# ashiq24/UNO

Measured on AMD Instinct MI355X. Metric: UNO training samples/s (421^2 Darcy), higher is better.
Workload: dtype f32; 1 GPU; Darcy 2D 421x421, UNO_9(3,64,pad=5) 64ch, batch 16/GPU, train step (fwd+loss+bwd+allreduce+Adam); global_batch=16, parallelism=dp1

## Files before the change

include/uno_spectral.h:

```cpp
#ifndef UNO_SPECTRAL_H
#define UNO_SPECTRAL_H

#ifdef __cplusplus
extern "C" {
#endif

#define UNO_SPECTRAL_ABI_VERSION 14

int uno_abi_version(void);
void* uno_upload_table(const void* host, long long bytes);

const char* uno_last_error(void);

long long uno_spectral_conv2d_fwd_ws_bytes(int B, int Ci, int Co, int m1, int m2);
long long uno_spectral_conv2d_bwd_ws_bytes(int B, int Ci, int Co, int m1, int m2);

int uno_spectral_conv2d_forward(const float* x, const float* w1, const float* w2, float* y,
                                float* xtrunc, void* ws, int B, int Ci, int Co, int H, int W,
                                int Ho, int Wo, int m1, int m2, void* stream);

int uno_spectral_conv2d_backward(const float* gy, const float* xtrunc, const float* w1,
                                 const float* w2, float* gx, float* gw1, float* gw2, void* ws,
                                 int B, int Ci, int Co, int H, int W, int Ho, int Wo, int m1,
                                 int m2, void* stream);

int uno_spectral_conv2d_forward_bf16(const void* x, const float* w1, const float* w2, void* y,
                                     float* xtrunc, void* ws, int B, int Ci, int Co, int H, int W,
                                     int Ho, int Wo, int m1, int m2, void* stream);
int uno_spectral_conv2d_backward_bf16(const void* gy, const float* xtrunc, const float* w1,
                                      const float* w2, void* gx, float* gw1, float* gw2, void* ws,
                                      int B, int Ci, int Co, int H, int W, int Ho, int Wo, int m1,
                                      int m2, void* stream);

long long uno_fft_resample3d_ws_bytes(int n_vol, int D1, int M1, int J1, int J2, int m3);
int uno_fft_resample3d(const float* x, float* y, void* ws, int n_vol, int D1, int D2, int D3, int M1, int M2, int M3,
                       int J1, const int* f1_in, const int* f1_out, int J2, const int* f2_in, const int* f2_out, int m3,
                       float scale, int herm_in, int herm_out, void* stream);

int uno_fft_resample3d_acc(const float* x, float* y, float* y_act, void* ws, int n_vol, int D1, int D2, int D3, int M1, int M2, int M3,
                           int J1, const int* f1_in, const int* f1_out, int J2, const int* f2_in, const int* f2_out, int m3,
                           float scale, int herm_in, int herm_out, void* stream);

long long uno_fft_resample3d_any_ws_bytes(int n_vol, int D1, int M1, int J1, int J2, int m3);
int uno_fft_resample3d_any(const float* x, float* y, void* ws, int n_vol, int D1, int D2, int D3, int M1, int M2, int M3,
                           int J1, const int* f1_in, const int* f1_out, int J2, const int* f2_in, const int* f2_out, int m3,
                           float scale, int herm_in, int herm_out, void* stream);

int uno_fft_resample3d_any_acc(const float* x, float* y, float* y_act, void* ws, int n_vol, int D1, int D2, int D3, int M1, int M2, int M3,
                               int J1, const int* f1_in, const int* f1_out, int J2, const int* f2_in, const int* f2_out, int m3,
                               float scale, int herm_in, int herm_out, void* stream);

long long uno_spectral_conv3d_fwd_ws_bytes(int B, int Ci, int Co, int H, int Ho, int m1, int m2, int m3);
long long uno_spectral_conv3d_bwd_ws_bytes(int B, int Ci, int Co, int H, int Ho, int m1, int m2, int m3);
int uno_spectral_conv3d_forward(const float* x, const float* const* w, float* y, float* xtrunc, void* ws,
                                int B, int Ci, int Co, int H, int W, int T, int Ho, int Wo, int To,
                                int m1, int m2, int m3, void* stream);
int uno_spectral_conv3d_backward(const float* gy, const float* xtrunc, const float* const* w, float* gx,
                                 float* const* gw, void* ws, int B, int Ci, int Co, int H, int W, int T,
                                 int Ho, int Wo, int To, int m1, int m2, int m3, void* stream);

int uno_cdft_axis(const float* in, float* out, int inverse, int n_img, int H, int m1, int m2, int m3,
                  float scale, int mask_overlap, void* stream);


int uno_dft2d_forward(const float* images, float* spec, int n_img, int H, int W, int m1, int m2,
                      float scale, int hermitian_cols, int mask_overlap, void* stream);

int uno_dft2d_inverse(const float* spec, float* images, int n_img, int H, int W, int m1, int m2,
                      float scale, int hermitian_cols, int mask_overlap, void* stream);

int uno_reserve_cus(int n);

int uno_sweep_alternation(int enable);

int uno_dft2d_inverse_add_applies(int n_img, int H, int W, int m1, int m2, int Hs, int Ws);
int uno_dft2d_inverse_add(const float* spec, float* images, int n_img, int H, int W, int m1, int m2, float scale, int hermitian_cols,
                          int mask_overlap, const float* addend, int Hs, int Ws, const int* tile_p0, const float* row_op,
                          const int* col_v0, const float* col_op, void* stream);

int uno_dft2d_forward_resample_applies(int n_img, int H, int W, int m1, int m2, int Ho, int Wo, int KW);
int uno_dft2d_forward_resample(const float* images, float* spec, int n_img, int H, int W, int m1, int m2, float scale, int hermitian_cols,
                               int mask_overlap, int group, int stride, int offset, float* resampled, int Ho, int Wo, const int* col_start,
                               const float* col_wt, int KW, const int* row_tiles, const float* row_op, void* stream);

int uno_dft2d_forward_bf16(const void* images, float* spec, int n_img, int H, int W, int m1, int m2,
                           float scale, int hermitian_cols, int mask_overlap, void* stream);
int uno_dft2d_inverse_bf16(const float* spec, void* images, int n_img, int H, int W, int m1, int m2,
                           float scale, int hermitian_cols, int mask_overlap, void* stream);

int uno_dft2d_forward_grouped(const float* images, float* spec, int n_img, int H, int W, int m1, int m2, float scale,
                              int hermitian_cols, int mask_overlap, int group, int stride, int offset, void* stream);
int uno_dft2d_inverse_grouped(const float* spec, float* images, int n_img, int H, int W, int m1, int m2, float scale,
                              int hermitian_cols, int mask_overlap, int group, int stride, int offset, void* stream);

int uno_mode_mix(const float* in, const float* const* w, float* out, int op, int B, int Ci, int Co,
                 int ncorner, int modes_per_corner, void* stream);

int uno_mode_wgrad(const float* xtrunc, const float* go, float* const* gw, int B, int Ci, int Co,
                   int ncorner, int modes_per_corner, void* stream);
int uno_mode_backward(const float* xtrunc, const float* go, const float* const* w, float* gx_spec, float* const* gw, int B, int Ci,
                      int Co, int ncorner, int modes_per_corner, int accumulate, void* stream);
int uno_mode_wgrad_acc(const float* xtrunc, const float* go, float* const* gw, int B, int Ci, int Co, int ncorner,
                       int modes_per_corner, int accumulate, void* stream);
int uno_spectral_conv2d_backward_acc(const void* gy, const float* xtrunc, const void* w1, const void* w2, void* gx,
                                     float* gw1, float* gw2, void* ws, int B, int Ci, int Co, int H, int W, int Ho, int Wo,
                                     int m1, int m2, int io_format, int accumulate_gw, void* stream);

int uno_resample2d(const float* in, float* out, float* tmp, int n_img, int H, int W, int Ho, int Wo,
                   const int* startH, const float* wtH, int KH, const int* startW, const float* wtW, int KW,
                   const int* tile_p0, const float* tile_w, int NP, int accumulate, void* stream);

int uno_channel_mix(const float* x, const float* w, const float* bias, float* y, int B, int Ci, int Co,
                    long long P, int transpose_w, int accumulate, int act_in, const float* dgelu_of, void* stream);

long long uno_channel_wgrad_ws_bytes(int B, int Ci, int Co, long long P);
int uno_channel_wgrad(const float* gy, const float* x, float* gw, float* gb, void* ws, int B, int Ci, int Co,
                      long long P, int act_x, void* stream);

int uno_channel_mix2(const float* x1, const float* x2, int C1, const float* w, const float* bias, float* y1, float* y2, int Co1,
                     float* y_act, int B, int Ci, int Co, long long P, int transpose_w, int accumulate, int act_in,
                     const float* dgelu_of, const float* proj_w, const float* proj_b, float* proj_out, void* stream);
int uno_channel_wgrad2(const float* gy, const float* x1, const float* x2, int C1, float* gw, float* gb, void* ws, int B, int Ci,
                       int Co, long long P, int act_x, int accumulate, void* stream);
int uno_channel_wgrad_finish(const void* parts, float* gw, float* gb, int Ci, int Co, long long nparts, int accumulate, void* stream);

int uno_gelu_project_forward(const float* pre, const float* w, const float* bias, float* out, int B, int C, long long P,
                             void* stream);
long long uno_gelu_project_bwd_ws_bytes(int B, int C, long long P);
int uno_gelu_project_backward(const float* pre, const float* w, const float* gout, float* gpre, float* gw, float* gb,
                              void* ws, int B, int C, long long P, void* stream);

int uno_gelu_project2_forward(const float* pre, const float* s, const float* w, const float* bias, float* out, int B, int C1, int C2,
                              long long P, int act2, void* stream);
long long uno_gelu_project2_bwd_ws_bytes(int B, int C1, int C2, long long P);
int uno_gelu_project2_backward(const float* pre, const float* s, const float* w, const float* gout, float* gpre, float* gs, float* gw,
                               float* gb, void* ws, int B, int C1, int C2, long long P, int act2, void* stream);

long long uno_rel_l2_steps_ws_bytes(int B, long long P, int T);
int uno_rel_l2_steps(const float* pred, const float* target, float* sums, float* rel, float* totals, void* ws, int B, long long P, int T,
                     void* stream);

long long uno_rollout_ws_bytes(int B, long long P, int T);
int uno_rollout_advance(float* window, const float* frame, const float* target, float* pred, void* ws, int B, int C, int T_in, long long P,
                        int T, int t, int shift, void* stream);
int uno_rollout_finish(const void* ws, float* sums, float* rel, float* totals, int B, long long P, int T, void* stream);

int uno_rollout_lift(const float* given, const float* pred, const float* feat, const float* w, const float* bias, float* h, int B, int T_in,
                     int F, int Cm, long long P, int T, int t, void* stream);
long long uno_rollout_lift_bwd_ws_bytes(int B, int T_in, int F, int Cm, long long P, int T);
int uno_rollout_lift_backward(const float* gh, const float* given, const float* pred, const float* target, const float* feat, const float* w,
                              const float* sums, const float* gL, float* gpred, float* gframe, void* parts, int B, int T_in, int F, int Cm,
                              long long P, int T, int t, void* stream);
int uno_rollout_loss_seed(const float* pred, const float* target, const float* sums, const float* gL, float* gframe, int B, long long P, int T,
                          void* stream);

int uno_channel_mix2_win(const float* x1, const float* x2, int C1, const float* w, const float* bias, float* y1, float* y2, int Co1,
                         float* y_act, int B, int Ci, int Co, int rows, int cols, int pitch, long long plane, int transpose_w,
                         int accumulate, int act_in, const float* dgelu_of, const float* proj_w, const float* proj_b, float* proj_out,
                         void* stream);
int uno_channel_wgrad2_win(const float* gy, const float* x1, const float* x2, int C1, float* gw, float* gb, void* ws, int B, int Ci,
                           int Co, int rows, int cols, int pitch, long long plane, int act_x, int accumulate, void* stream);
int uno_gelu_project_backward_win(const float* pre, const float* w, const float* gout, float* gpre, float* gw, float* gb, void* ws,
                                  int B, int C, int rows, int cols, int pitch, long long plane, void* stream);
int uno_project_backward_applies(int B, int C1, int Ci, int Co, int rows, int cols, int pitch, long long plane);
long long uno_project_backward_ws_bytes(int B, int Ci, int Co, long long P);
int uno_project_backward(const float* x1, const float* x2, int C1, const float* w, const float* pre, const float* w2, const float* gout,
                         float* g1, float* g2, float* gw, float* gb, float* gw2, float* gb2, void* ws, int B, int Ci, int Co, int rows,
                         int cols, int pitch, long long plane, int act_in, int accumulate_w, void* stream);
int uno_clear_border(float* t, long long n_planes, int Hp, int Wp, int rows, int cols, void* stream);
int uno_channel_mix_act_padded(const float* x, const float* w, const float* bias, float* y, float* y_act, int B, int Ci, int Co, int H,
                               int W, int Hp, int Wp, int act_in, void* stream);
int uno_channel_mix_dgelu_padded(const float* x, const float* w, const float* bias, const float* g_padded, float* gz, int B, int Ci,
                                 int Co, int H, int W, int Hp, int Wp, int act_in, void* stream);
int uno_lift_forward(const float* x, const float* w1, const float* b1, const float* w0, const float* b0, float* act, int B, int Cin,
                     int Cm, int Co, int H, int W, int Hp, int Wp, void* stream);
long long uno_lift_bwd_ws_bytes(int B, int Cin, int Cm, int Co, int H, int W);
int uno_lift_backward(const float* x, const float* w1, const float* b1, const float* w0, const float* b0, const float* g_act, float* gw1,
                      float* gb1, float* gw0, float* gb0, void* ws, int B, int Cin, int Cm, int Co, int H, int W, int Hp, int Wp,
                      void* stream);
int uno_lift_backward_takes_second(int B, int Cin, int Cm, int Co, int H, int W, int Hp, int Wp);
int uno_lift_backward2(const float* x, const float* w1, const float* b1, const float* w0, const float* b0, const float* g_act,
                       const float* g_act2, float* gw1, float* gb1, float* gw0, float* gb0, void* ws, int B, int Cin, int Cm, int Co,
                       int H, int W, int Hp, int Wp, void* stream);

int uno_gelu_pad(const float* s, const float* gy, float* out, int n_img, int H, int W, int Hp, int Wp, int backward,
                 void* stream);

int uno_instnorm_forward(const float* x, const float* gamma, const float* beta, float* y, float* mean, float* rstd, long long rows,
                         int C, long long N, float eps, int gelu, void* stream);
int uno_instnorm_backward(const float* x, const float* gy, const float* gamma, const float* beta, const float* mean,
                          const float* rstd, float* gx, float* s1, float* s2, long long rows, int C, long long N, int gelu,
                          void* stream);

int uno_adam_step(float* p, const float* g, float* m, float* v, long long n, int is_complex, double lr, double beta1,
                  double beta2, double eps, double weight_decay, int step, void* stream);

int uno_adam_step_multi(int n_tensors, float* const* p, const float* const* g, float* const* m, float* const* v,
                        const long long* n, const int* is_complex, double lr, double beta1, double beta2, double eps,
                        double weight_decay, int step, void* stream);

int uno_adam_step_multi_dev(int n_tensors, float* const* p, const float* const* g, float* const* m, float* const* v,
                            const long long* n, const int* is_complex, double lr, double beta1, double beta2, double eps,
                            double weight_decay, int* step_counter, float* scalars, const double* hyper, void* stream);

int uno_spectral_conv2d_forward_mixed(const void* x_bf16, const void* w1_f16, const void* w2_f16, void* y_bf16,
                                      float* xtrunc, void* ws, int B, int Ci, int Co, int H, int W, int Ho, int Wo,
                                      int modes1, int modes2, void* stream);
int uno_spectral_conv2d_backward_mixed(const void* gy_bf16, const float* xtrunc, const void* w1_f16, const void* w2_f16,
                                       void* gx_bf16, float* gw1, float* gw2, void* ws, int B, int Ci, int Co, int H, int W,
                                       int Ho, int Wo, int modes1, int modes2, void* stream);
int uno_mode_mix_f16w(const float* in, const void* const* w_f16, float* out, int op, int B, int Ci, int Co, int ncorner,
                      int modes_per_corner, void* stream);
int uno_dft2d_forward_grouped_bf16(const void* images, float* spec, int n_img, int H, int W, int m1, int m2, float scale,
                                   int hermitian_cols, int mask_overlap, int group, int stride, int offset, void* stream);
int uno_dft2d_inverse_grouped_bf16(const float* spec, void* images, int n_img, int H, int W, int m1, int m2, float scale,
                                   int hermitian_cols, int mask_overlap, int group, int stride, int offset, void* stream);
int uno_resample2d_bf16(const void* in, void* out, float* tmp, int n_img, int H, int W, int Ho, int Wo, const int* startH,
                        const float* wtH, int KH, const int* startW, const float* wtW, int KW, const int* tile_p0,
                        const float* tile_w, int NP, int accumulate, void* stream);
int uno_channel_mix_bf16(const void* x, const float* w, const float* bias, void* y, int B, int Ci, int Co, long long P,
                         int transpose_w, int accumulate, int act_in, const void* dgelu_of, void* stream);
int uno_channel_wgrad_bf16(const void* gy, const void* x, float* gw, float* gb, void* ws, int B, int Ci, int Co, long long P,
                           int act_x, void* stream);
int uno_channel_mix2_bf16(const void* x1, const void* x2, int C1, const float* w, const float* bias, void* y1, void* y2, int Co1,
                          void* y_act, int B, int Ci, int Co, long long P, int transpose_w, int accumulate, int act_in,
                          const void* dgelu_of, const float* proj_w, const float* proj_b, void* proj_out, void* stream);
int uno_channel_wgrad2_bf16(const void* gy, const void* x1, const void* x2, int C1, float* gw, float* gb, void* ws, int B, int Ci,
                            int Co, long long P, int act_x, int accumulate, void* stream);
int uno_gelu_project_forward_bf16(const void* pre, const float* w, const float* bias, void* out, int B, int C, long long P,
                                  void* stream);
int uno_gelu_project_backward_bf16(const void* pre, const float* w, const void* gout, void* gpre, float* gw, float* gb,
                                   void* ws, int B, int C, long long P, void* stream);
int uno_gelu_pad_bf16(const void* s, const void* gy, void* out, int n_img, int H, int W, int Hp, int Wp, int backward,
                      void* stream);
int uno_instnorm_forward_bf16(const void* x, const float* gamma, const float* beta, void* y, float* mean, float* rstd,
                              long long rows, int C, long long N, float eps, int gelu, void* stream);
// ... 20 lines not shown
```

uno_amd/_native.py:

```python
from __future__ import annotations

import ctypes as C
import os
import threading

import torch

_HERE = os.path.dirname(os.path.abspath(__file__))
LIB_PATH = os.path.join(_HERE, "lib", "libuno_spectral.so")
ABI_VERSION = 14

_lib = None
_lock = threading.Lock()

_fp = C.c_void_p
_i = C.c_int
_SIGNATURES = {
    "uno_abi_version": (C.c_int, []),
    "uno_last_error": (C.c_char_p, []),
    "uno_dft2d_any_ws_bytes": (C.c_longlong, [_i] * 5),
    "uno_scratch_provide": (C.c_int, [_fp, C.c_longlong]),
    "uno_spectral_conv2d_fwd_ws_bytes": (C.c_longlong, [_i] * 5),
    "uno_spectral_conv2d_bwd_ws_bytes": (C.c_longlong, [_i] * 5),
    "uno_spectral_conv2d_forward": (C.c_int, [_fp] * 6 + [_i] * 9 + [_fp]),
    "uno_spectral_conv2d_backward": (C.c_int, [_fp] * 8 + [_i] * 9 + [_fp]),
    "uno_spectral_conv2d_forward_bf16": (C.c_int, [_fp] * 6 + [_i] * 9 + [_fp]),
    "uno_spectral_conv2d_backward_bf16": (C.c_int, [_fp] * 8 + [_i] * 9 + [_fp]),
    "uno_fft_resample3d_ws_bytes": (C.c_longlong, [_i] * 6),
    "uno_fft_resample3d": (C.c_int, [_fp] * 3 + [_i] * 8 + [_fp, _fp, _i, _fp, _fp, _i, C.c_float, _i, _i, _fp]),
    "uno_fft_resample3d_acc": (C.c_int, [_fp] * 4 + [_i] * 8 + [_fp, _fp, _i, _fp, _fp, _i, C.c_float, _i, _i, _fp]),
    "uno_fft_resample3d_any_ws_bytes": (C.c_longlong, [_i] * 6),
    "uno_fft_resample3d_any": (C.c_int, [_fp] * 3 + [_i] * 8 + [_fp, _fp, _i, _fp, _fp, _i, C.c_float, _i, _i, _fp]),
    "uno_fft_resample3d_any_acc": (C.c_int, [_fp] * 4 + [_i] * 8 + [_fp, _fp, _i, _fp, _fp, _i, C.c_float, _i, _i, _fp]),
    "uno_dft2d_forward": (C.c_int, [_fp, _fp] + [_i] * 5 + [C.c_float, _i, _i, _fp]),
    "uno_dft2d_forward_bf16": (C.c_int, [_fp, _fp] + [_i] * 5 + [C.c_float, _i, _i, _fp]),
    "uno_dft2d_inverse_bf16": (C.c_int, [_fp, _fp] + [_i] * 5 + [C.c_float, _i, _i, _fp]),
    "uno_dft2d_inverse": (C.c_int, [_fp, _fp] + [_i] * 5 + [C.c_float, _i, _i, _fp]),
    "uno_reserve_cus": (C.c_int, [_i]),
    "uno_sweep_alternation": (C.c_int, [_i]),
    "uno_dft2d_inverse_add_applies": (C.c_int, [_i] * 7),
    "uno_dft2d_forward_resample_applies": (C.c_int, [_i] * 8),
    "uno_dft2d_forward_resample": (C.c_int, [_fp, _fp] + [_i] * 5 + [C.c_float] + [_i] * 5 + [_fp, _i, _i, _fp, _fp, _i, _fp, _fp, _fp]),
    "uno_dft2d_inverse_add": (C.c_int, [_fp, _fp] + [_i] * 5 + [C.c_float, _i, _i, _fp, _i, _i, _fp, _fp, _fp, _fp, _fp]),
    "uno_dft2d_forward_grouped": (C.c_int, [_fp, _fp] + [_i] * 5 + [C.c_float] + [_i] * 5 + [_fp]),
    "uno_dft2d_inverse_grouped": (C.c_int, [_fp, _fp] + [_i] * 5 + [C.c_float] + [_i] * 5 + [_fp]),
    "uno_mode_mix": (C.c_int, [_fp, C.POINTER(_fp), _fp] + [_i] * 6 + [_fp]),
    "uno_mode_wgrad": (C.c_int, [_fp, _fp, C.POINTER(_fp)] + [_i] * 5 + [_fp]),
    "uno_mode_backward": (C.c_int, [_fp, _fp, C.POINTER(_fp), _fp, C.POINTER(_fp)] + [_i] * 6 + [_fp]),
    "uno_spectral_conv3d_fwd_ws_bytes": (C.c_longlong, [_i] * 8),
    "uno_spectral_conv3d_bwd_ws_bytes": (C.c_longlong, [_i] * 8),
    "uno_spectral_conv3d_forward": (C.c_int, [_fp, C.POINTER(_fp), _fp, _fp, _fp] + [_i] * 12 + [_fp]),
    "uno_spectral_conv3d_backward": (C.c_int, [_fp, _fp, C.POINTER(_fp), _fp, C.POINTER(_fp), _fp] + [_i] * 12 + [_fp]),
    "uno_cdft_axis": (C.c_int, [_fp, _fp] + [_i] * 6 + [C.c_float, _i, _fp]),
    "uno_resample2d": (C.c_int, [_fp, _fp, _fp] + [_i] * 5 + [_fp, _fp, _i, _fp, _fp, _i, _fp, _fp, _i, _i, _fp]),
    "uno_channel_mix": (C.c_int, [_fp, _fp, _fp, _fp, _i, _i, _i, C.c_longlong, _i, _i, _i, _fp, _fp]),
    "uno_channel_wgrad_ws_bytes": (C.c_longlong, [_i, _i, _i, C.c_longlong]),
    "uno_channel_wgrad": (C.c_int, [_fp, _fp, _fp, _fp, _fp, _i, _i, _i, C.c_longlong, _i, _fp]),
    "uno_channel_mix2": (C.c_int, [_fp, _fp, _i, _fp, _fp, _fp, _fp, _i, _fp, _i, _i, _i, C.c_longlong, _i, _i, _i, _fp, _fp, _fp, _fp, _fp]),
    "uno_channel_wgrad2": (C.c_int, [_fp, _fp, _fp, _i, _fp, _fp, _fp, _i, _i, _i, C.c_longlong, _i, _i, _fp]),
    "uno_channel_mix2_win": (C.c_int, [_fp, _fp, _i, _fp, _fp, _fp, _fp, _i, _fp, _i, _i, _i, _i, _i, _i, C.c_longlong, _i, _i, _i, _fp, _fp, _fp, _fp, _fp]),
    "uno_channel_mix_ws_bytes": (C.c_longlong, [_i, _i, C.c_longlong, _i]),
    "uno_clear_border": (C.c_int, [_fp, C.c_longlong, _i, _i, _i, _i, _fp]),
    "uno_channel_mix_act_padded": (C.c_int, [_fp, _fp, _fp, _fp, _fp, _i, _i, _i, _i, _i, _i, _i, _i, _fp]),
    "uno_lift_forward": (C.c_int, [_fp] * 6 + [_i] * 8 + [_fp]),
    "uno_lift_bwd_ws_bytes": (C.c_longlong, [_i] * 6),
    "uno_lift_backward": (C.c_int, [_fp] * 11 + [_i] * 8 + [_fp]),
    "uno_lift_backward2": (C.c_int, [_fp] * 12 + [_i] * 8 + [_fp]),
    "uno_lift_backward_takes_second": (C.c_int, [_i] * 8),
    "uno_channel_mix_dgelu_padded": (C.c_int, [_fp, _fp, _fp, _fp, _fp, _i, _i, _i, _i, _i, _i, _i, _i, _fp]),
    "uno_channel_wgrad2_win": (C.c_int, [_fp, _fp, _fp, _i, _fp, _fp, _fp, _i, _i, _i, _i, _i, _i, C.c_longlong, _i, _i, _fp]),
    "uno_gelu_project_backward_win": (C.c_int, [_fp] * 7 + [_i, _i, _i, _i, _i, C.c_longlong, _fp]),
    "uno_channel_wgrad_finish": (C.c_int, [_fp, _fp, _fp, _i, _i, C.c_longlong, _i, _fp]),
    "uno_mode_wgrad_acc": (C.c_int, [_fp, _fp, C.POINTER(_fp)] + [_i] * 6 + [_fp]),
    "uno_spectral_conv2d_backward_acc": (C.c_int, [_fp] * 8 + [_i] * 11 + [_fp]),
    "uno_upload_table": (C.c_void_p, [_fp, C.c_longlong]),
    "uno_project_backward_applies": (C.c_int, [_i] * 7 + [C.c_longlong]),
    "uno_project_backward_ws_bytes": (C.c_longlong, [_i, _i, _i, C.c_longlong]),
    "uno_project_backward": (C.c_int, [_fp, _fp, _i] + [_fp] * 11 + [_i] * 6 + [C.c_longlong, _i, _i, _fp]),
    "uno_gelu_project_forward": (C.c_int, [_fp, _fp, _fp, _fp, _i, _i, C.c_longlong, _fp]),
    "uno_gelu_project_bwd_ws_bytes": (C.c_longlong, [_i, _i, C.c_longlong]),
    "uno_gelu_project_backward": (C.c_int, [_fp] * 7 + [_i, _i, C.c_longlong, _fp]),
    "uno_gelu_project2_forward": (C.c_int, [_fp] * 5 + [_i, _i, _i, C.c_longlong, _i, _fp]),
    "uno_gelu_project2_bwd_ws_bytes": (C.c_longlong, [_i, _i, _i, C.c_longlong]),
    "uno_gelu_project2_backward": (C.c_int, [_fp] * 9 + [_i, _i, _i, C.c_longlong, _i, _fp]),
    "uno_rel_l2_steps_ws_bytes": (C.c_longlong, [_i, C.c_longlong, _i]),
    "uno_rel_l2_steps": (C.c_int, [_fp] * 6 + [_i, C.c_longlong, _i, _fp]),
    "uno_rollout_ws_bytes": (C.c_longlong, [_i, C.c_longlong, _i]),
    "uno_rollout_advance": (C.c_int, [_fp] * 5 + [_i, _i, _i, C.c_longlong, _i, _i, _i, _fp]),
    "uno_rollout_finish": (C.c_int, [_fp] * 4 + [_i, C.c_longlong, _i, _fp]),
    "uno_rollout_lift": (C.c_int, [_fp] * 6 + [_i, _i, _i, _i, C.c_longlong, _i, _i, _fp]),
    "uno_rollout_lift_bwd_ws_bytes": (C.c_longlong, [_i, _i, _i, _i, C.c_longlong, _i]),
    "uno_rollout_lift_backward": (C.c_int, [_fp] * 11 + [_i, _i, _i, _i, C.c_longlong, _i, _i, _fp]),
    "uno_rollout_loss_seed": (C.c_int, [_fp] * 5 + [_i, C.c_longlong, _i, _fp]),
    "uno_gelu_pad": (C.c_int, [_fp, _fp, _fp] + [_i] * 6 + [_fp]),
    "uno_transpose_batched": (C.c_int, [_fp, _fp, _i, C.c_longlong, _i] + [C.c_longlong] * 4 + [_fp]),
    "uno_instnorm_forward": (C.c_int, [_fp] * 6 + [C.c_longlong, _i, C.c_longlong, C.c_float, _i, _fp]),
    "uno_instnorm_backward": (C.c_int, [_fp] * 9 + [C.c_longlong, _i, C.c_longlong, _i, _fp]),
    "uno_adam_step": (C.c_int, [_fp, _fp, _fp, _fp, C.c_longlong, _i] + [C.c_double] * 5 + [_i, _fp]),
    "uno_adam_step_multi": (C.c_int, [_i, C.POINTER(_fp), C.POINTER(_fp), C.POINTER(_fp), C.POINTER(_fp), C.POINTER(C.c_longlong),
                                      C.POINTER(_i)] + [C.c_double] * 5 + [_i, _fp]),
    "uno_adam_step_multi_dev": (C.c_int, [_i, C.POINTER(_fp), C.POINTER(_fp), C.POINTER(_fp), C.POINTER(_fp), C.POINTER(C.c_longlong),
                                          C.POINTER(_i)] + [C.c_double] * 5 + [_fp, _fp, _fp, _fp]),
    "uno_spectral_conv2d_forward_mixed": (C.c_int, [_fp] * 6 + [_i] * 9 + [_fp]),
    "uno_spectral_conv2d_backward_mixed": (C.c_int, [_fp] * 8 + [_i] * 9 + [_fp]),
    "uno_mode_mix_f16w": (C.c_int, [_fp, C.POINTER(_fp), _fp] + [_i] * 6 + [_fp]),
    "uno_dft2d_forward_grouped_bf16": (C.c_int, [_fp, _fp] + [_i] * 5 + [C.c_float] + [_i] * 5 + [_fp]),
    "uno_dft2d_inverse_grouped_bf16": (C.c_int, [_fp, _fp] + [_i] * 5 + [C.c_float] + [_i] * 5 + [_fp]),
    "uno_resample2d_bf16": (C.c_int, [_fp, _fp, _fp] + [_i] * 5 + [_fp, _fp, _i, _fp, _fp, _i, _fp, _fp, _i, _i, _fp]),
    "uno_channel_mix_bf16": (C.c_int, [_fp, _fp, _fp, _fp, _i, _i, _i, C.c_longlong, _i, _i, _i, _fp, _fp]),
    "uno_channel_wgrad_bf16": (C.c_int, [_fp, _fp, _fp, _fp, _fp, _i, _i, _i, C.c_longlong, _i, _fp]),
    "uno_channel_mix2_bf16": (C.c_int, [_fp, _fp, _i, _fp, _fp, _fp, _fp, _i, _fp, _i, _i, _i, C.c_longlong, _i, _i, _i, _fp, _fp, _fp, _fp, _fp]),
    "uno_channel_wgrad2_bf16": (C.c_int, [_fp, _fp, _fp, _i, _fp, _fp, _fp, _i, _i, _i, C.c_longlong, _i, _i, _fp]),
    "uno_gelu_project_forward_bf16": (C.c_int, [_fp, _fp, _fp, _fp, _i, _i, C.c_longlong, _fp]),
    "uno_gelu_project_backward_bf16": (C.c_int, [_fp] * 7 + [_i, _i, C.c_longlong, _fp]),
    "uno_gelu_pad_bf16": (C.c_int, [_fp, _fp, _fp] + [_i] * 6 + [_fp]),
    "uno_instnorm_forward_bf16": (C.c_int, [_fp] * 6 + [C.c_longlong, _i, C.c_longlong, C.c_float, _i, _fp]),
    "uno_instnorm_backward_bf16": (C.c_int, [_fp] * 9 + [C.c_longlong, _i, C.c_longlong, _i, _fp]),
    "uno_profile_begin": (C.c_int, [_i]),
    "uno_profile_end": (C.c_int, []),
    "uno_profile_get": (C.c_int, [_i, C.c_char_p, _i, C.POINTER(C.c_double), C.POINTER(C.c_double)]),
}
EXPORTED_SYMBOLS = tuple(_SIGNATURES)


def lib():
    global _lib
    if _lib is None:
        with _lock:
            if _lib is None:
                if not os.path.exists(LIB_PATH):
                    raise RuntimeError(
                        f"uno_amd: native library {LIB_PATH} is missing - build it with "
                        "`python -m uno_amd.build` (hipcc, gfx950); there is no CPU fallback")
                h = C.CDLL(LIB_PATH)
                for name, (res, args) in _SIGNATURES.items():
                    fn = getattr(h, name)
                    fn.restype = res
                    fn.argtypes = args
                if h.uno_abi_version() != ABI_VERSION:
                    raise RuntimeError(f"uno_amd: ABI mismatch, library {h.uno_abi_version()} != binding {ABI_VERSION}")
                _lib = h
    return _lib


def _check(rc: int, what: str):
    if rc != 0:
        msg = lib().uno_last_error().decode(errors="replace")
        raise RuntimeError(f"{what} failed (code {rc}): {msg}")


def _ptr(t: torch.Tensor):
    return C.c_void_p(t.data_ptr())


def _opt(t):
    return _ptr(t) if t is not None else C.c_void_p(0)


def _count(lead) -> int:
    n = 1
    for d in lead:
        n *= d
    return n


def _stream(t: torch.Tensor):
    return C.c_void_p(torch.cuda.current_stream(t.device).cuda_stream)


class _scratch:

    def __init__(self, device, nbytes):
        self.bytes, self.device, self.buf = nbytes, device, None

    def __enter__(self):
        if self.bytes > 0:
            self.buf = torch.empty(self.bytes, dtype=torch.uint8, device=self.device)
            _check(lib().uno_scratch_provide(_ptr(self.buf), self.bytes), "uno_scratch_provide")
        return self

    def __exit__(self, *exc):
        if self.bytes > 0:
            lib().uno_scratch_provide(None, 0)
        return False


class _any_mode_scratch(_scratch):

    def __init__(self, device, *needs):
        L = lib()
        _scratch.__init__(self, device, max((int(L.uno_dft2d_any_ws_bytes(*[int(v) for v in n])) for n in needs), default=0))


class _mix_scratch(_scratch):

    def __init__(self, device, Ci, Co, P, bf16):
        _scratch.__init__(self, device, int(lib().uno_channel_mix_ws_bytes(int(Ci), int(Co), int(P), 1 if bf16 else 0)))

# ... 17 lines not shown
    _require(t, torch.bfloat16 if bf16 else torch.float32, name)
    return bf16


def _weights_half(w1, w2, bf16):
    if w1.dtype == torch.float16:
        if not bf16:
            raise RuntimeError("uno_amd: half-precision weight storage goes with bfloat16 activations")
        for w, name in ((w1, "weights1"), (w2, "weights2")):
            _require(w, torch.float16, name)
            if w.dim() != 5 or w.shape[-1] != 2:
                raise RuntimeError("uno_amd: half-precision weights are stored as (Ci, Co, m1, m2, 2) = (re, im)")
        return True
    _require(w1, torch.complex64, "weights1")
    _require(w2, torch.complex64, "weights2")
    return False


def _complex_grad_buffers(out, shape, n: int, device, accumulate: bool):
    if out is None:
        return [torch.empty(shape, dtype=torch.complex64, device=device) for _ in range(n)], False
    gws = list(out)
    for t in gws:
        _require(t, torch.complex64, "weight-gradient buffer")
        if tuple(t.shape) != tuple(shape):
            raise RuntimeError("uno_amd: weight-gradient buffer has the wrong shape")
    return gws, accumulate


def _real_grad_buffers(out_w, out_b, Ci: int, Co: int, need_bias: bool, device, accumulate: bool):
    if out_w is None:
        gw = torch.empty((Co, Ci), dtype=torch.float32, device=device)
        return gw, (torch.empty((Co,), dtype=torch.float32, device=device) if need_bias else None), False
    gw, gb = out_w, (out_b if need_bias else None)
    _require(gw, torch.float32, "weight-gradient buffer")
    if gw.numel() != Co * Ci or (need_bias and (gb is None or gb.numel() != Co)):
        raise RuntimeError("uno_amd: gradient buffers do not match the layer")
    if gb is not None:
        _require(gb, torch.float32, "bias-gradient buffer")
    return gw, gb, accumulate


def spectral_conv2d_forward(x, w1, w2, Ho: int, Wo: int, xt_out=None):
    bf16 = _act_dtype(x, "x")
    wh = _weights_half(w1, w2, bf16)
    B, Ci, H, W = x.shape
    Ci2, Co, m1, m2 = w1.shape[:4]
    if Ci2 != Ci or tuple(w2.shape) != tuple(w1.shape):
        raise RuntimeError(f"uno_amd: weight shapes {tuple(w1.shape)} / {tuple(w2.shape)} do not match input channels {Ci}")
    L = lib()
    with torch.cuda.device(x.device):
        y = torch.empty((B, Co, Ho, Wo), dtype=x.dtype, device=x.device)
        if xt_out is None:
            xt = torch.empty((B, Ci, 2 * m1, m2), dtype=torch.complex64, device=x.device)
        else:
            xt = xt_out
            _require(xt, torch.complex64, "xtrunc buffer")
            if tuple(xt.shape) != (B, Ci, 2 * m1, m2):
                raise RuntimeError("uno_amd: xtrunc buffer has the wrong shape")
        ws = torch.empty(max(1, L.uno_spectral_conv2d_fwd_ws_bytes(B, Ci, Co, m1, m2)), dtype=torch.uint8, device=x.device)
        fn = L.uno_spectral_conv2d_forward_mixed if wh else _entry("uno_spectral_conv2d_forward", bf16)
        with _any_mode_scratch(x.device, (B * Ci, H, W, m1, m2), (B * Co, Ho, Wo, m1, m2)):
            rc = fn(_ptr(x), _ptr(w1), _ptr(w2), _ptr(y), _ptr(xt), _ptr(ws), B, Ci, Co, H, W, Ho, Wo, m1, m2, _stream(x))
    _check(rc, "uno_spectral_conv2d_forward")
    return y, xt


def spectral_conv2d_backward(gy, xt, w1, w2, H: int, W: int, need_gx=True, need_gw=True, gw_out=None, accumulate_gw=False):
    bf16 = _act_dtype(gy, "grad_output")
    _require(xt, torch.complex64, "xtrunc")
    wh = _weights_half(w1, w2, bf16)
    B, Co, Ho, Wo = gy.shape
    Ci, Co2, m1, m2 = w1.shape[:4]
    if Co2 != Co:
        raise RuntimeError("uno_amd: grad_output channels do not match the weights")
    L = lib()
    with torch.cuda.device(gy.device):
        gx = torch.empty((B, Ci, H, W), dtype=gy.dtype, device=gy.device) if need_gx else None
        gw1, gw2, accumulate_gw = None, None, accumulate_gw and need_gw
        if need_gw:
            (gw1, gw2), accumulate_gw = _complex_grad_buffers(gw_out, (Ci, Co, m1, m2), 2, gy.device, accumulate_gw)
        ws = torch.empty(max(1, L.uno_spectral_conv2d_bwd_ws_bytes(B, Ci, Co, m1, m2)), dtype=torch.uint8, device=gy.device)
        with _any_mode_scratch(gy.device, (B * Co, Ho, Wo, m1, m2), (B * Ci, H, W, m1, m2)):
            rc = L.uno_spectral_conv2d_backward_acc(_ptr(gy), _ptr(xt), _ptr(w1), _ptr(w2), _opt(gx), _opt(gw1), _opt(gw2),
                                                    _ptr(ws), B, Ci, Co, H, W, Ho, Wo, m1, m2, 2 if wh else (1 if bf16 else 0),
                                                    1 if accumulate_gw else 0, _stream(gy))
    _check(rc, "uno_spectral_conv2d_backward")
    return gx, gw1, gw2


def _fft_resample3d(any_grid: bool, x, out_size, f1, f2, m3, scale, adjoint, out, act):
    name = "uno_fft_resample3d_any" if any_grid else "uno_fft_resample3d"
    _require(x, torch.float32, "x")
    *lead, D1, D2, D3 = x.shape
    M1, M2, M3 = (int(v) for v in out_size)
    n = _count(lead)
    for t in (*f1, *f2):
        if t.dtype != torch.int32 or not t.is_cuda or not t.is_contiguous():
            raise RuntimeError("uno_amd: frequency tables must be contiguous int32 device tensors")
    J1, J2 = f1[0].numel(), f2[0].numel()
    if any_grid and (f1[1].numel() != J1 or f2[1].numel() != J2):
        raise RuntimeError("uno_amd: the forward and inverse frequency tables of an axis must have the same length")
    L = lib()
    with torch.cuda.device(x.device):
        ws = torch.empty(max(1, getattr(L, name + "_ws_bytes")(n, D1, M1, J1, J2, int(m3))), dtype=torch.uint8, device=x.device)
        if out is not None:
            _require(out, torch.float32, "out")
            if tuple(out.shape) != (*lead, M1, M2, M3) or not out.is_contiguous():
                raise RuntimeError(f"uno_amd: out must be a contiguous {(*lead, M1, M2, M3)} tensor")
            ya = torch.empty_like(out) if act else None
            fn, dst, res = getattr(L, name + "_acc"), (_ptr(out), _opt(ya)), ((out, ya) if act else out)
        else:
            res = torch.empty((*lead, M1, M2, M3), dtype=torch.float32, device=x.device)
            fn, dst = getattr(L, name), (_ptr(res),)
        rc = fn(_ptr(x), *dst, _ptr(ws), n, D1, D2, D3, M1, M2, M3, J1, _ptr(f1[0]), _ptr(f1[1]), J2, _ptr(f2[0]), _ptr(f2[1]),
                int(m3), float(scale), int(adjoint), int(not adjoint), _stream(x))
    _check(rc, name + ("_acc" if out is not None else ""))
    return res


def fft_resample3d(x, out_size, f1, f2, m3: int, scale: float, adjoint: bool, out=None, act=False):
    return _fft_resample3d(False, x, out_size, f1, f2, m3, scale, adjoint, out, act)


def fft_resample3d_any(x, out_size, f1, f2, m3: int, scale: float, adjoint: bool, out=None, act=False):
    return _fft_resample3d(True, x, out_size, f1, f2, m3, scale, adjoint, out, act)


def dft2d_forward(images, m1, m2, scale=1.0, hermitian_cols=False, mask_overlap=False, out=None, channel_offset=0):
    bf16 = _act_dtype(images, "images")
    *lead, H, W = images.shape
    n = _count(lead)
    if out is None:
        spec = torch.empty((*lead, 2 * m1, m2), dtype=torch.complex64, device=images.device)
        with torch.cuda.device(images.device):
            fn = _entry("uno_dft2d_forward", bf16)
            with _any_mode_scratch(images.device, (n, H, W, m1, m2)):
                rc = fn(_ptr(images), _ptr(spec), n, H, W, m1, m2, float(scale), int(hermitian_cols), int(mask_overlap), _stream(images))
        _check(rc, "uno_dft2d_forward")
        return spec
    _require(out, torch.complex64, "out")
    if images.dim() != 4 or out.dim() != 4 or out.shape[0] != images.shape[0] or tuple(out.shape[2:]) != (2 * m1, m2) \
            or channel_offset < 0 or channel_offset + images.shape[1] > out.shape[1]:
        raise RuntimeError("uno_amd: out must be (B, Ctot, 2*m1, m2) with room for the image channels at channel_offset")
    with torch.cuda.device(images.device):
        fn = _entry("uno_dft2d_forward_grouped", bf16)
        with _any_mode_scratch(images.device, (n, H, W, m1, m2)):
            rc = fn(_ptr(images), _ptr(out), n, H, W, m1, m2, float(scale), int(hermitian_cols),
                    int(mask_overlap), images.shape[1], out.shape[1], int(channel_offset), _stream(images))
    _check(rc, "uno_dft2d_forward_grouped")
    return out


def reserve_cus(n: int) -> int:
    return int(lib().uno_reserve_cus(int(n)))


def sweep_alternation(enable: bool) -> bool:
    return bool(lib().uno_sweep_alternation(1 if enable else 0))


def sweep_direction(mode: str, mask: int = 255) -> int:
    if mode not in ("alternate", "forward", "reversed") or not 0 <= int(mask) <= 255:
        raise ValueError(f"uno_amd: sweep_direction({mode!r}, {mask!r}): mode is alternate | forward | reversed, mask 0 .. 255")
    value = {"alternate": int(mask), "forward": 0, "reversed": 256 | int(mask)}[mode]
    if value == 1:
        raise ValueError("uno_amd: sweep_direction('alternate', 1): the C entry point reads 1 as 'every family' (255)")
    return int(lib().uno_sweep_alternation(value))


def dft2d_inverse_add_applies(n_img, H, W, m1, m2, Hs, Ws) -> bool:
    return bool(lib().uno_dft2d_inverse_add_applies(int(n_img), int(H), int(W), int(m1), int(m2), int(Hs), int(Ws)))


def dft2d_forward_resample_applies(n_img, H, W, m1, m2, Ho, Wo, KW) -> bool:
    return bool(lib().uno_dft2d_forward_resample_applies(int(n_img), int(H), int(W), int(m1), int(m2), int(Ho), int(Wo), int(KW)))


def dft2d_forward_resample(images, m1, m2, Ho, Wo, tables, scale=1.0, hermitian_cols=False, mask_overlap=False, out=None, channel_offset=0):
    _require(images, torch.float32, "images")
    col_start, col_wt, row_tiles, row_op = tables
    *lead, H, W = images.shape
    n = _count(lead)
    group = stride = 0
    if out is None:
        spec = torch.empty((*lead, 2 * m1, m2), dtype=torch.complex64, device=images.device)
    else:
        _require(out, torch.complex64, "out")
        if images.dim() != 4 or out.dim() != 4 or out.shape[0] != images.shape[0] or tuple(out.shape[2:]) != (2 * m1, m2) \
                or channel_offset < 0 or channel_offset + images.shape[1] > out.shape[1]:
            raise RuntimeError("uno_amd: out must be (B, Ctot, 2*m1, m2) with room for the image channels at channel_offset")
        spec, group, stride = out, images.shape[1], out.shape[1]
    res = torch.empty((*lead, Ho, Wo), dtype=torch.float32, device=images.device)
    with torch.cuda.device(images.device):
        rc = lib().uno_dft2d_forward_resample(_ptr(images), _ptr(spec), n, H, W, m1, m2, float(scale), int(hermitian_cols), int(mask_overlap),
                                              int(group), int(stride), int(channel_offset), _ptr(res), int(Ho), int(Wo), _ptr(col_start),
                                              _ptr(col_wt), int(col_wt.shape[1]), _ptr(row_tiles), _ptr(row_op), _stream(images))
    _check(rc, "uno_dft2d_forward_resample")
    return spec, res


def dft2d_inverse(spec, H, W, scale=1.0, hermitian_cols=True, mask_overlap=True, channels=None, channel_offset=0,
                  dtype=torch.float32, addend=None):
    _require(spec, torch.complex64, "spec")
    *lead, r2, m2 = spec.shape
    m1 = r2 // 2
    if addend is not None:
        t, (p0, rowop, v0, colop) = addend
        _require(t, torch.float32, "addend")
        if channels is not None or dtype != torch.float32 or tuple(t.shape[:-2]) != tuple(lead):
            raise RuntimeError("uno_amd: dft2d_inverse(addend=) takes the plain float32 form with one addend image per spectrum")
        n = _count(lead)
        img = torch.empty((*lead, H, W), dtype=torch.float32, device=spec.device)
        with torch.cuda.device(spec.device):
            rc = lib().uno_dft2d_inverse_add(_ptr(spec), _ptr(img), n, H, W, m1, m2, float(scale), int(hermitian_cols), int(mask_overlap),
                                             _ptr(t), t.shape[-2], t.shape[-1], _ptr(p0), _ptr(rowop), _ptr(v0), _ptr(colop), _stream(spec))
        _check(rc, "uno_dft2d_inverse_add")
        return img
    if channels is None:
        n = _count(lead)
        if dtype not in (torch.float32, torch.bfloat16):
            raise RuntimeError("uno_amd: images are float32 or bfloat16")
        img = torch.empty((*lead, H, W), dtype=dtype, device=spec.device)
        with torch.cuda.device(spec.device):
            fn = _entry("uno_dft2d_inverse", dtype == torch.bfloat16)
            with _any_mode_scratch(spec.device, (n, H, W, m1, m2)):
                rc = fn(_ptr(spec), _ptr(img), n, H, W, m1, m2, float(scale), int(hermitian_cols), int(mask_overlap), _stream(spec))
        _check(rc, "uno_dft2d_inverse")
        return img
    if dtype not in (torch.float32, torch.bfloat16):
        raise RuntimeError("uno_amd: images are float32 or bfloat16")
    if spec.dim() != 4 or channel_offset < 0 or channels < 1 or channel_offset + channels > spec.shape[1]:
        raise RuntimeError("uno_amd: spec must be (B, Ctot, 2*m1, m2) holding the requested channel range")
    B = spec.shape[0]
    img = torch.empty((B, channels, H, W), dtype=dtype, device=spec.device)
    with torch.cuda.device(spec.device):
        fn = _entry("uno_dft2d_inverse_grouped", dtype == torch.bfloat16)
        with _any_mode_scratch(spec.device, (B * channels, H, W, m1, m2)):
            rc = fn(_ptr(spec), _ptr(img), B * channels, H, W, m1, m2, float(scale), int(hermitian_cols),
                    int(mask_overlap), int(channels), spec.shape[1], int(channel_offset), _stream(spec))
    _check(rc, "uno_dft2d_inverse_grouped")
    return img


def _ptr_array(ts):
    return (C.c_void_p * len(ts))(*[t.data_ptr() for t in ts])


def mode_mix(inp, weights, op: int):
    _require(inp, torch.complex64, "spectrum")
    half = weights[0].dtype == torch.float16
    for w in weights:
        _require(w, torch.float16 if half else torch.complex64, "weights")
    B = inp.shape[0]
    Ci, Co = weights[0].shape[:2]
    nc = len(weights)
    Mc = weights[0][0, 0].numel() // (2 if half else 1)
    cout = Co if op == 0 else Ci
    out = torch.empty((B, cout, *inp.shape[2:]), dtype=torch.complex64, device=inp.device)
    with torch.cuda.device(inp.device):
        fn = lib().uno_mode_mix_f16w if half else lib().uno_mode_mix
        rc = fn(_ptr(inp), _ptr_array(weights), _ptr(out), op, B, Ci, Co, nc, Mc, _stream(inp))
    _check(rc, "uno_mode_mix")
    return out


def mode_wgrad(xt, go, weight_shape, ncorner: int, out=None, accumulate: bool = False):
    _require(xt, torch.complex64, "xtrunc")
    _require(go, torch.complex64, "grad spectrum")
    B, Ci = xt.shape[:2]
    Co = go.shape[1]
    gws, accumulate = _complex_grad_buffers(out, weight_shape, ncorner, xt.device, accumulate)
    Mc = gws[0][0, 0].numel()
    with torch.cuda.device(xt.device):
        rc = lib().uno_mode_wgrad_acc(_ptr(xt), _ptr(go), _ptr_array(gws), B, Ci, Co, ncorner, Mc, 1 if accumulate else 0, _stream(xt))
    _check(rc, "uno_mode_wgrad")
    return gws


def mode_backward(xt, go, weights, out=None, accumulate: bool = False):
    _require(xt, torch.complex64, "xtrunc")
    _require(go, torch.complex64, "grad spectrum")
    for w in weights:
        _require(w, torch.complex64, "weights")
    B, Ci = xt.shape[:2]
    Co = go.shape[1]
    nc = len(weights)
    Mc = weights[0][0, 0].numel()
    gws, accumulate = _complex_grad_buffers(out, weights[0].shape, nc, xt.device, accumulate)
    gX = torch.empty((B, Ci, nc * Mc), dtype=torch.complex64, device=xt.device)
    with torch.cuda.device(xt.device):
        rc = lib().uno_mode_backward(_ptr(xt), _ptr(go), _ptr_array(list(weights)), _ptr(gX), _ptr_array(gws), B, Ci, Co, nc, Mc,
                                     1 if accumulate else 0, _stream(xt))
    _check(rc, "uno_mode_backward")
    return gX, gws


def spectral_conv3d_forward(x, ws_, Ho: int, Wo: int, To: int):
    _require(x, torch.float32, "x")
    if len(ws_) != 4:
        raise RuntimeError("uno_amd: the 3-D spectral convolution takes four weight tensors")
    for w in ws_:
        _require(w, torch.complex64, "weights")
        if tuple(w.shape) != tuple(ws_[0].shape):
            raise RuntimeError("uno_amd: weights1..4 must have one shape")
    B, Ci, H, W, T = x.shape
# ... 839 lines not shown
```

uno_amd/block2d.py:

```python
import torch
import torch.nn.functional as F
from torch.autograd.function import once_differentiable

from . import _native
from ._param_grads import _grad_targets, _note_use, _stack_arrived, _stack_grad_slot, _stack_take, _stack_wanted
from .pointwise import _mix2_forward, _mix2_input_grads, _plain, _wgrad_into
from .resample import fused_resample_tables, resample_adjoint, resample_forward, upsample_add_tables


def _half_weights(w1, w2):
    out = []
    capturing = w1.is_cuda and torch.cuda.is_current_stream_capturing()
    with torch.no_grad():
        for w in (w1, w2):
            cached = None if capturing else getattr(w, "_uno_half", None)
            if cached is None or cached[0] != w._version or cached[1].device != w.device or cached[2] != w.data_ptr():
                cached = (w._version, torch.view_as_real(w.detach()).half().contiguous(), w.data_ptr())
                if not capturing:
                    try:
                        w._uno_half = cached
                    except (AttributeError, RuntimeError):
                        pass
            out.append(cached[1])
    return out[0], out[1]


def _xt_slot(stack):
    return None if stack is None else stack.xt


def _xt_dest(stack, B, Ci, m1, m2, device):
    slot = _xt_slot(stack)
    return torch.empty((B, Ci, 2 * m1, m2), dtype=torch.complex64, device=device) if slot is None else slot


def _block_prologue(ctx, iw, x, Ci, w1, w2, cw, cb, Ho, Wo, half_weights):
    B, _, H, W = x.shape
    ctx.stack = _stack_take(w1, (B, Ci, 2 * w1.shape[2], w1.shape[3]), x.device, _stack_wanted(ctx, iw, x, half_weights))
    w1, w2 = _plain(w1), _plain(w2)
    if half_weights:
        w1, w2 = _half_weights(w1, w2)
    cwm = _plain(cw).reshape(cw.shape[0], Ci)
    cb = None if cb is None else _plain(cb)
    same = (H, W) == (Ho, Wo)
    return w1, w2, cwm, cb, same, same or Ho * Wo < H * W


def _pointwise_input_grads(g_src, w, C1, gx1, gx2, geom, dgelu_of=None, dgelu_total=False, g_act=None):
    H, W, Ho, Wo, same, mix_last = geom
    B = g_src.shape[0]
    direct = same or not mix_last

    def dest(gx):
        return gx.view(B, gx.shape[1], -1) if direct else None

    g1, g2 = g_act, None
    if gx1 is not None and gx2 is not None:
        g1, g2 = _mix2_input_grads(g_src, w, C1, out1=dest(gx1), out2=dest(gx2))
    else:
        if gx1 is not None and g1 is None:
            g1 = _native.channel_mix(g_src, w if C1 == w.shape[1] else w[:, :C1].contiguous(), None, transpose_w=True, out=dest(gx1),
                                     dgelu_of=dgelu_of, dgelu_total=dgelu_total)
        if gx2 is not None:
            g2 = _native.channel_mix(g_src, w[:, C1:].contiguous(), None, transpose_w=True, out=dest(gx2))
    if not direct:
        for g, gx in ((g1, gx1), (g2, gx2)):
            if gx is not None:
                resample_adjoint(g.view(B, gx.shape[1], Ho, Wo), H, W, out=gx)


class _SpectralConv2dFn(torch.autograd.Function):

    @staticmethod
    def forward(ctx, x, w1, w2, Ho, Wo, half_weights=False):
        ctx.params = (w1, w2)
        x = _plain(x)
        ctx.stack = _stack_take(w1, (x.shape[0], x.shape[1], 2 * w1.shape[2], w1.shape[3]), x.device, _stack_wanted(ctx, 1, x, half_weights))
        w1, w2 = _plain(w1), _plain(w2)
        if half_weights:
            w1, w2 = _half_weights(w1, w2)
        y, xt = _native.spectral_conv2d_forward(x, w1, w2, int(Ho), int(Wo), xt_out=_xt_slot(ctx.stack))
        ctx.save_for_backward(xt, w1, w2)
        ctx.in_hw = (x.shape[-2], x.shape[-1])
        return y

    @staticmethod
    @once_differentiable
    def backward(ctx, gy):
        xt, w1, w2 = ctx.saved_tensors
        gx, gw1, gw2, _ = _spectral_backward(_plain(gy), xt, w1, w2, ctx.in_hw[0], ctx.in_hw[1], ctx.needs_input_grad[0],
                                          ctx.needs_input_grad[1] or ctx.needs_input_grad[2],
                                          ctx.needs_input_grad[1] and ctx.needs_input_grad[2], ctx.params, ctx.stack)
        return gx, gw1, gw2, None, None, None


FUSE_UPSAMPLE_ADD = True


def _fused_addend(t, H, W, m1, m2, adjoint):
    if not FUSE_UPSAMPLE_ADD or t.dtype != torch.float32 or t.dim() != 4 or not t.is_cuda:
        return None
    Hs, Ws = t.shape[-2], t.shape[-1]
    if Hs * Ws >= H * W or not _native.dft2d_inverse_add_applies(t.shape[0] * t.shape[1], H, W, m1, m2, Hs, Ws):
        return None
    tabs = upsample_add_tables(Hs, Ws, H, W, str(t.device), bool(adjoint))
    return None if tabs is None else (t, tabs)


FUSE_FORWARD_RESAMPLE = True


def _fused_resample(x, m1, m2, Ho, Wo, adjoint):
    if not FUSE_FORWARD_RESAMPLE or x.dtype != torch.float32 or x.dim() != 4 or not x.is_cuda:
        return None
    H, W = x.shape[-2], x.shape[-1]
    n = x.shape[0] * x.shape[1]
    if Ho * Wo >= H * W or not _native.dft2d_forward_resample_applies(n, H, W, m1, m2, Ho, Wo, 1):
        return None
    tabs = fused_resample_tables(H, W, Ho, Wo, str(x.device), bool(adjoint))
    if tabs is None or not _native.dft2d_forward_resample_applies(n, H, W, m1, m2, Ho, Wo, tabs[1].shape[1]):
        return None
    return tabs


def _stage_wgrad(stack, gslot, xt, gO, w1, w2, leaves, both_gw, need_gx):
    if gslot is not None:
        return (None, *_stack_arrived(stack, leaves, w1.shape, both_gw))
    tg = _grad_targets(leaves) if both_gw else None
    _note_use(leaves[0])
    out, acc = (tg.dest, tg.accumulate) if tg else (None, False)
    gX = None
    if need_gx and w1.dtype == torch.complex64:
        gX, (gw1, gw2) = _native.mode_backward(xt, gO, [w1, w2], out=out, accumulate=acc)
        gX = gX.view(xt.shape)
    else:
        gw1, gw2 = _native.mode_wgrad(xt, gO, tuple(w1.shape[:4]), 2, out=out, accumulate=acc)
    if tg:
        gw1, gw2 = tg.returned
    return gX, gw1, gw2


def _spectral_backward(gs, xt, w1, w2, H, W, need_gx, need_gw, both_gw, leaves, stack, join=None, addend=None, k1=None):
    B, Co = gs.shape[:2]
    Ci, _, m1, m2 = w1.shape[:4]
    gslot = _stack_grad_slot(stack, Co) if (stack is not None and need_gw) else None
    merging = join is not None and need_gx and bool(join.spectra)
    if addend is not None and not need_gx:
        raise RuntimeError("uno_amd: an addend for the input gradient needs the input gradient")
    if gslot is None and not merging and addend is None and k1 is None and not (need_gx and need_gw and w1.dtype == torch.complex64):
        tg = _grad_targets(leaves) if (need_gw and both_gw) else None
        if need_gw:
            _note_use(leaves[0])
        gx, gw1, gw2 = _native.spectral_conv2d_backward(gs, xt, w1, w2, H, W, need_gx=need_gx, need_gw=need_gw,
                                                        gw_out=tg.dest if tg else None, accumulate_gw=bool(tg and tg.accumulate))
        if tg:
            gw1, gw2 = tg.returned
        return gx, gw1, gw2, False
    gO = _native.dft2d_forward(gs, m1, m2, 1.0, True, True, out=gslot) if k1 is None else k1(gslot)
    gX, gw1, gw2 = _stage_wgrad(stack, gslot, xt, gO, w1, w2, leaves, both_gw, need_gx) if need_gw else (None, None, None)
    gx = None
    if need_gx:
        if gX is None:
            gX = _native.mode_mix(gO.view(B, Co, 2, m1 * m2), [w1, w2], 1).view(B, Ci, 2 * m1, m2)
        if merging:
            gX = join.merge(gX, (H, W))
        gx = _native.dft2d_inverse(gX, H, W, 1.0 / (H * W), False, False, dtype=gs.dtype, addend=addend)
    return gx, gw1, gw2, gslot is not None


class _OperatorBlock2dFn(torch.autograd.Function):

    @staticmethod
    def forward(ctx, x, w1, w2, cw, cb, Ho, Wo, half_weights=False, fuse_gelu=False, join=None, out_join=None):
        ctx.leaves = (w1, w2, cw, cb)
        ctx.join = None
        if join is not None:
            join.reset()
            if ctx.needs_input_grad[0]:
                join.owner = True
                ctx.join = join
        x = _plain(x)
        B, Ci, H, W = x.shape
        Co = cw.shape[0]
        w1, w2, cwm, cb, same, mix_last = _block_prologue(ctx, 1, x, Ci, w1, w2, cw, cb, Ho, Wo, half_weights)
        t = fused = None
        if not mix_last and not half_weights and x.dtype == torch.float32:
            t = _native.channel_mix(x.view(B, Ci, -1), cwm, cb).view(B, Co, H, W)
            fused = _fused_addend(t, Ho, Wo, w1.shape[2], w1.shape[3], False)
        if fused is not None:
            m1, m2 = w1.shape[2], w1.shape[3]
            xt = _xt_dest(ctx.stack, B, Ci, m1, m2, x.device)
            _native.dft2d_forward(x, m1, m2, 1.0 / (H * W), out=xt, channel_offset=0)
            O = _native.mode_mix(xt.view(B, Ci, 2, m1 * m2), [w1, w2], 0)
            s = _native.dft2d_inverse(O.view(B, Co, 2 * m1, m2), Ho, Wo, 1.0, True, True, addend=fused)
        elif mix_last and not same and not half_weights and (rs := _fused_resample(x, w1.shape[2], w1.shape[3], Ho, Wo, False)) is not None:
            m1, m2 = w1.shape[2], w1.shape[3]
            xt = _xt_dest(ctx.stack, B, Ci, m1, m2, x.device)
            _, pre_act = _native.dft2d_forward_resample(x, m1, m2, Ho, Wo, rs, 1.0 / (H * W), out=xt, channel_offset=0)
            O = _native.mode_mix(xt.view(B, Ci, 2, m1 * m2), [w1, w2], 0)
            s = _native.dft2d_inverse(O.view(B, Co, 2 * m1, m2), Ho, Wo, 1.0, True, True)
        else:
            pre_act = None
            if mix_last and not same:
                pre_act = resample_forward(x, Ho, Wo)
            s, xt = _native.spectral_conv2d_forward(x, w1, w2, Ho, Wo, xt_out=_xt_slot(ctx.stack))
        out = s
        if fused is not None:
            act = x
            if fuse_gelu:
                out = F.gelu(s)
        elif mix_last:
            act = x if same else pre_act
            if fuse_gelu:
                _, out = _native.channel_mix2(act.view(B, Ci, -1), None, cwm, cb, out=s.view(B, Co, -1), accumulate=True, y_act=True)
                out = out.view(B, Co, Ho, Wo)
            else:
                _native.channel_mix(act.view(B, Ci, -1), cwm, cb, out=s.view(B, Co, -1))
        else:
            act = x
            if t is None:
                t = _native.channel_mix(x.view(B, Ci, -1), cwm, cb).view(B, Co, H, W)
            resample_forward(t, Ho, Wo, out=s)
            if fuse_gelu:
                out = F.gelu(s)
        ctx.save_for_backward(xt, w1, w2, cwm, act, s if fuse_gelu else None)
        ctx.geom = (H, W, same, mix_last, cb is not None, tuple(cw.shape))
        ctx.out_join = None
        if fuse_gelu and out_join is not None:
            out_join.pre, out_join.dgelu_applied = s, False
            ctx.out_join = out_join
        return out

    @staticmethod
    @once_differentiable
    def backward(ctx, gs):
        xt, w1, w2, cwm, act, pre = ctx.saved_tensors
        H, W, same, mix_last, has_bias, cw_shape = ctx.geom
        gs = _plain(gs)
        if pre is not None:
            oj = ctx.out_join
            if oj is not None and oj.dgelu_applied and oj.pre is not None and oj.pre.data_ptr() == pre.data_ptr():
                oj.dgelu_applied = False
            else:
                gs = torch.ops.aten.gelu_backward(gs, pre)
            if oj is not None:
                oj.pre = None
        B, Co, Ho, Wo = gs.shape
        Ci = cwm.shape[1]
        need_gx = ctx.needs_input_grad[0]
        need_gw = ctx.needs_input_grad[1] or ctx.needs_input_grad[2]
        need_gc = ctx.needs_input_grad[3] or (has_bias and ctx.needs_input_grad[4])
        join = ctx.join
        lw1, lw2, lcw, lcb = ctx.leaves
        g_act = addend = g_t = k1 = None
        if not mix_last:
            rs = _fused_resample(gs, w1.shape[2], w1.shape[3], H, W, True) if w1.dtype == torch.complex64 else None
            if rs is None:
                g_t = resample_adjoint(gs, H, W).view(B, Co, -1)
            else:
                both = []

                def k1(out):
                    both.extend(_native.dft2d_forward_resample(gs, w1.shape[2], w1.shape[3], H, W, rs, 1.0, True, True, out=out))
                    return both[0]
        if mix_last and not same and need_gx and gs.dtype == torch.float32:
            g_act = _native.channel_mix(gs.view(B, Co, -1), cwm, None, transpose_w=True).view(B, Ci, Ho, Wo)
            addend = _fused_addend(g_act, H, W, w1.shape[2], w1.shape[3], True)
        gx, gw1, gw2, stacked = _spectral_backward(gs, xt, w1, w2, H, W, need_gx, need_gw, ctx.needs_input_grad[1] and ctx.needs_input_grad[2],
                                                   (lw1, lw2), ctx.stack, join, addend, k1)
        if k1 is not None:
            g_t = both[1].view(B, Co, -1)
        pstack = ctx.stack if stacked else None
        gcw = gcb = None
        xpre = join.pre if (join is not None and need_gx) else None
        own_last = xpre is not None and not join.pending
        dg_view = xpre.view(B, Ci, -1) if own_last else None
        direct = same or not mix_last
        g_src = gs.view(B, Co, -1) if mix_last else g_t
        if need_gx and (direct or addend is None):
            _pointwise_input_grads(g_src, cwm, Ci, gx, None, (H, W, Ho, Wo, same, mix_last), dgelu_of=dg_view if direct else None,
                                   dgelu_total=own_last and direct, g_act=g_act)
        dg_done = own_last and direct
        if need_gc:
            gcw, gcb = _wgrad_into((lcw, lcb), g_src, act.view(B, Ci, -1), None, ctx.needs_input_grad[3],
                                   has_bias and ctx.needs_input_grad[4], stack=pstack)
            gcw = None if gcw is None else gcw.view(cw_shape)
        if join is not None:
            if need_gx:
                dg_done = join.apply(gx, xpre if not dg_done else None) or dg_done
                if xpre is not None:
                    if not dg_done:
                        gx = torch.ops.aten.gelu_backward(gx, xpre)
                    join.dgelu_applied = True
            join.reset()
        return gx, gw1, gw2, gcw, gcb, None, None, None, None, None, None


class _OperatorBlock2dCatFn(torch.autograd.Function):

    @staticmethod
    def forward(ctx, x1, x2, w1, w2, cw, cb, Ho, Wo, half_weights=False, defer=None):
        ctx.leaves = (w1, w2, cw, cb)
        ctx.defer = defer if (defer is not None and defer.owner and ctx.needs_input_grad[1]) else None
        x1, x2 = _plain(x1), _plain(x2)
        B, C1, H, W = x1.shape
        C2 = x2.shape[1]
        Ci, Co, m1, m2 = w1.shape
        w1, w2, cwm, cb, same, mix_last = _block_prologue(ctx, 2, x1, Ci, w1, w2, cw, cb, Ho, Wo, half_weights)
        xt = _xt_dest(ctx.stack, B, Ci, m1, m2, x1.device)
        _native.dft2d_forward(x1, m1, m2, 1.0 / (H * W), out=xt, channel_offset=0)
        _native.dft2d_forward(x2, m1, m2, 1.0 / (H * W), out=xt, channel_offset=C1)
        O = _native.mode_mix(xt.view(B, Ci, 2, m1 * m2), [w1, w2], 0)
        t = fused = None
        if not mix_last and not half_weights and x1.dtype == torch.float32:
            t = _mix2_forward(x1.view(B, C1, -1), x2.view(B, C2, -1), cwm, cb).view(B, Co, H, W)
            fused = _fused_addend(t, Ho, Wo, m1, m2, False)
        s = _native.dft2d_inverse(O.view(B, Co, 2 * m1, m2), Ho, Wo, 1.0, True, True, dtype=x1.dtype, addend=fused)
        if fused is not None:
            a1, a2 = x1, x2
        elif mix_last:
            a1 = x1 if same else resample_forward(x1, Ho, Wo)
            a2 = x2 if same else resample_forward(x2, Ho, Wo)
            _mix2_forward(a1.view(B, C1, -1), a2.view(B, C2, -1), cwm, cb, out=s.view(B, Co, -1), accumulate=True)
        else:
            a1, a2 = x1, x2
            if t is None:
                t = _mix2_forward(x1.view(B, C1, -1), x2.view(B, C2, -1), cwm, cb).view(B, Co, H, W)
            resample_forward(t, Ho, Wo, out=s)
        ctx.save_for_backward(xt, w1, w2, cwm, a1, a2)
        ctx.geom = (H, W, same, mix_last, cb is not None, tuple(cw.shape))
        return s

    @staticmethod
    @once_differentiable
    def backward(ctx, gs):
        xt, w1, w2, cwm, a1, a2 = ctx.saved_tensors
        H, W, same, mix_last, has_bias, cw_shape = ctx.geom
        gs = _plain(gs)
        B, Co, Ho, Wo = gs.shape
        Ci, _, m1, m2 = w1.shape[:4]
        C1, C2 = a1.shape[1], a2.shape[1]
        need1, need2 = ctx.needs_input_grad[0], ctx.needs_input_grad[1]
        need_gw = ctx.needs_input_grad[2] or ctx.needs_input_grad[3]
        need_gc = ctx.needs_input_grad[4] or (has_bias and ctx.needs_input_grad[5])
        lw1, lw2, lcw, lcb = ctx.leaves
        both_gw = ctx.needs_input_grad[2] and ctx.needs_input_grad[3]
        gslot = _stack_grad_slot(ctx.stack, Co) if (ctx.stack is not None and need_gw) else None
        rs = _fused_resample(gs, m1, m2, H, W, True) if (not mix_last and w1.dtype == torch.complex64) else None
        if rs is not None:
            gO, g_src = _native.dft2d_forward_resample(gs, m1, m2, H, W, rs, 1.0, True, True, out=gslot)
            g_src = g_src.view(B, Co, -1)
        else:
            g_src = gs.view(B, Co, -1) if mix_last else resample_adjoint(gs, H, W).view(B, Co, -1)
            gO = _native.dft2d_forward(gs, m1, m2, 1.0, True, True, out=gslot)
        gXp, gw1, gw2 = _stage_wgrad(ctx.stack, gslot, xt, gO, w1, w2, (lw1, lw2), both_gw, need1 or need2) if need_gw else (None, None, None)
        gx1 = gx2 = None
        defer = ctx.defer if (need2 and ctx.defer is not None and ctx.defer.owner) else None
        if need1 or need2:
            gX = gXp if gXp is not None else _native.mode_mix(gO.view(B, Co, 2, m1 * m2), [w1, w2], 1).view(B, Ci, 2 * m1, m2)
            if need1:
                gx1 = _native.dft2d_inverse(gX, H, W, 1.0 / (H * W), False, False, channels=C1, channel_offset=0, dtype=gs.dtype)
            if defer is not None:
                defer.spectra.append((gX[:, C1:].contiguous(), (H, W)))
            elif need2:
                gx2 = _native.dft2d_inverse(gX, H, W, 1.0 / (H * W), False, False, channels=C2, channel_offset=C1, dtype=gs.dtype)
        gcw = gcb = None
        geom = (H, W, Ho, Wo, same, mix_last)
        if defer is not None:
            cw2 = cwm[:, C1:].contiguous()

            def x2_part(out, dg=None):
                _pointwise_input_grads(g_src, cw2, C2, out, None, geom, dgelu_of=None if dg is None else dg.view(B, C2, -1),
                                       dgelu_total=dg is not None)
            defer.pending.append((x2_part, same or not mix_last))
            _pointwise_input_grads(g_src, cwm, C1, gx1, None, geom)
        else:
            _pointwise_input_grads(g_src, cwm, C1, gx1, gx2, geom)
        if need_gc:
            gcw, gcb = _wgrad_into((lcw, lcb), g_src, a1.view(B, C1, -1), a2.view(B, C2, -1), ctx.needs_input_grad[4],
                                   has_bias and ctx.needs_input_grad[5])
            gcw = None if gcw is None else gcw.view(cw_shape)
        if ctx.defer is not None and gx2 is not None:
            gx2 = ctx.defer.late(gx2)
        return gx1, gx2, gw1, gw2, gcw, gcb, None, None, None, None


def spectral_conv2d(x, weights1, weights2, dim1, dim2):
    return _SpectralConv2dFn.apply(x, weights1, weights2, dim1, dim2)


def spectral_conv2d_mixed(x, weights1, weights2, dim1, dim2):
    if x.dtype != torch.bfloat16:
        raise RuntimeError(f"spectral_conv2d_mixed: input must be bfloat16 (got {x.dtype})")
    for w in (weights1, weights2):
        if w.dtype == torch.float16 and w.shape[-1] != 2:
            raise RuntimeError("spectral_conv2d_mixed: half-precision weights are stored as (..., 2) = (re, im)")
    if weights1.dtype == torch.float16:
        return _SpectralConv2dHalfFn.apply(x, weights1, weights2, dim1, dim2)
    return _SpectralConv2dFn.apply(x, weights1, weights2, dim1, dim2)


class _SpectralConv2dHalfFn(torch.autograd.Function):

    @staticmethod
    def forward(ctx, x, w1h, w2h, Ho, Wo):
        x, w1h, w2h = _plain(x), _plain(w1h), _plain(w2h)
        y, xt = _native.spectral_conv2d_forward(x, w1h, w2h, int(Ho), int(Wo))
        ctx.save_for_backward(xt, w1h, w2h)
        ctx.in_hw = (x.shape[-2], x.shape[-1])
        return y

    @staticmethod
    @once_differentiable
    def backward(ctx, gy):
        xt, w1h, w2h = ctx.saved_tensors
        need_gx = ctx.needs_input_grad[0]
        need_gw = ctx.needs_input_grad[1] or ctx.needs_input_grad[2]
        gx, gw1, gw2 = _native.spectral_conv2d_backward(_plain(gy), xt, w1h, w2h, ctx.in_hw[0], ctx.in_hw[1],
                                                        need_gx=need_gx, need_gw=need_gw)
        if need_gw:
            gw1, gw2 = torch.view_as_real(gw1).half(), torch.view_as_real(gw2).half()
        return gx, gw1, gw2, None, None
```

uno_amd/build.py:

```python
from __future__ import annotations

import argparse
import concurrent.futures as cf
import hashlib
import os
import shutil
import subprocess
import sys

HERE = os.path.dirname(os.path.abspath(__file__))
CSRC = os.path.join(HERE, "csrc")
LIBDIR = os.path.join(HERE, "lib")
LIB = os.path.join(LIBDIR, "libuno_spectral.so")
STAMP = os.path.join(LIBDIR, "libuno_spectral.stamp")
SOURCES = ["capi.hip", "capi_spectral.hip", "capi_pointwise.hip", "dft2d_fwd.hip", "dft2d_fwd_r4.hip", "dft2d_fwd_fd.hip", "dft2d_inv.hip", "dft2d_inv_b.hip", "dft2d_inv_c.hip", "dft2d_inv_add.hip", "dft2d_plane.hip", "dft2d_b16.hip", "mode_gemm.hip", "cdft_axis.hip", "dft3d_volume.hip", "dft_generic.hip", "resample3d_any.hip", "resample2d.hip", "channel_mix.hip", "channel_wgrad.hip", "adam.hip", "pointwise_fused.hip", "instnorm.hip", "lift_bwd.hip", "rel_l2_steps.hip", "rollout.hip", "rollout_train.hip"]
HEADERS = ["uno_common.h", "channel_mix_common.h", "dft2d_fwd_common.h", "dft2d_fwd_kernel.h", "dft2d_fwd_ft_kernel.h", "dft2d_fwd_ht_kernel.h", "dft2d_fwd_fd_kernel.h", "dft2d_inv_kernel.h", "dft2d_inv_add_kernel.h", os.path.join("..", "..", "include", "uno_spectral.h")]
ARCH = "gfx950"
FLAGS = ["-O3", "-std=c++17", "-fPIC", f"--offload-arch={ARCH}", "-fno-gpu-rdc", "-Wall", "-Wno-unused-function"]
EXTRA_FLAGS = {"mode_gemm.hip": ["-mllvm", "-amdgpu-mfma-vgpr-form"], "dft2d_inv_add.hip": ["-mllvm", "-amdgpu-mfma-vgpr-form"]}


def _hipcc() -> str:
    for cand in (os.environ.get("HIPCC"), shutil.which("hipcc"), "/opt/rocm/bin/hipcc"):
        if cand and os.path.exists(cand):
            return cand
    raise RuntimeError("hipcc not found (set HIPCC or install ROCm)")


def _digest() -> str:
    h = hashlib.sha256()
    for f in SOURCES + HEADERS:
        with open(os.path.join(CSRC, f), "rb") as fh:
            h.update(fh.read())
    h.update(" ".join(FLAGS).encode())
    h.update(repr(sorted(EXTRA_FLAGS.items())).encode())
    return h.hexdigest()


def build(force: bool = False, verbose: bool = False) -> str:
    os.makedirs(LIBDIR, exist_ok=True)
    digest = _digest()
    if not force and os.path.exists(LIB) and os.path.exists(STAMP) and open(STAMP).read().strip() == digest:
        return LIB
    hipcc = _hipcc()
    objdir = os.path.join(LIBDIR, "obj")
    os.makedirs(objdir, exist_ok=True)

    def compile_one(src):
        obj = os.path.join(objdir, os.path.splitext(src)[0] + ".o")
        cmd = [hipcc, *FLAGS, *EXTRA_FLAGS.get(src, []), "-c", os.path.join(CSRC, src), "-o", obj]
        if verbose:
            print(" ".join(cmd), flush=True)
        r = subprocess.run(cmd, capture_output=True, text=True)
        if r.returncode != 0:
            raise RuntimeError(f"hipcc failed on {src}:\n{r.stdout}\n{r.stderr}")
        if verbose and r.stderr.strip():
            print(r.stderr)
        return obj

    jobs = min(len(SOURCES), os.cpu_count() or 1, int(os.environ.get("MAX_JOBS", 16)))
    with cf.ThreadPoolExecutor(max_workers=max(1, jobs)) as ex:
        objs = list(ex.map(compile_one, SOURCES))
    cmd = [hipcc, "-shared", "-fPIC", f"--offload-arch={ARCH}", "-fno-gpu-rdc", *objs, "-o", LIB]
    r = subprocess.run(cmd, capture_output=True, text=True)
    if r.returncode != 0:
        raise RuntimeError(f"link failed:\n{r.stdout}\n{r.stderr}")
    with open(STAMP, "w") as fh:
        fh.write(digest)
    return LIB


if __name__ == "__main__":
    ap = argparse.ArgumentParser()
    ap.add_argument("--force", action="store_true")
    ap.add_argument("--verbose", action="store_true")
    a = ap.parse_args()
    print(build(a.force, a.verbose))
```

uno_amd/csrc/capi_spectral.hip:

```cpp
#include "../../include/uno_spectral.h"
#include "uno_common.h"

#include <cstdlib>
#include <map>
#include <mutex>

namespace uno {

static int check_modes2d(const char* who, int H, int W, int Ho, int Wo, int m1, int m2) {
    if (H < 1 || W < 1 || Ho < 1 || Wo < 1) { set_error("%s: empty grid %dx%d -> %dx%d", who, H, W, Ho, Wo); return -1; }
    if (m1 < 1 || m1 > H || m1 > Ho) {
        set_error("%s: modes1=%d incompatible with grid rows %d -> %d (need 1 <= modes1 <= min rows)", who, m1, H, Ho);
        return -1;
    }
    if (m2 < 1 || m2 > W / 2 + 1 || m2 > Wo / 2 + 1) {
        set_error("%s: modes2=%d incompatible with grid cols %d -> %d (need modes2 <= cols/2+1)", who, m2, W, Wo);
        return -1;
    }
    return 0;
}

static int dft2d(bool inverse, const float* in, float* out, int n_img, int H, int W, int m1, int m2, float scale,
                 int herm, int mask, hipStream_t s, int sp_group = 0, int sp_stride = 0, int sp_offset = 0, int bf16 = 0) {
    const char* who = inverse ? "uno_dft2d_inverse" : "uno_dft2d_forward";
// ... 68 lines not shown
                     float2* const* out_w, int B, int Ci, int Co, int nc, int Mc, hipStream_t s, int w_half = 0, int accumulate = 0) {
    ModeGemmParams p;
    const int rc = mode_gemm_params(p, op, act, w, go, out_act, out_w, B, Ci, Co, nc, Mc, s, w_half, accumulate);
    if (rc != 0) return rc < 0 ? rc : 0;
    return launch_mode_gemm(p, s);
}

static int mode_backward(const float2* xtrunc, const float2* go, const float2* const* w, float2* gx_spec, float2* const* gw, int B, int Ci,
                         int Co, int nc, int Mc, hipStream_t s, int accumulate) {
    ModeGemmParams pa, pb;
    const int ra = mode_gemm_params(pa, 1, go, w, nullptr, gx_spec, nullptr, B, Ci, Co, nc, Mc, s, 0, 0);
    if (ra < 0) return ra;
    const int rb = mode_gemm_params(pb, 2, xtrunc, nullptr, go, nullptr, gw, B, Ci, Co, nc, Mc, s, 0, accumulate);
    if (rb < 0) return rb;
    if (ra == 0 && rb == 0) return launch_mode_gemm_pair(pa, pb, s);
    if (rb == 0) if (int rc = launch_mode_gemm(pb, s)) return rc;
    if (ra == 0) return launch_mode_gemm(pa, s);
    return 0;
}

}

using namespace uno;


namespace {
struct SideStream {
    hipStream_t s = nullptr;
    hipEvent_t fork_ev = nullptr, join_ev = nullptr;
    std::mutex mu;
    bool ok = false;
};
SideStream* side_stream_of_current_device() {
    static std::mutex mu;
    static std::map<int, SideStream*> table;
    int dev = 0;
    if (hipGetDevice(&dev) != hipSuccess) return nullptr;
    std::lock_guard<std::mutex> g(mu);
    auto it = table.find(dev);
    if (it != table.end()) return it->second->ok ? it->second : nullptr;
    SideStream* ss = new SideStream();
    ss->ok = hipStreamCreateWithFlags(&ss->s, hipStreamNonBlocking) == hipSuccess &&
             hipEventCreateWithFlags(&ss->fork_ev, hipEventDisableTiming) == hipSuccess &&
             hipEventCreateWithFlags(&ss->join_ev, hipEventDisableTiming) == hipSuccess;
    table[dev] = ss;
    return ss->ok ? ss : nullptr;
}
}

extern "C" {

long long uno_dft2d_any_ws_bytes(int n_img, int H, int W, int m1, int m2) {
    (void)W;
    if (n_img <= 0 || H <= 0 || m2 <= 0) return 0;
    return (m1 > 40 || m2 > 48) ? 8LL * n_img * H * m2 : 0;
}

long long uno_spectral_conv2d_fwd_ws_bytes(int B, int Ci, int Co, int m1, int m2) {
    (void)Ci;
    return 8LL * B * Co * 2 * m1 * m2;
}

long long uno_spectral_conv2d_bwd_ws_bytes(int B, int Ci, int Co, int m1, int m2) {
    return 8LL * B * (Ci + Co) * 2 * m1 * m2;
}

int uno_dft2d_forward(const float* images, float* spec, int n_img, int H, int W, int m1, int m2, float scale,
                      int hermitian_cols, int mask_overlap, void* stream) {
    return dft2d(false, images, spec, n_img, H, W, m1, m2, scale, hermitian_cols, mask_overlap, (hipStream_t)stream);
}

int uno_dft2d_inverse(const float* spec, float* images, int n_img, int H, int W, int m1, int m2, float scale,
                      int hermitian_cols, int mask_overlap, void* stream) {
    return dft2d(true, spec, images, n_img, H, W, m1, m2, scale, hermitian_cols, mask_overlap, (hipStream_t)stream);
}

int uno_dft2d_inverse_add_applies(int n_img, int H, int W, int m1, int m2, int Hs, int Ws) {
    if (n_img < 1 || H < 1 || W < 1 || m1 < 1 || m2 < 1 || Hs < 1 || Ws < 1 || m1 > H || m2 > W / 2 + 1 || m1 > 40 || m2 > 48) return 0;
    Dft2dParams p;
    p.n_img = n_img; p.H = H; p.W = W; p.m1 = m1; p.m2 = m2; p.herm = 1; p.mask = 1;
    p.sp_group = n_img; p.sp_stride = 0;
    p.add_Hs = Hs; p.add_Ws = Ws;
    if (dft2d_inv_plane_applies(p)) return 0;
    return dft2d_inv_add_applies(p) ? 1 : 0;
}

int uno_dft2d_inverse_add(const float* spec, float* images, int n_img, int H, int W, int m1, int m2, float scale, int hermitian_cols,
                          int mask_overlap, const float* addend, int Hs, int Ws, const int* tile_p0, const float* row_op,
                          const int* col_v0, const float* col_op, void* stream) {
    const char* who = "uno_dft2d_inverse_add";
    if (n_img < 0) { set_error("%s: negative image count", who); return -1; }
    if (n_img > 0 && (!spec || !images || !addend || !tile_p0 || !row_op || !col_v0 || !col_op)) { set_error("%s: null pointer", who); return -1; }
    if (int rc = check_modes2d(who, H, W, H, W, m1, m2)) return rc;
    if (Hs < 1 || Ws < 12 || (long long)Hs * Ws * 4 > 0x7fffffffLL) { set_error("%s: bad addend grid %dx%d", who, Hs, Ws); return -1; }
    if (n_img == 0) return 0;
    if (!uno_dft2d_inverse_add_applies(n_img, H, W, m1, m2, Hs, Ws)) {
        set_error("%s: the fused form does not apply to %d images of %dx%d, modes (%d, %d) (query uno_dft2d_inverse_add_applies)", who, n_img, H, W, m1, m2);
        return -3;
    }
    Dft2dParams p;
    p.in = spec; p.out = images; p.n_img = n_img; p.H = H; p.W = W; p.m1 = m1; p.m2 = m2;
    p.scale = scale; p.herm = hermitian_cols ? 1 : 0; p.mask = mask_overlap ? 1 : 0;
    p.sp_group = n_img; p.sp_stride = 0;
    p.twH = twiddle_table(H);
    p.twW = twiddle_table(W);
    if (!p.twH || !p.twW) return -6;
    p.add_src = addend; p.add_Hs = Hs; p.add_Ws = Ws; p.add_p0 = tile_p0; p.add_rowop = row_op; p.add_v0 = col_v0; p.add_colop = col_op;
#ifdef UNO_K3A_DEV
    { static const int dev_exp = getenv("UNO_K3A_STAGGER") ? atoi(getenv("UNO_K3A_STAGGER")) : 0; p.exp = dev_exp; }
#endif
    return launch_dft2d_inv_add(p, (hipStream_t)stream);
}

static void fwd_resample_shape(Dft2dParams& p, int n_img, int H, int W, int m1, int m2, int Ho, int Wo, int KW) {
    p.n_img = n_img; p.H = H; p.W = W; p.m1 = m1; p.m2 = m2;
    p.fd_Ho = Ho; p.fd_Wo = Wo; p.fd_KW = KW;
}

int uno_dft2d_forward_resample_applies(int n_img, int H, int W, int m1, int m2, int Ho, int Wo, int KW) {
    if (n_img < 1 || H < 1 || W < 1 || m1 < 1 || m2 < 1 || Ho < 1 || Wo < 1 || KW < 1 || m1 > H || m2 > W / 2 + 1 || m1 > 40 || m2 > 48) return 0;
    Dft2dParams p;
    fwd_resample_shape(p, n_img, H, W, m1, m2, Ho, Wo, KW);
    return dft2d_fwd_fd_applies(p) ? 1 : 0;
}

int uno_dft2d_forward_resample(const float* images, float* spec, int n_img, int H, int W, int m1, int m2, float scale, int hermitian_cols,
                               int mask_overlap, int group, int stride, int offset, float* resampled, int Ho, int Wo, const int* col_start,
                               const float* col_wt, int KW, const int* row_tiles, const float* row_op, void* stream) {
    const char* who = "uno_dft2d_forward_resample";
    if (n_img < 0) { set_error("%s: negative image count", who); return -1; }
    if (n_img > 0 && (!images || !spec || !resampled || !col_start || !col_wt || !row_tiles || !row_op)) { set_error("%s: null pointer", who); return -1; }
    if (int rc = check_modes2d(who, H, W, H, W, m1, m2)) return rc;
    if (Ho < 1 || Wo < 1 || KW < 1) { set_error("%s: bad output grid %dx%d or band (%d taps)", who, Ho, Wo, KW); return -1; }
    if (n_img == 0) return 0;
    if (group <= 0) { group = n_img; stride = 0; offset = 0; }
    else if (offset < 0 || stride < offset + group || n_img % group) {
        set_error("%s: bad spectrum grouping (group %d, stride %d, offset %d, images %d)", who, group, stride, offset, n_img);
        return -1;
    }
    if (!uno_dft2d_forward_resample_applies(n_img, H, W, m1, m2, Ho, Wo, KW)) {
        set_error("%s: the fused form does not apply to %d images of %dx%d -> %dx%d, modes (%d, %d), %d taps (query uno_dft2d_forward_resample_applies)",
                  who, n_img, H, W, Ho, Wo, m1, m2, KW);
        return -3;
    }
    Dft2dParams p;
    fwd_resample_shape(p, n_img, H, W, m1, m2, Ho, Wo, KW);
    p.in = images; p.out = spec; p.scale = scale; p.herm = hermitian_cols ? 1 : 0; p.mask = mask_overlap ? 1 : 0;
    p.sp_group = group; p.sp_stride = stride; p.sp_offset = offset;
    p.twH = twiddle_table(H);
    p.twW = twiddle_table(W);
    if (!p.twH || !p.twW) return -6;
    p.fd_out = resampled; p.fd_startW = col_start; p.fd_wtW = col_wt; p.fd_tiles = row_tiles; p.fd_rowop = row_op;
    return launch_dft2d_fwd_fd(p, (hipStream_t)stream);
}

int uno_dft2d_forward_bf16(const void* images, float* spec, int n_img, int H, int W, int m1, int m2, float scale,
                           int hermitian_cols, int mask_overlap, void* stream) {
    return dft2d(false, static_cast<const float*>(images), spec, n_img, H, W, m1, m2, scale, hermitian_cols, mask_overlap,
                 (hipStream_t)stream, 0, 0, 0, 1);
}

int uno_dft2d_inverse_bf16(const float* spec, void* images, int n_img, int H, int W, int m1, int m2, float scale,
                           int hermitian_cols, int mask_overlap, void* stream) {
    return dft2d(true, spec, static_cast<float*>(images), n_img, H, W, m1, m2, scale, hermitian_cols, mask_overlap,
                 (hipStream_t)stream, 0, 0, 0, 1);
}

int uno_dft2d_forward_grouped(const float* images, float* spec, int n_img, int H, int W, int m1, int m2, float scale,
                              int hermitian_cols, int mask_overlap, int group, int stride, int offset, void* stream) {
    if (group < 1) { set_error("uno_dft2d_forward_grouped: group must be positive"); return -1; }
    return dft2d(false, images, spec, n_img, H, W, m1, m2, scale, hermitian_cols, mask_overlap, (hipStream_t)stream, group, stride, offset);
}

int uno_dft2d_forward_grouped_bf16(const void* images, float* spec, int n_img, int H, int W, int m1, int m2, float scale,
                                   int hermitian_cols, int mask_overlap, int group, int stride, int offset, void* stream) {
    if (group < 1) { set_error("uno_dft2d_forward_grouped_bf16: group must be positive"); return -1; }
    return dft2d(false, static_cast<const float*>(images), spec, n_img, H, W, m1, m2, scale, hermitian_cols, mask_overlap,
                 (hipStream_t)stream, group, stride, offset, 1);
}

int uno_dft2d_inverse_grouped_bf16(const float* spec, void* images, int n_img, int H, int W, int m1, int m2, float scale,
                                   int hermitian_cols, int mask_overlap, int group, int stride, int offset, void* stream) {
    if (group < 1) { set_error("uno_dft2d_inverse_grouped_bf16: group must be positive"); return -1; }
    return dft2d(true, spec, static_cast<float*>(images), n_img, H, W, m1, m2, scale, hermitian_cols, mask_overlap,
                 (hipStream_t)stream, group, stride, offset, 1);
}

int uno_dft2d_inverse_grouped(const float* spec, float* images, int n_img, int H, int W, int m1, int m2, float scale,
                              int hermitian_cols, int mask_overlap, int group, int stride, int offset, void* stream) {
    if (group < 1) { set_error("uno_dft2d_inverse_grouped: group must be positive"); return -1; }
    return dft2d(true, spec, images, n_img, H, W, m1, m2, scale, hermitian_cols, mask_overlap, (hipStream_t)stream, group, stride, offset);
}

static int mode_mix_impl(const float* in, const float* const* w, float* out, int op, int B, int Ci, int Co, int ncorner,
                         int modes_per_corner, void* stream, int w_half) {
    if (!w || (B > 0 && (!in || !out))) { set_error("uno_mode_mix: null pointer"); return -1; }
    if (op != 0 && op != 1) { set_error("uno_mode_mix: op must be 0 or 1"); return -1; }
    if (ncorner < 1 || ncorner > 4) { set_error("uno_mode_mix: ncorner=%d out of range", ncorner); return -1; }
    for (int c = 0; c < ncorner; ++c)
        if (!w[c]) { set_error("uno_mode_mix: null weight pointer %d", c); return -1; }
    return mode_gemm(op, reinterpret_cast<const float2*>(in), reinterpret_cast<const float2* const*>(w), nullptr,
                     reinterpret_cast<float2*>(out), nullptr, B, Ci, Co, ncorner, modes_per_corner, (hipStream_t)stream, w_half);
}

int uno_mode_mix(const float* in, const float* const* w, float* out, int op, int B, int Ci, int Co, int ncorner,
                 int modes_per_corner, void* stream) {
    return mode_mix_impl(in, w, out, op, B, Ci, Co, ncorner, modes_per_corner, stream, 0);
}

int uno_mode_mix_f16w(const float* in, const void* const* w, float* out, int op, int B, int Ci, int Co, int ncorner,
                      int modes_per_corner, void* stream) {
    return mode_mix_impl(in, reinterpret_cast<const float* const*>(w), out, op, B, Ci, Co, ncorner, modes_per_corner, stream, 1);
}

static int mode_wgrad_impl(const float* xtrunc, const float* go, float* const* gw, int B, int Ci, int Co, int ncorner,
                           int modes_per_corner, int accumulate, void* stream) {
    if (!gw || (B > 0 && (!xtrunc || !go))) { set_error("uno_mode_wgrad: null pointer"); return -1; }
    if (ncorner < 1 || ncorner > 4) { set_error("uno_mode_wgrad: ncorner=%d out of range", ncorner); return -1; }
    for (int c = 0; c < ncorner; ++c)
        if (!gw[c]) { set_error("uno_mode_wgrad: null output pointer %d", c); return -1; }
    return mode_gemm(2, reinterpret_cast<const float2*>(xtrunc), nullptr, reinterpret_cast<const float2*>(go), nullptr,
                     reinterpret_cast<float2* const*>(gw), B, Ci, Co, ncorner, modes_per_corner, (hipStream_t)stream, 0, accumulate);
}

int uno_mode_wgrad(const float* xtrunc, const float* go, float* const* gw, int B, int Ci, int Co, int ncorner,
                   int modes_per_corner, void* stream) {
    return mode_wgrad_impl(xtrunc, go, gw, B, Ci, Co, ncorner, modes_per_corner, 0, stream);
}

int uno_mode_backward(const float* xtrunc, const float* go, const float* const* w, float* gx_spec, float* const* gw, int B, int Ci, int Co,
                      int ncorner, int modes_per_corner, int accumulate, void* stream) {
    if (!w || !gw || (B > 0 && (!xtrunc || !go || !gx_spec))) { set_error("uno_mode_backward: null pointer"); return -1; }
    if (ncorner < 1 || ncorner > 4) { set_error("uno_mode_backward: ncorner=%d out of range", ncorner); return -1; }
    for (int c = 0; c < ncorner; ++c)
        if (!w[c] || !gw[c]) { set_error("uno_mode_backward: null weight / gradient pointer %d", c); return -1; }
    return mode_backward(reinterpret_cast<const float2*>(xtrunc), reinterpret_cast<const float2*>(go), reinterpret_cast<const float2* const*>(w),
                         reinterpret_cast<float2*>(gx_spec), reinterpret_cast<float2* const*>(gw), B, Ci, Co, ncorner, modes_per_corner,
                         (hipStream_t)stream, accumulate);
}

int uno_mode_wgrad_acc(const float* xtrunc, const float* go, float* const* gw, int B, int Ci, int Co, int ncorner,
                       int modes_per_corner, int accumulate, void* stream) {
    return mode_wgrad_impl(xtrunc, go, gw, B, Ci, Co, ncorner, modes_per_corner, accumulate, stream);
}

int uno_cdft_axis(const float* in, float* out, int inverse, int n_img, int H, int m1, int m2, int m3, float scale,
                  int mask_overlap, void* stream) {
    if (n_img < 0 || H < 1 || m1 < 1 || m1 > H || m2 < 1 || m3 < 1) {
        set_error("uno_cdft_axis: bad sizes n_img=%d H=%d modes=(%d,%d,%d)", n_img, H, m1, m2, m3);
        return -1;
    }
    if (n_img == 0) return 0;
    if (!in || !out) { set_error("uno_cdft_axis: null pointer"); return -1; }
    CdftParams p;
    p.in = in; p.out = out; p.n_img = n_img; p.H = H; p.C = 2 * m2 * m3; p.m1 = m1; p.m2 = m2; p.m3 = m3;
    p.scale = scale; p.mask = mask_overlap ? 1 : 0;
    p.tw = twiddle_table(H);
    if (!p.tw) return -6;
    if (m1 > 40) return launch_cdft_generic(p, inverse != 0, (hipStream_t)stream);
    return launch_cdft(p, inverse != 0, (hipStream_t)stream);
}

long long uno_fft_resample3d_ws_bytes(int n_vol, int D1, int M1, int J1, int J2, int m3) {
    const long long C = (long long)J2 * m3;
    return 8LL * n_vol * ((long long)D1 * C + (long long)M1 * C + (long long)J1 * C);
}

static int fft_resample3d_impl(const float* x, float* y, void* ws, int n_vol, int D1, int D2, int D3, int M1, int M2, int M3,
                               int J1, const int* f1_in, const int* f1_out, int J2, const int* f2_in, const int* f2_out, int m3,
                               float scale, int herm_in, int herm_out, int accumulate, float* act_out, void* stream) {
    const char* who = "uno_fft_resample3d";
    if (n_vol < 0 || D1 < 1 || D2 < 1 || D3 < 1 || M1 < 1 || M2 < 1 || M3 < 1) { set_error("%s: bad sizes", who); return -1; }
    if (J1 < 2 || (J1 & 1) || J2 < 2 || (J2 & 1) || J1 > 80 || J2 > 48 || m3 < 1 || m3 > D3 / 2 + 1 || m3 > M3 / 2 + 1) {
        set_error("%s: row counts must be even (J1=%d <= 80, J2=%d <= 48) and 1 <= modes3=%d <= n/2+1", who, J1, J2, m3);
        return -1;
    }
    if (n_vol == 0) return 0;
    if (!x || !y || !ws || !f1_in || !f1_out || !f2_in || !f2_out) { set_error("%s: null pointer", who); return -1; }
    hipStream_t s = (hipStream_t)stream;
    const long long C = (long long)J2 * m3;
    float* Z1 = static_cast<float*>(ws);
    float* Z2 = Z1 + 2LL * n_vol * D1 * C;
    float* S = Z2 + 2LL * n_vol * M1 * C;
    Dft2dParams p;
    p.n_img = n_vol * D1; p.H = D2; p.W = D3; p.m1 = J2 / 2; p.m2 = m3; p.herm = herm_in ? 1 : 0;
    p.sp_group = p.n_img; p.sp_stride = 0;
    p.in = x; p.out = Z1; p.rowfreq = f2_in;
    p.twH = twiddle_table(D2); p.twW = twiddle_table(D3);
    if (!p.twH || !p.twW) return -6;
    if (!dft2d_fwd_plane_applies(p)) { set_error("%s: input planes %d x %d (%d of them) are outside the plane-batched kernels' range", who, D2, D3, p.n_img); return -2; }
    if (int rc = launch_dft2d_fwd_plane(p, s)) return rc;
    CdftParams c;
    c.n_img = n_vol; c.C = (int)C; c.m1 = J1 / 2; c.m2 = J2 / 2; c.m3 = m3;
    c.in = Z1; c.out = S; c.H = D1; c.rowfreq = f1_in; c.tw = twiddle_table(D1);
    if (!c.tw) return -6;
    if (int rc = launch_cdft(c, false, s)) return rc;
    c.in = S; c.out = Z2; c.H = M1; c.rowfreq = f1_out; c.tw = twiddle_table(M1);
    if (!c.tw) return -6;
    if (int rc = launch_cdft(c, true, s)) return rc;
    p.n_img = n_vol * M1; p.H = M2; p.W = M3; p.scale = scale; p.herm = herm_out ? 1 : 0;
    p.sp_group = p.n_img;
    p.in = Z2; p.out = y; p.rowfreq = f2_out;
    p.twH = twiddle_table(M2); p.twW = twiddle_table(M3);
    if (!p.twH || !p.twW) return -6;
    if (!dft2d_inv_plane_applies(p)) { set_error("%s: output planes %d x %d (%d of them) are outside the plane-batched kernels' range", who, M2, M3, p.n_img); return -2; }
    p.accumulate = accumulate ? 1 : 0; p.act_out = act_out;
// ... 268 lines not shown
```

uno_amd/csrc/dft2d_fwd_fd.hip:

```cpp
#include "dft2d_fwd_fd_kernel.h"

namespace uno {

static bool fd_class(const Dft2dParams& p, int* NT, int* MT, int* R4) {
    if (p.m1 < 1 || p.m2 < 1 || p.m1 > 40 || p.m2 > 48) return false;
    *NT = (p.m2 + 15) / 16; *MT = (2 * p.m1 + 15) / 16;
    const int rem = p.m2 - 16 * (*NT - 1);
    if (rem > 8) return false;
    *R4 = (rem + 3) / 4;
    return (*NT == 2 && *MT == 3 && *R4 == 1) || (*NT == 1 && *MT == 1 && (*R4 == 1 || *R4 == 2));
}

bool dft2d_fwd_fd_applies(const Dft2dParams& p) {
    int NT, MT, R4;
    FwdFtGeometry g;
    return fd_class(p, &NT, &MT, &R4) && fwd_fd_geometry(p, NT, MT, R4, &g);
}

int launch_dft2d_fwd_fd(const Dft2dParams& p, hipStream_t s) {
    int NT, MT, R4;
    FwdFtGeometry g;
    if (!fd_class(p, &NT, &MT, &R4) || !fwd_fd_geometry(p, NT, MT, R4, &g)) { set_error("dft2d_fwd_fd: the form does not apply"); return -3; }
    if (NT == 2) return launch_fwd_fd<2, 3, 1>(p, g, s);
    return R4 == 1 ? launch_fwd_fd<1, 1, 1>(p, g, s) : launch_fwd_fd<1, 1, 2>(p, g, s);
}

}
```

uno_amd/csrc/dft2d_fwd_fd_kernel.h:

```cpp
#pragma once
#include "dft2d_fwd_common.h"
#include "dft2d_fwd_ft_kernel.h"

namespace uno {

constexpr int FD_NC = 13;
constexpr int FD_KT = 10;
constexpr int FD_CE = 4;
constexpr int FD_WR = (FD_NC * 16 + 63) / 64;
#ifndef UNO_FD_KO
#define UNO_FD_KO 0
#endif
constexpr int FD_MINW = 416, FD_MAXW = 447;

template <int NT, int MT, int R4>
__global__ __launch_bounds__(256) void dft2d_fwd_fd_kernel(Dft2dParams p) {
    constexpr int NTF = R4 > 0 ? NT - 1 : NT;
    constexpr int NQ = R4 > 0 ? R4 : 1;
    constexpr int NTFA = NTF > 0 ? NTF : 1;
    extern __shared__ __attribute__((aligned(16))) char smem[];
    const int H = p.H, W = p.W, m1 = p.m1, m2 = p.m2;
    const int Ho = p.fd_Ho, Wo = p.fd_Wo;
    const int tid = threadIdx.x;
    const int nthreads = blockDim.x;
    const int NWT = nthreads >> 6;
    const int wave = __builtin_amdgcn_readfirstlane(tid >> 6);
    const int lane = tid & 63;
    const int r16 = lane & 15;
    const int kk = lane >> 4;
    const unsigned H8 = 8u * H;
    UNO_FWD_COLUMN_PAIRS(W);
    const int nk = 4 * nfull + tailsteps;

    const int tile_stride = (16 * W + 32 + 3) & ~3;
    float* sTile = reinterpret_cast<float*>(smem);
    float2* sTabF = reinterpret_cast<float2*>(sTile + (size_t)NWT * tile_stride);
    const int nka = UNO_FWD_TABLE_STEPS(nfull);
    float2* sTab4 = sTabF + (size_t)nka * NTF * 64;
    float2* sTwH = sTab4 + (size_t)nka * R4 * 16;
    int* sTailW = reinterpret_cast<int*>(sTwH + H);

    const int image = sweep_x(p.rev) * NWT + wave;
    const bool active = image < p.n_img;
    const int nrt = (H + 15) >> 4;
    float* buf = sTile + (size_t)wave * tile_stride;

    int a0;
    const __amdgpu_buffer_rsrc_t rsrc = image_rsrc(p.in, p.n_img, H, W, active ? image : 0, &a0);
    auto request_tile = [&](int rt) {
        const int toff = a0 + rt * 16 * W;
        const int rows = min(16, H - 16 * rt);
        const int total = (toff & 31) + rows * W;
        const int npiece = (total + 255) >> 8;
        const unsigned v0 = (unsigned)(((toff & ~31) + 4 * lane) * 4);
        for (int i = 0; i < npiece; ++i)
            if (256 * i + 4 * lane < total)
                __builtin_amdgcn_raw_ptr_buffer_load_lds(rsrc, (lds_ptr_t)(buf + 256 * i), 16, v0 + 1024u * (unsigned)i, 0, 0, FT_AUX);
    };
    if (active) request_tile(0);

    for (int n = tid; n < H; n += nthreads) sTwH[n] = p.twH[n];
    for (int e = tid; e < FWD_TAILMAX * 64; e += nthreads) { UNO_FWD_PUT_TAIL_COLUMNS(e); }
    UNO_FWD_BUILD_OPERAND_TABLES();

    int sc[FD_CE];
    float wc[FD_CE][FD_KT];
    {
        const int KW = p.fd_KW;
#pragma unroll
        for (int e = 0; e < FD_CE; ++e) {
            const int j = min(64 * e + lane, Wo - 1);
            const int s = p.fd_startW[j];
            sc[e] = max(min(s - (lane >> 5), W - FD_KT), 0);
            const int d = s - sc[e];
#pragma unroll
            for (int t = 0; t < FD_KT; ++t) {
                const int u = t - d;
                const bool in = u >= 0 && u < KW && s + u < W;
                const float wv = p.fd_wtW[(size_t)j * KW + min(max(u, 0), KW - 1)];
                wc[e][t] = in ? wv : 0.f;
            }
        }
    }
    __syncthreads();

    UNO_FWD_ACCUMULATORS(false, MT);

    const float2* tabF = sTabF + lane;
    const float2* tab4 = sTab4 + 4 * kk + (lane & 3);

    float C[FD_NC][FD_CE];
#pragma unroll
    for (int c = 0; c < FD_NC; ++c)
#pragma unroll
        for (int e = 0; e < FD_CE; ++e) C[c][e] = 0.f;

    if (active) {
        float* const oimg = p.fd_out + (size_t)image * Ho * Wo;
        int pend_ibase = 0, pend_ncomp = 0;
        auto flush_rows = [&]() {
#pragma unroll
            for (int c = 0; c < FD_NC; ++c) {
                if (c < pend_ncomp && (unsigned)(pend_ibase + c) < (unsigned)Ho && !(UNO_FD_KO & 4)) {
                    float* orow = oimg + (size_t)(pend_ibase + c) * Wo;
#pragma unroll
                    for (int e = 0; e < FD_CE; ++e)
                        if (64 * e + lane < Wo) orow[64 * e + lane] = C[c][e];
                }
            }
#pragma unroll
            for (int n = 1; n < 16; n *= 2) {
                if (pend_ncomp & n) {
#pragma unroll
                    for (int c = 0; c < FD_NC; ++c)
#pragma unroll
                        for (int e = 0; e < FD_CE; ++e) C[c][e] = (c + n < FD_NC) ? C[(c + n < FD_NC) ? c + n : 0][e] : 0.f;
                }
            }
        };
        for (int rt = 0; rt < nrt; ++rt) {
            const int toff = a0 + rt * 16 * W;
            const int phase = toff & 31;
            const int rows = min(16, H - 16 * rt);
            const float* row = buf + phase + r16 * W;
            asm volatile("s_waitcnt vmcnt(0)" ::: "memory");
            flush_rows();
            if (rows < 16) {
                for (int i = phase + rows * W + lane; i < phase + 16 * W; i += 64) buf[i] = 0.f;
            }
            const float* wd = p.fd_rowop + (size_t)rt * (FD_NC * 16);
            float wv[FD_WR];
#pragma unroll
            for (int k = 0; k < FD_WR; ++k) wv[k] = wd[min(64 * k + lane, FD_NC * 16 - 1)];
            int tinfo = p.fd_tiles[4 * rt + (lane & 3)];

            f32x4 Tr[NT], Tn[NT];
            f32x4 Qr[NQ], Qn[NQ];
#pragma unroll
            for (int t = 0; t < NT; ++t) { Tr[t] = f32x4{0, 0, 0, 0}; Tn[t] = f32x4{0, 0, 0, 0}; }
#pragma unroll
            for (int g = 0; g < NQ; ++g) { Qr[g] = f32x4{0, 0, 0, 0}; Qn[g] = f32x4{0, 0, 0, 0}; }
#define UNO_FD_MFMA(E_, D_, TWF_, TW4_)                                                   \
    do {                                                                                  \
        _Pragma("unroll") for (int t = 0; t < NTF; ++t) {                                 \
            Tr[t] = mfma16((E_), (TWF_)[t].x, Tr[t]);                                     \
            Tn[t] = mfma16((D_), (TWF_)[t].y, Tn[t]);                                     \
        }                                                                                 \
        _Pragma("unroll") for (int g = 0; g < R4; ++g) {                                  \
            Qr[g] = mfma4((E_), (TW4_)[g].x, Qr[g]);                                   \
            Qn[g] = mfma4((D_), (TW4_)[g].y, Qn[g]);                                   \
        }                                                                                 \
    } while (0)

            struct RowOps { float xl[4], xr[4]; float2 twF[4][NTFA], tw4[4][NQ]; };
            RowOps opA, opB;
            const float* pl = row + 1 + 4 * kk;
            const float* pr = row + W - 4 - 4 * kk;
            auto load_ops = [&](RowOps& o, int c) {
                const int cn = min(c, max(nfull - 1, 0));
                const float2* tf = tabF + (size_t)(4 * c) * (NTF * 64);
                const float2* t4 = tab4 + (size_t)(4 * c) * (R4 * 16);
#pragma unroll
                for (int s = 0; s < 4; ++s) {
                    o.xl[s] = pl[16 * cn + s]; o.xr[s] = pr[-16 * cn + s];
#pragma unroll
                    for (int t = 0; t < NTF; ++t) o.twF[s][t] = tf[(s * NTF + t) * 64];
#pragma unroll
                    for (int g = 0; g < R4; ++g) o.tw4[s][g] = t4[(s * R4 + g) * 16];
                }
            };
            auto chunk = [&](RowOps& cur, RowOps& nxt, int c) {
                load_ops(nxt, c + 1);
                __builtin_amdgcn_sched_barrier(0);
#pragma unroll
                for (int s = 0; s < 4; ++s) {
                    const float E = cur.xl[s] + cur.xr[3 - s];
                    const float D = cur.xl[s] - cur.xr[3 - s];
                    UNO_FD_MFMA(E, D, cur.twF[s], cur.tw4[s]);
                }
                __builtin_amdgcn_sched_barrier(0);
            };
            load_ops(opA, 0);
            {
                int c = 0;
                for (; c + 2 <= nfull; c += 2) { chunk(opA, opB, c); chunk(opB, opA, c + 1); }
                if (c < nfull) { chunk(opA, opB, c); opA = opB; }
            }
            float2 (&twF)[4][NTFA] = opA.twF;
            float2 (&tw4)[4][NQ] = opA.tw4;
            {
                const float2* tf = tabF + (size_t)(4 * nfull) * (NTF * 64);
                const float2* t4 = tab4 + (size_t)(4 * nfull) * (R4 * 16);
                float TL[FWD_TAILMAX], TR[FWD_TAILMAX];
#pragma unroll
                for (int s = 0; s < FWD_TAILMAX; ++s) {
                    const int wl = sTailW[(s * 2 + 0) * 64 + lane], wr = sTailW[(s * 2 + 1) * 64 + lane];
                    const float vl = row[max(wl, 0)], vr = row[max(wr, 0)];
                    TL[s] = wl >= 0 ? vl : 0.f; TR[s] = wr >= 0 ? vr : 0.f;
                }
                float2 twF5[NTFA], tw45[NQ];
#pragma unroll
                for (int t = 0; t < NTF; ++t) twF5[t] = tf[(4 * NTF + t) * 64];
#pragma unroll
                for (int g = 0; g < R4; ++g) tw45[g] = t4[(4 * R4 + g) * 16];
#pragma unroll
                for (int s = 0; s < FWD_TAILMAX; ++s) {
                    if (s < tailsteps) {
                        const float E = TL[s] + TR[s];
                        const float D = TL[s] - TR[s];
                        if (s < 4) UNO_FD_MFMA(E, D, twF[s], tw4[s]);
                        else UNO_FD_MFMA(E, D, twF5, tw45);
                    }
                }
            }
#undef UNO_FD_MFMA

            float Y[16][FD_CE];
            {
                const float* trow = buf + phase;
                float xv[2][FD_CE][FD_KT];
                auto read_row = [&](float (&x)[FD_CE][FD_KT], int r) {
#pragma unroll
                    for (int e = 0; e < FD_CE; ++e) {
                        const float* q = trow + r * W + sc[e];
#pragma unroll
                        for (int t = 0; t < FD_KT; ++t) x[e][t] = q[t];
                    }
                };
                if (!(UNO_FD_KO & 1)) read_row(xv[0], 0);
#pragma unroll
                for (int r = 0; r < 16; ++r) {
                    if (UNO_FD_KO & 1) { for (int e = 0; e < FD_CE; ++e) Y[r][e] = 0.f; continue; }
                    if (r + 1 < 16) read_row(xv[(r + 1) & 1], r + 1);
                    __builtin_amdgcn_sched_barrier(0);
#pragma unroll
                    for (int e = 0; e < FD_CE; ++e) {
                        float acc = 0.f;
#pragma unroll
                        for (int t = 0; t < FD_KT; ++t) acc = fmaf(wc[e][t], xv[r & 1][e][t], acc);
                        asm volatile("" : "+v"(acc));
                        Y[r][e] = acc;
                    }
                    __builtin_amdgcn_sched_barrier(0);
                }
            }
#pragma unroll
            for (int k = 0; k < FD_WR; ++k) asm volatile("" : "+v"(wv[k]));
            asm volatile("" : "+v"(tinfo));
            asm volatile("s_waitcnt lgkmcnt(0)" ::: "memory");
            if (rt + 1 < nrt) request_tile(rt + 1);

            const int ibase = __builtin_amdgcn_readlane(tinfo, 0);
            const int ncomp = __builtin_amdgcn_readlane(tinfo, 1);
            const unsigned mlo = (unsigned)__builtin_amdgcn_readlane(tinfo, 2);
            const unsigned mhi = (unsigned)__builtin_amdgcn_readlane(tinfo, 3);
#pragma unroll
            for (int c = 0; c < FD_NC; ++c) {
#pragma unroll
                for (int q4 = 0; q4 < 4; ++q4) {
                    const int b = 4 * c + q4;
                    const unsigned bit = b < 32 ? (mlo >> (b & 31)) & 1u : (mhi >> ((b - 32) & 31)) & 1u;
                    if (bit && !(UNO_FD_KO & 2)) {
#pragma unroll
                        for (int r = 4 * q4; r < 4 * q4 + 4; ++r) {
                            const float w = __int_as_float(__builtin_amdgcn_readlane(__float_as_int(wv[(c * 16 + r) >> 6]), (c * 16 + r) & 63));
#pragma unroll
                            for (int e = 0; e < FD_CE; ++e) C[c][e] = fmaf(w, Y[r][e], C[c][e]);
                        }
                    }
                }
            }
            pend_ibase = ibase;
            pend_ncomp = ncomp;

            UNO_FWD_REGROUP_4X4();
            UNO_FWD_STAGE_B(false, MT);
        }
        flush_rows();
    }

    if (active) UNO_FWD_STORE_SPECTRUM(false, MT, image);
}

static bool fwd_fd_geometry(const Dft2dParams& p, int NT, int MT, int R4, FwdFtGeometry* out) {
    (void)MT;
    const int NTF = R4 > 0 ? NT - 1 : NT;
    if (p.bf16 || p.rowfreq || p.W < FD_MINW || p.W > FD_MAXW) return false;
    if (p.fd_Ho < 1 || p.fd_Wo < 1 || p.fd_Wo > 64 * FD_CE || p.fd_KW < 1 || p.fd_KW > FD_KT - 1) return false;
    if ((long long)p.fd_Ho * p.fd_Wo > 0x7fffffffLL / 4) return false;
    const int cus = ft_device_cu_count();
    int g = 4;
    while (g > 1 && (long long)(p.n_img + g - 1) / g < cus) --g;
    while (g > 1 && fwd_ft_lds_bytes(p, NTF, R4, g) > FT_LDS_BUDGET) --g;
    const size_t lds = fwd_ft_lds_bytes(p, NTF, R4, g);
    if (lds > FT_LDS_BUDGET) return false;
    *out = FwdFtGeometry{1, g, lds};
    return true;
}

template <int NT, int MT, int R4>
static int launch_fwd_fd(Dft2dParams p, const FwdFtGeometry& g, hipStream_t s) {
    auto K = dft2d_fwd_fd_kernel<NT, MT, R4>;
    static int lds_slot[64];
    if (!ensure_dynamic_lds(reinterpret_cast<const void*>(K), g.lds, lds_slot)) { set_error("dft2d_fwd_fd: cannot raise dynamic LDS to %zu", g.lds); return -4; }
    char name[64];
    snprintf(name, sizeof(name), "uno::dft2d_fwd_fd_kernel<%d, %d, %d>", NT, MT, R4);
    p.nw = 1;
    p.rev = fwd_ft_sweep();
    {
        ProfScope prof(name, (double)p.n_img * ((double)p.H * p.W * 4.0 + (double)p.fd_Ho * p.fd_Wo * 4.0 + 2.0 * p.m1 * p.m2 * 8.0), s);
        hipLaunchKernelGGL(K, dim3((p.n_img + g.g - 1) / g.g), dim3(64 * g.g), g.lds, s, p);
    }
    const hipError_t e = hipGetLastError();
    if (e != hipSuccess) { set_error("dft2d_fwd_fd launch: %s", hipGetErrorString(e)); return -5; }
    return 0;
}

}
```

uno_amd/csrc/uno_common.h:

```cpp
#pragma once
#include <hip/hip_runtime.h>
#include <stdint.h>

namespace uno {

typedef float f32x4 __attribute__((ext_vector_type(4)));

__device__ __forceinline__ f32x4 mfma16(float a, float b, f32x4 c) {
    return __builtin_amdgcn_mfma_f32_16x16x4f32(a, b, c, 0, 0, 0);
}

__device__ __forceinline__ float uno_erf(float x) {
    x = __builtin_fminf(__builtin_fmaxf(x, -4.f), 4.f);
    const float t = x * x;
    float p = -2.72614225801306e-10f;
    p = fmaf(p, t, 2.77068142495902e-08f);
    p = fmaf(p, t, -2.10102402082508e-06f);
    p = fmaf(p, t, -5.69250639462346e-05f);
    p = fmaf(p, t, -7.34990630326855e-04f);
    p = fmaf(p, t, -2.95459980854025e-03f);
    p = fmaf(p, t, -1.60960333262415e-02f);
    p *= x;
    float q = -1.45660718464996e-05f;
    q = fmaf(q, t, -2.13374055278905e-04f);
// ... 66 lines not shown
__device__ __forceinline__ void io_store4(float* dst, float a, float b, float c, float d) {
    *reinterpret_cast<f4u*>(dst) = f4u{{a, b, c, d}};
}
__device__ __forceinline__ void io_store4(unsigned short* dst, float a, float b, float c, float d) {
    struct __attribute__((packed, aligned(2))) h4w { unsigned w[2]; };
    *reinterpret_cast<h4w*>(dst) = h4w{{bf16_pack2(a, b), bf16_pack2(c, d)}};
}
__device__ __forceinline__ void io_store8(unsigned short* dst, const f32x4& a, const f32x4& b) {
    *reinterpret_cast<h8u*>(dst) = h8u{{bf16_pack2(a[0], a[1]), bf16_pack2(a[2], a[3]), bf16_pack2(b[0], b[1]), bf16_pack2(b[2], b[3])}};
}
__device__ __forceinline__ float4 io_ld4(const float* p) {
    const f4u v = *reinterpret_cast<const f4u*>(p);
    return make_float4(v.v[0], v.v[1], v.v[2], v.v[3]);
}
__device__ __forceinline__ float4 io_ld4(const unsigned short* p) {
    const h4u v = *reinterpret_cast<const h4u*>(p);
    return make_float4(io_widen(v.v[0]), io_widen(v.v[1]), io_widen(v.v[2]), io_widen(v.v[3]));
}
__device__ __forceinline__ void io_store1(float* dst, float a) { *dst = a; }
__device__ __forceinline__ void io_store1(unsigned short* dst, float a) { *dst = bf16_rne(a); }

__device__ __forceinline__ float2 lds_tw(const float2* tab, unsigned byte_off) {
    return *reinterpret_cast<const float2*>(reinterpret_cast<const char*>(tab) + byte_off);
}

__device__ __forceinline__ float herm_weight(int l, int N) {
    return (l == 0 || 2 * l == N) ? 1.0f : 2.0f;
}

__host__ __device__ __forceinline__ int corner_freq(int j, int m, int N) { return j < m ? j : N - 2 * m + j; }

__host__ __device__ __forceinline__ bool row_survives(int j, int m, int N) { return j >= m || j < N - m; }

inline int pick_waves_per_image(int n_row_tiles) {
    int best = 1, best_waste = 1 << 30;
    for (int nw = 4; nw >= 1; --nw) {
        if (nw > n_row_tiles) continue;
        const int per = (n_row_tiles + nw - 1) / nw;
        const int waste = (per * nw - n_row_tiles) * 12 / nw;
        if (waste < best_waste) { best_waste = waste; best = nw; }
    }
    return best;
}

__device__ __forceinline__ int sweep_x(int rev) { return rev ? (int)(gridDim.x - 1 - blockIdx.x) : (int)blockIdx.x; }
__device__ __forceinline__ int sweep_y(int rev) { return rev ? (int)(gridDim.y - 1 - blockIdx.y) : (int)blockIdx.y; }

struct Dft2dParams {
    const float* in = nullptr;
    float* out = nullptr;
    const float2* twH = nullptr;
    const float2* twW = nullptr;
    int n_img = 0, H = 0, W = 0, m1 = 0, m2 = 0;
    float scale = 1.f;
    int herm = 0;
    int mask = 0;
    int sp_group = 1, sp_stride = 1, sp_offset = 0;
    int bf16 = 0;
    const int* rowfreq = nullptr;
    int nw = 1;
    int exp = 0;
    int accumulate = 0;
    float* act_out = nullptr;
    int rev = 0;
    const float* add_src = nullptr;
    int add_Hs = 0, add_Ws = 0;
    const int* add_p0 = nullptr;
    const float* add_rowop = nullptr;
    const int* add_v0 = nullptr;
    const float* add_colop = nullptr;
    float* fd_out = nullptr;
    int fd_Ho = 0, fd_Wo = 0, fd_KW = 0;
    const int* fd_startW = nullptr;
    const float* fd_wtW = nullptr;
    const int* fd_tiles = nullptr;
    const float* fd_rowop = nullptr;
};

__device__ __forceinline__ size_t spectrum_index(const Dft2dParams& p, int img) {
    return (size_t)(img / p.sp_group) * p.sp_stride + p.sp_offset + img % p.sp_group;
}

struct ModeOperand {
    const float2* base[4];
    long long s0, s1;
    int conj;
    int half;
};
struct ModeGemmParams {
    ModeOperand A, B;
    float2* out[4];
    long long o_sm, o_sn;
    int M, N, K, ncorner, Mc;
    int accumulate;
};

struct CdftParams {
    const float* in = nullptr;
    float* out = nullptr;
    const float2* tw = nullptr;
    int n_img = 0, H = 0, C = 0, m1 = 0, m2 = 0, m3 = 0;
    float scale = 1.f;
    int mask = 0;
    const int* rowfreq = nullptr;
};

struct Vol3dParams {
    const float* in = nullptr;
    float* out = nullptr;
    const float2* tw1 = nullptr;
    const float2* tw2 = nullptr;
    const float2* tw3 = nullptr;
    int n_vol = 0, D1 = 0, D2 = 0, D3 = 0, m1 = 0, m2 = 0, m3 = 0;
    float scale = 1.f;
    int herm = 0;
    const float* ctab = nullptr;
};

const float2* twiddle_table(int N);
void* upload_table(const void* host, size_t bytes);
float2 twiddle_value(long long n, int N);

inline bool ensure_dynamic_lds(const void* kernel, size_t bytes, int* slot) {
    if (bytes <= 64 * 1024) return true;
    int dev = 0;
    if (hipGetDevice(&dev) != hipSuccess || dev < 0 || dev >= 64) dev = 0;
    if ((size_t)__atomic_load_n(&slot[dev], __ATOMIC_RELAXED) >= bytes) return true;
    const int want = 160 * 1024;
    if (hipFuncSetAttribute(kernel, hipFuncAttributeMaxDynamicSharedMemorySize, want) != hipSuccess) return false;
    __atomic_store_n(&slot[dev], want, __ATOMIC_RELAXED);
    return true;
}
void set_error(const char* fmt, ...);
struct Scratch { void* ptr; size_t bytes; };
const Scratch& thread_scratch();
int reserved_cus();
int next_sweep_reversed(int family);
enum { SWEEP_K1 = 1, SWEEP_K3 = 2, SWEEP_K7 = 4, SWEEP_K8 = 8, SWEEP_K9 = 16, SWEEP_NORM = 32, SWEEP_PROJ = 64, SWEEP_LIFT = 128 };
inline int usable_cus(int device_cus) { const int r = reserved_cus(); return device_cus - r >= 8 ? device_cus - r : (device_cus < 8 ? device_cus : 8); }

struct ProfScope {
    int slot;
    hipStream_t stream;
    ProfScope(const char* name, double bytes, hipStream_t s);
    ~ProfScope();
};

int launch_dft2d_fwd(const Dft2dParams& p, hipStream_t s);
int launch_dft2d_inv(const Dft2dParams& p, hipStream_t s);
bool dft2d_inv_add_applies(const Dft2dParams& p);
int launch_dft2d_inv_add(const Dft2dParams& p, hipStream_t s);
bool dft2d_fwd_fd_applies(const Dft2dParams& p);
int launch_dft2d_fwd_fd(const Dft2dParams& p, hipStream_t s);
bool dft2d_fwd_plane_applies(const Dft2dParams& p);
bool dft2d_inv_plane_applies(const Dft2dParams& p);
bool dft2d_b16_applies(const Dft2dParams& p);
int launch_dft2d_fwd_b16(const Dft2dParams& p, hipStream_t s);
int launch_dft2d_inv_b16(const Dft2dParams& p, hipStream_t s);
int launch_dft2d_fwd_plane(const Dft2dParams& p, hipStream_t s);
int launch_dft2d_inv_plane(const Dft2dParams& p, hipStream_t s);
bool vol3d_fwd_applies(int n_vol, int D1, int D2, int D3, int m1, int m2, int m3);
bool vol3d_inv_applies(int n_vol, int D1, int D2, int D3, int m1, int m2, int m3);
int launch_dft3d_fwd_volume(const Vol3dParams& p, hipStream_t s);
int launch_dft3d_inv_volume(const Vol3dParams& p, hipStream_t s);
int launch_mode_gemm(const ModeGemmParams& p, hipStream_t s);
int launch_mode_gemm_pair(const ModeGemmParams& input_grad, const ModeGemmParams& weight_grad, hipStream_t s);
int launch_cdft(const CdftParams& p, bool inverse, hipStream_t s);
int launch_dft2d_generic(const Dft2dParams& p, bool inverse, void* ws, size_t ws_bytes, hipStream_t s);
int launch_cdft_generic(const CdftParams& p, bool inverse, hipStream_t s);
int launch_resample3d_any(const float* x, float* y, float* y_act, int accumulate, void* ws, int n_vol, int D1, int D2, int D3, int M1, int M2, int M3, int J1,
                          const int* f1_in, const int* f1_out, int J2, const int* f2_in, const int* f2_out, int m3, float scale,
                          int herm_in, int herm_out, hipStream_t s);
int launch_resample2d(const void* in, void* out, float* tmp, int n_img, int H, int W, int Ho, int Wo, const int* startH,
                      const float* wtH, int KH, const int* startW, const float* wtW, int KW, const int* tile_p0,
                      const float* tile_w, int NP, int accumulate, int bf16, hipStream_t s);
struct ChannelMixArgs {
    const void* x; const void* x2; const float* w; const float* bias; void* y; void* y2; void* y_act; const void* dgelu_of;
    const float* proj_w; const float* proj_b; void* proj_out;
    int B, Ci, Co, C1, Co1; long long P; int transpose_w, accumulate, act_in, bf16;
    PixelWindow win;
    void* ws = nullptr; size_t ws_bytes = 0;
    const float* vh_x = nullptr; const float* vh_w = nullptr; const float* vh_b = nullptr; int vh_ci = 0, vh_mode = 0;
    const void* gmul = nullptr;
    const float* pb_w2 = nullptr; const float* pb_g = nullptr;
    int act_cols = 0, act_pitch = 0; long long act_plane = 0;
};
int launch_clear_border(float* t, long long n_planes, int Hp, int Wp, int rows, int cols, hipStream_t s);
int launch_channel_mix2(const ChannelMixArgs& a, hipStream_t s);
int launch_channel_mix(const void* x, const float* w, const float* bias, void* y, int B, int Ci, int Co, long long P,
                       int transpose_w, int accumulate, int act_in, const void* dgelu_of, int bf16, hipStream_t s, void* ws = nullptr,
                       size_t ws_bytes = 0);
long long channel_mix_ws_bytes(int Ci, int Co, long long P, int bf16);
int launch_adam_multi(int n_tensors, float* const* p, const float* const* g, float* const* m, float* const* v, const long long* n,
                      const int* is_complex, double lr, double beta1, double beta2, double eps, double wd, int step, hipStream_t s,
                      const float* dev_scalars = nullptr);
int launch_adam_advance(int* step, float* scalars, const double* hyper, double lr, double eps, double wd, double beta1, double beta2,
                        hipStream_t s);
int launch_adam(float* p, const float* g, float* m, float* v, long long n, int is_complex, double lr, double beta1, double beta2,
                double eps, double wd, int step, hipStream_t s);
struct GeluProjectSecond { const void* s = nullptr; void* gs = nullptr; int C1 = 0, act = 0; };
int launch_gelu_project_fwd(const void* pre, const float* w, const float* bias, void* out, int B, int C, long long P, int bf16, hipStream_t s,
                            const GeluProjectSecond* two = nullptr);
long long gelu_project_ws_floats(int B, int C, long long P);
int launch_gelu_project_bwd(const void* pre, const float* w, const void* gout, void* gpre, float* gw, float* gb, float* ws, int B,
                            int C, long long P, int bf16, hipStream_t s, const PixelWindow& win = PixelWindow(),
                            const GeluProjectSecond* two = nullptr);
int launch_gelu_pad(const void* s, const void* gy, void* out, int n_img, int H, int W, int Hp, int Wp, int backward, int bf16, hipStream_t st);
int launch_transpose_batched(const float* in, float* out, int B, long long R, int C, long long ld_in, long long sb_in, long long ld_out,
                             long long sb_out, hipStream_t st);
int launch_instnorm_fwd(const void* x, const float* gamma, const float* beta, void* y, float* mean, float* rstd, long long rows, int C,
                        long long N, float eps, int gelu, int bf16, hipStream_t s);
int launch_instnorm_bwd(const void* x, const void* gy, const float* gamma, const float* beta, const float* mean, const float* rstd,
                        void* gx, float* s1, float* s2, long long rows, int C, long long N, int gelu, int bf16, hipStream_t s);
long long channel_wgrad_ws_floats(int B, int Ci, int Co, long long P, int* nsplit_out);
int launch_channel_wgrad(const void* gy, const void* x, float* gw, float* gb, float* ws, int B, int Ci, int Co, long long P,
                         int act_x, int bf16, hipStream_t s);
struct WgradProjectedBack { const float* w2 = nullptr; const float* g = nullptr; float* gw2 = nullptr; float* gb2 = nullptr; };
bool channel_wgrad_pb_applies(int B, int Ci, int Co, int C1, long long P);
long long channel_wgrad_pb_ws_floats(int B, int Ci, int Co, long long P);
int launch_channel_wgrad2(const void* gy, const void* x, const void* x2, int C1, float* gw, float* gb, float* ws, int B, int Ci, int Co,
                          long long P, int act_x, int accumulate, int bf16, hipStream_t s, const PixelWindow& win = PixelWindow(),
                          const WgradProjectedBack& pb = WgradProjectedBack());
int launch_channel_wgrad_vh(const void* gy, const float* vh_x, const float* vh_w, const float* vh_b, int vh_ci, float* gw, float* gb, float* ws,
                            int B, int Ci, int Co, long long P, int act_x, hipStream_t s, int accumulate = 0);
bool lift_bwd_fused_applies(int Cin, int Cm, int Co, int W, long long P);
long long lift_bwd_fused_parts(int B, int H, int W);
int launch_lift_forward_fused(const float* x, const float* w1, const float* b1, const float* w0, const float* b0, float* act, int B, int Cin,
                              int H, int W, int Hp, int Wp, hipStream_t s);
int launch_lift_backward_fused(const float* x, const float* w1, const float* b1, const float* w0, const float* b0, const float* g, float* part,
                               float* part1, int B, int Cin, int H, int W, int Hp, int Wp, hipStream_t s, const float* g2 = nullptr);
int launch_channel_wgrad_finish(const float* parts, float* gw, float* gb, int Ci, int Co, long long nparts, int accumulate, hipStream_t s);
long long rel_l2_steps_chunks(long long P, int T, long long* chunk_pixels);
long long rel_l2_steps_ws_floats(int B, long long P, int T);
int launch_rel_l2_steps(const float* pred, const float* target, float* sums, float* rel, float* totals, float* ws, int B, long long P, int T,
                        hipStream_t s);
int launch_rel_l2_steps_finish(const float* ws, float* sums, float* rel, float* totals, int B, int T, long long nc, hipStream_t s);
long long rollout_chunks(long long P, long long* chunk_pixels);
long long rollout_ws_floats(int B, long long P, int T);
int launch_rollout_advance(float* window, const float* frame, const float* target, float* pred, float* ws, int B, int C, int T_in, long long P,
                           int T, int t, int shift, hipStream_t s);
long long rollout_lift_bwd_ws_floats(int B, int C, int Cm, long long P, int T);
int launch_rollout_lift(const float* given, const float* pred, const float* feat, const float* w, const float* bias, float* h, int B, int T_in,
                        int F, int Cm, long long P, int T, int t, hipStream_t s);
int launch_rollout_lift_backward(const float* gh, const float* given, const float* pred, const float* target, const float* feat, const float* w,
                                 const float* sums, const float* gL, float* gpred, float* gframe, float* parts, int B, int T_in, int F, int Cm,
                                 long long P, int T, int t, hipStream_t s);
int launch_rollout_loss_seed(const float* pred, const float* target, const float* sums, const float* gL, float* gframe, int B, long long P, int T,
                             hipStream_t s);

}
```

uno_amd/harness/models.py:

```python
from __future__ import annotations

import math

import torch
import torch.nn as nn
import torch.nn.functional as F

from ..integral_operators import (GradJoin, OperatorBlock_2D, OperatorBlock_3D, channel_mix, channel_mix_cat, channel_mix_cat_project,
                                  enable_native_resample3d_any, enable_one_buffer_any_grid, gelu_channel_mix, gelu_channel_mix_pad, gelu_pad2d, gelu_project, gelu_project2,
                                  lift_gelu_pad)


def _block_cat(block, xs, *dims):
    if hasattr(block, "forward_cat"):
        return block.forward_cat(xs, *dims)
    return block(torch.cat(list(xs), dim=1), *dims)


def _cached(cache: dict, key, build):
    grid = cache.get(key)
    if grid is None:
        grid = build()
        cache.clear()
        cache[key] = grid
    return grid


class UNO_9(nn.Module):

    def __init__(self, in_width, width, pad=5, factor=1, block_cls=OperatorBlock_2D):
        super().__init__()
        self.in_width = in_width
        self.width = width
        self.padding = pad
        w, f = width, factor
        self.fc_n1 = nn.Linear(in_width, w // 2)
        self.fc0 = nn.Linear(w // 2, w)
        self.conv0 = block_cls(w, 2 * f * w, 40, 40, 18, 18)
        self.conv1 = block_cls(2 * f * w, 4 * f * w, 20, 20, 8, 8, Normalize=True)
        self.conv2 = block_cls(4 * f * w, 4 * f * w, 20, 20, 8, 8)
        self.conv4 = block_cls(4 * f * w, 2 * f * w, 40, 40, 8, 8, Normalize=True)
        self.conv5 = block_cls(4 * f * w, w, 85, 85, 18, 18)
        self.fc1 = nn.Linear(2 * w, w)
        self.fc2 = nn.Linear(w, 1)
        self._grid_cache = {}

    def get_grid(self, shape, device):
        def build():
            b, sx, sy = shape[0], shape[1], shape[2]
            gx = torch.linspace(0, 1, sx, dtype=torch.float64).to(torch.float32).reshape(1, sx, 1, 1).expand(b, sx, sy, 1)
            gy = torch.linspace(0, 1, sy, dtype=torch.float64).to(torch.float32).reshape(1, 1, sy, 1).expand(b, sx, sy, 1)
            return torch.cat((gx, gy), dim=-1).contiguous().to(device)
        return _cached(self._grid_cache, (tuple(shape[:3]), str(device)), build)

    def forward(self, x):
        S1, S2 = x.shape[1], x.shape[2]
        x = torch.cat((x, self.get_grid(x.shape, x.device).to(x.dtype)), dim=-1).permute(0, 3, 1, 2).contiguous()
        scale = math.ceil(S2 / 85)
        margin = scale * self.padding
        product = hasattr(self.conv5, "forward_cat")
        fused = product and self.conv5.non_lin and not self.conv5.normalize
        jl = GradJoin() if fused else None
        lifted = lift_gelu_pad(x, self.fc_n1, self.fc0, margin, margin, grad_join=jl)
        d1, d2 = lifted.shape[-2], lifted.shape[-1]

        if fused:
            jc, j2 = GradJoin(), GradJoin()
            c0 = self.conv0(lifted, d1 // 2, d2 // 2, join=jl, out_join=jc)
            c1 = self.conv1(c0, d1 // 4, d2 // 4, join=jc)
            c2 = self.conv2(c1, d1 // 4, d2 // 4, out_join=j2)
            skip5 = [self.conv4(c2, d1 // 2, d2 // 2, join=j2), c0]
            out = channel_mix_cat_project([self.conv5.forward_cat(skip5, d1, d2, defer_gelu=True, defer_grad=jc), lifted], self.fc1.weight,
                                          self.fc1.bias, self.fc2.weight, self.fc2.bias, gelu_first=True, defer_grad=jl, crop=(S1, S2))
            return out[:, :, :S1, :S2].permute(0, 2, 3, 1).contiguous()
        else:
            c0 = self.conv0(lifted, d1 // 2, d2 // 2)
            c1 = self.conv1(c0, d1 // 4, d2 // 4)
            c2 = self.conv2(c1, d1 // 4, d2 // 4)
            skip5 = [self.conv4(c2, d1 // 2, d2 // 2), c0]
            c5 = channel_mix_cat([_block_cat(self.conv5, skip5, d1, d2), lifted], self.fc1.weight, self.fc1.bias)
        out = gelu_project(c5, self.fc2.weight, self.fc2.bias)
        return out[:, :, :S1, :S2].permute(0, 2, 3, 1).contiguous()


class UNO(nn.Module):

    _BLOCKS = ((48, 48, 22, 22), (32, 32, 14, 14), (16, 16, 6, 6), (16, 16, 6, 6), (32, 32, 6, 6), (48, 48, 14, 14), (64, 64, 22, 22))
    _LIFT = None
    _FC1 = 4
    _TWO_SOURCE = False

    def __init__(self, in_width, width, pad=0, factor=3 / 4, block_cls=OperatorBlock_2D):
        super().__init__()
        self.in_width, self.width, self.factor, self.padding = in_width, width, factor, pad
        w, f = width, factor
        lift = w // 2 if self._LIFT is None else self._LIFT
        self.fc = nn.Linear(in_width, lift)
        self.fc0 = nn.Linear(lift, w)
        cin = (w, 2 * f * w, 4 * f * w, 8 * f * w, 8 * f * w, 8 * f * w, 4 * f * w)
        cout = (2 * f * w, 4 * f * w, 8 * f * w, 8 * f * w, 4 * f * w, 2 * f * w, w)
        for i, row in enumerate(self._BLOCKS):
            setattr(self, f"L{i}", block_cls(cin[i], cout[i], *row))
        self.fc1 = nn.Linear(2 * w, self._FC1 * w)
        self.fc2 = nn.Linear(self._FC1 * w + (lift if self._TWO_SOURCE else 0), 1)
        self._grid_cache = {}

    def get_grid(self, shape, device):
        def build():
            b, sx, sy = shape[0], shape[1], shape[2]
            gx = torch.linspace(0, 2 * math.pi, sx, dtype=torch.float64).to(torch.float32).reshape(1, sx, 1, 1).expand(b, sx, sy, 1)
            gy = torch.linspace(0, 2 * math.pi, sy, dtype=torch.float64).to(torch.float32).reshape(1, 1, sy, 1).expand(b, sx, sy, 1)
            return torch.cat((torch.sin(gx), torch.sin(gy), torch.cos(gx), torch.cos(gy)), dim=-1).contiguous().to(device)
        return _cached(self._grid_cache, (tuple(shape[:3]), str(device)), build)

    def _grids(self, d1, d2):
        a, b, c = (int(d1 * self.factor), int(d2 * self.factor)), (d1 // 2, d2 // 2), (d1 // 4, d2 // 4)
        return a, b, c, c, b, a, (d1, d2)

    def forward(self, x):
        z = torch.cat((x.permute(0, 3, 1, 2), self.get_grid(x.shape, x.device).permute(0, 3, 1, 2)), dim=1)
        return self.forward_cf(z).permute(0, 2, 3, 1).contiguous()

    def forward_cf(self, x):
        return self.body_cf(channel_mix(x, self.fc.weight, self.fc.bias))

    def body_cf(self, h):
        lifted = F.gelu(gelu_channel_mix(h, self.fc0.weight, self.fc0.bias))
        p = self.padding
        if p != 0:
            lifted = F.pad(lifted, [p, p, p, p])
        g = self._grids(lifted.shape[-2], lifted.shape[-1])
        c0 = self.L0(lifted, *g[0])
        c1 = self.L1(c0, *g[1])
        if hasattr(self.L6, "forward_cat") and all(b.non_lin and not b.normalize for b in (self.L2, self.L3)):
            j2, j3 = GradJoin(), GradJoin()
            c2 = self.L2(c1, *g[2], out_join=j2)
            c3 = self.L3(c2, *g[3], join=j2, out_join=j3)
            c4 = self.L4(c3, *g[4], join=j3)
        else:
            c4 = self.L4(self.L3(self.L2(c1, *g[2]), *g[3]), *g[4])
        c4 = torch.cat([c4, c1], dim=1)
        c5 = torch.cat([self.L5(c4, *g[5]), c0], dim=1)
        c6 = torch.cat([self.L6(c5, *g[6]), lifted], dim=1)
        if p != 0:
            c6 = c6[..., p:-p, p:-p] if self._TWO_SOURCE else c6[..., :-p, :-p]
        out = channel_mix(c6.contiguous(), self.fc1.weight, self.fc1.bias)
        if self._TWO_SOURCE:
            return gelu_project2(out, h, self.fc2.weight, self.fc2.bias, act2=True)
        return gelu_project(out, self.fc2.weight, self.fc2.bias)


class UNO_P(UNO):

    _BLOCKS = ((32, 32, 14, 14), (16, 16, 6, 6), (8, 8, 3, 3), (8, 8, 3, 3), (16, 16, 3, 3), (32, 32, 6, 6), (64, 64, 14, 14))
    _FC1, _TWO_SOURCE = 3, True
    _DIV = (2, 4, 8, 8, 4, 2, 1)

    def __init__(self, in_width, width, pad=0, factor=1, block_cls=OperatorBlock_2D):
        super().__init__(in_width, width, pad, factor, block_cls)

    def _grids(self, d1, d2):
        return [(d1 // k, d2 // k) for k in self._DIV]


class UNO_S256(UNO_P):

    _BLOCKS = ((64, 64, 32, 33), (16, 16, 8, 9), (8, 8, 4, 5), (8, 8, 4, 5), (16, 16, 4, 5), (64, 64, 8, 9), (256, 256, 32, 32))
    _LIFT = 16
    _DIV = (4, 16, 32, 32, 16, 4, 1)


def _grids3d(d1, d2, bottom, times):
    a, b, c = (int(3 * d1 / 4), int(3 * d2 / 4)), (d1 // 2, d2 // 2), (d1 // 4, d2 // 4)
    return [(*s, t) for s, t in zip((a, b, c, bottom, b, a, (d1, d2)), times)]


class Uno3D_T20(nn.Module):

    _NAMES = ("conv0", "conv1", "conv2", "conv3", "conv6", "conv7", "conv8")
    _BLOCKS = ((48, 48, 10, 22, 22, 5), (32, 32, 10, 14, 14, 5), (16, 16, 12, 6, 6, 5), (16, 16, 12, 6, 6, 6), (32, 32, 18, 6, 6, 6),
               (48, 48, 20, 14, 14, 8), (64, 64, 20, 22, 22, 8))

    @staticmethod
    def _lift_width(in_width, width):
        return in_width * 2

    @staticmethod
    def _plan(d1, d2, d3, padding):
        return _grids3d(d1, d2, (d1 // 4, d2 // 4), (d3, d3, int(d3 * 1.2), int(d3 * 1.2), int(d3 * 1.8), int(2.0 * d3), 2 * d3)), 2 * padding

    def __init__(self, in_width, width, pad=2, factor=1, pad_both=False, block_cls=OperatorBlock_3D):
        super().__init__()
        self.in_width, self.width, self.pad, self.pad_both = in_width, width, pad, pad_both
        w, f = width, factor
        lift = self._lift_width(in_width, w)
        self.fc = nn.Linear(in_width, lift)
        self.fc0 = nn.Linear(lift, w)
        cin = (w, 2 * f * w, 4 * f * w, 8 * f * w, 16 * f * w, 8 * f * w, 4 * f * w)
        cout = (2 * f * w, 4 * f * w, 8 * f * w, 16 * f * w, 4 * f * w, 2 * f * w, 2 * w)
        for i, (name, row) in enumerate(zip(self._NAMES, self._BLOCKS)):
            setattr(self, name, block_cls(cin[i], cout[i], *row, Normalize=name in ("conv0", "conv3", "conv7")))
        self.fc1 = nn.Linear(3 * w, 4 * w)
        self.fc2 = nn.Linear(4 * w, 1)
        self._grid_cache = {}

    def get_grid(self, shape, device):
        def build():
            b, sx, sy, sz = shape[0], shape[1], shape[2], shape[3]
            lin = lambda hi, n: torch.linspace(0, hi, n, dtype=torch.float64).to(torch.float32)
            gx = lin(2 * math.pi, sx).reshape(1, sx, 1, 1, 1).expand(b, sx, sy, sz, 1)
            gy = lin(2 * math.pi, sy).reshape(1, 1, sy, 1, 1).expand(b, sx, sy, sz, 1)
            gz = lin(1, sz).reshape(1, 1, 1, sz, 1).expand(b, sx, sy, sz, 1)
            return torch.cat((torch.sin(gx), torch.sin(gy), torch.cos(gx), torch.cos(gy), gz), dim=-1).contiguous().to(device)
        return _cached(self._grid_cache, (tuple(shape[:4]), str(device)), build)

    @staticmethod
    def _resize(t, like):
        from ..resample import resample3d_trilinear
        return resample3d_trilinear(t, tuple(like.shape[2:]))

    def forward(self, x):
        x = torch.cat((x, self.get_grid(x.shape, x.device)), dim=-1).permute(0, 4, 1, 2, 3).contiguous()
        lifted = F.gelu(gelu_channel_mix(channel_mix(x, self.fc.weight, self.fc.bias), self.fc0.weight, self.fc0.bias))
        self.padding = int(self.pad * 0.1 * lifted.shape[-1])
        lifted = F.pad(lifted, [self.padding, self.padding, 0, 0, 0, 0] if self.pad_both else [0, self.padding, 0, 0, 0, 0])
# ... 58 lines not shown
```

uno_amd/integral_operators.py:

```python
from __future__ import annotations

import torch
import torch.nn as nn
import torch.nn.functional as F

from ._param_grads import release_pass_state
from .block2d import _OperatorBlock2dCatFn, _OperatorBlock2dFn, _SpectralConv2dFn, spectral_conv2d, spectral_conv2d_mixed
from .pointwise import (GradJoin, _dev_act, channel_mix, channel_mix_cat, channel_mix_cat_project, gelu_channel_mix, gelu_channel_mix_pad,
                        gelu_pad2d, gelu_project, gelu_project2, instance_norm_gelu, lift_gelu_pad)
from .resample import resample2d_bicubic_aa
from .spectral3d import (_FftResample3dAnyFn, _FftResample3dFn, _OperatorBlock3dFn, _resample3d_plan, _resample3d_plan_any, spectral_conv3d)

__all__ = [
    "enable_mixed_precision", "enable_native_resample3d_any", "enable_one_buffer_any_grid", "GradJoin", "channel_mix_cat_project", "release_pass_state",
    "SpectralConv1d_Uno", "pointwise_op_1D", "OperatorBlock_1D",
    "SpectralConv2d_Uno", "pointwise_op_2D", "OperatorBlock_2D",
    "SpectralConv3d_Uno", "pointwise_op_3D", "OperatorBlock_3D",
]


def enable_mixed_precision(module: nn.Module, enabled: bool = True) -> nn.Module:
    for m in module.modules():
        if isinstance(m, SpectralConv2d_Uno):
            m.mixed_precision = bool(enabled)
    return module


def _check_input(x: torch.Tensor, ndim: int, channels: int, who: str):
    if x.dim() != ndim:
        raise RuntimeError(f"{who}: expected a {ndim}-D tensor (batch, channels, *grid), got shape {tuple(x.shape)}")
    if x.shape[1] != channels:
        raise RuntimeError(f"{who}: expected {channels} input channels, got {x.shape[1]}")
    if x.dtype != torch.float32:
        raise RuntimeError(f"{who}: input must be float32 (got {x.dtype})")


class SpectralConv2d_Uno(nn.Module):

    def __init__(self, in_codim, out_codim, dim1, dim2, modes1=None, modes2=None):
        super().__init__()
        in_codim, out_codim = int(in_codim), int(out_codim)
        self.in_channels = in_codim
        self.out_channels = out_codim
        self.dim1 = dim1
        self.dim2 = dim2
        if modes1 is not None:
            self.modes1, self.modes2 = modes1, modes2
        else:
            self.modes1, self.modes2 = dim1 // 2 - 1, dim2 // 2
        self.scale = (1 / (2 * in_codim)) ** (1.0 / 2.0)
        shape = (in_codim, out_codim, self.modes1, self.modes2)
        self.weights1 = nn.Parameter(self.scale * torch.randn(*shape, dtype=torch.cfloat))
        self.weights2 = nn.Parameter(self.scale * torch.randn(*shape, dtype=torch.cfloat))
        self.mixed_precision = False

    def forward(self, x, dim1=None, dim2=None):
        if dim1 is not None:
            self.dim1 = dim1
            self.dim2 = dim2
        if self.mixed_precision and x.dtype == torch.bfloat16 and x.dim() == 4 and x.shape[1] == self.in_channels:
            if not self._bf16_kernels():
                return spectral_conv2d(x.float(), self.weights1, self.weights2, self.dim1, self.dim2).to(torch.bfloat16)
            return _SpectralConv2dFn.apply(x, self.weights1, self.weights2, self.dim1, self.dim2, True)
        _check_input(x, 4, self.in_channels, "SpectralConv2d_Uno")
        return spectral_conv2d(x, self.weights1, self.weights2, self.dim1, self.dim2)

    def _bf16_kernels(self):
        return self.modes1 <= 40 and self.modes2 <= 48


class pointwise_op_2D(nn.Module):

    def __init__(self, in_codim, out_codim, dim1, dim2):
        super().__init__()
        self.conv = nn.Conv2d(int(in_codim), int(out_codim), 1)
        self.dim1 = int(dim1)
        self.dim2 = int(dim2)

    def forward(self, x, dim1=None, dim2=None):
        if dim1 is None:
            dim1, dim2 = self.dim1, self.dim2
        if not (_dev_act(x) and x.dim() == 4):
            return F.interpolate(self.conv(x), size=(dim1, dim2), mode="bicubic", align_corners=True, antialias=True)
        if dim1 * dim2 < x.shape[-2] * x.shape[-1]:
            return channel_mix(resample2d_bicubic_aa(x, dim1, dim2), self.conv.weight, self.conv.bias)
        return resample2d_bicubic_aa(channel_mix(x.contiguous(), self.conv.weight, self.conv.bias), dim1, dim2)


class OperatorBlock_2D(nn.Module):

    def __init__(self, in_codim, out_codim, dim1, dim2, modes1, modes2, Normalize=False, Non_Lin=True):
        super().__init__()
        self.conv = SpectralConv2d_Uno(in_codim, out_codim, dim1, dim2, modes1, modes2)
        self.w = pointwise_op_2D(in_codim, out_codim, dim1, dim2)
        self.normalize = Normalize
        self.non_lin = Non_Lin
        if Normalize:
            self.normalize_layer = nn.InstanceNorm2d(int(out_codim), affine=True)

    def forward(self, x, dim1=None, dim2=None, *, join=None, out_join=None):
        if self.non_lin and not self.normalize:
            return self._branches(x, dim1, dim2, gelu=True, join=join, out_join=out_join)
        if out_join is not None:
            out_join.void()
        out = self._branches(x, dim1, dim2, join=join)
        if self.normalize:
            return instance_norm_gelu(out, self.normalize_layer, self.non_lin)
        return out

    def forward_cat(self, xs, dim1=None, dim2=None, defer_gelu=False, defer_grad=None):
        if defer_gelu and (self.normalize or not self.non_lin):
            raise ValueError("defer_gelu needs a block with Non_Lin=True and Normalize=False")
        xs = list(xs)
        conv, w = self.conv, self.w
        d1, d2 = (dim1, dim2) if dim1 is not None else (w.dim1, w.dim2)
        cdims = (dim1, dim2) if dim1 is not None else (conv.dim1, conv.dim2)
        fused = (len(xs) == 2 and all(self._takes(x) for x in xs) and xs[0].dtype == xs[1].dtype
                 and xs[0].shape[0] == xs[1].shape[0] and xs[0].shape[2:] == xs[1].shape[2:]
                 and xs[0].shape[1] + xs[1].shape[1] == conv.in_channels and cdims == (d1, d2)
                 and w.conv.weight.dtype == torch.float32)
        if not fused:
            if defer_grad is not None:
                defer_grad.void()
            if defer_gelu:
                return self._branches(torch.cat(xs, dim=1), dim1, dim2)
            return self.forward(torch.cat(xs, dim=1), dim1, dim2)
        if dim1 is not None:
            conv.dim1, conv.dim2 = dim1, dim2
        out = _OperatorBlock2dCatFn.apply(xs[0], xs[1], conv.weights1, conv.weights2, w.conv.weight, w.conv.bias, int(d1), int(d2),
                                          xs[0].dtype == torch.bfloat16, defer_grad)
        if defer_gelu:
            return out
        if self.normalize:
            return instance_norm_gelu(out, self.normalize_layer, self.non_lin)
        return F.gelu(out) if self.non_lin else out

    def _branches(self, x, dim1, dim2, gelu=False, join=None, out_join=None):
        conv, w = self.conv, self.w
        if dim1 is not None:
            conv.dim1, conv.dim2 = dim1, dim2
            d1, d2 = dim1, dim2
        else:
            d1, d2 = w.dim1, w.dim2
        fused = (self._takes(x) and (conv.dim1, conv.dim2) == (d1, d2)
                 and x.shape[1] == conv.in_channels and w.conv.weight.dtype == torch.float32)
        if not fused:
            for j in (join, out_join):
                if j is not None:
                    j.void()
            out = conv(x) + w(x, d1, d2)
            return F.gelu(out) if gelu else out
        return _OperatorBlock2dFn.apply(x, conv.weights1, conv.weights2, w.conv.weight, w.conv.bias, int(d1), int(d2),
                                        x.dtype == torch.bfloat16, bool(gelu), join, out_join)

    def _takes(self, x):
        return (x.is_cuda and x.dim() == 4 and
                (x.dtype == torch.float32 or (x.dtype == torch.bfloat16 and getattr(self.conv, "mixed_precision", False)
                                              and self.conv._bf16_kernels())))


class SpectralConv3d_Uno(nn.Module):

    def __init__(self, in_codim, out_codim, dim1, dim2, dim3, modes1=None, modes2=None, modes3=None):
        super().__init__()
        in_codim, out_codim = int(in_codim), int(out_codim)
        self.in_channels = in_codim
        self.out_channels = out_codim
        self.dim1, self.dim2, self.dim3 = dim1, dim2, dim3
        if modes1 is not None:
            self.modes1, self.modes2, self.modes3 = modes1, modes2, modes3
        else:
            self.modes1, self.modes2, self.modes3 = dim1, dim2, dim3 // 2 + 1
        self.scale = (1 / (2 * in_codim)) ** (1.0 / 2.0)
        shape = (in_codim, out_codim, self.modes1, self.modes2, self.modes3)
        self.weights1 = nn.Parameter(self.scale * torch.randn(*shape, dtype=torch.cfloat))
        self.weights2 = nn.Parameter(self.scale * torch.randn(*shape, dtype=torch.cfloat))
        self.weights3 = nn.Parameter(self.scale * torch.randn(*shape, dtype=torch.cfloat))
        self.weights4 = nn.Parameter(self.scale * torch.randn(*shape, dtype=torch.cfloat))

    def forward(self, x, dim1=None, dim2=None, dim3=None):
        if dim1 is not None:
            self.dim1, self.dim2, self.dim3 = dim1, dim2, dim3
        _check_input(x, 5, self.in_channels, "SpectralConv3d_Uno")
        return spectral_conv3d(x, [self.weights1, self.weights2, self.weights3, self.weights4],
                               self.dim1, self.dim2, self.dim3)


STOCK_FFT_RESAMPLE3D = False
NATIVE_RESAMPLE3D_ANY = False


def enable_native_resample3d_any(module: nn.Module, enabled: bool = True) -> nn.Module:
    for m in module.modules():
        if isinstance(m, pointwise_op_3D):
            m.native_any_grid = bool(enabled)
    return module


def _resample3d_kernels(w, din, dout, device):
    plan = _resample3d_plan(din, dout, device)
    if plan is None and (getattr(w, "native_any_grid", False) or NATIVE_RESAMPLE3D_ANY):
        plan = _resample3d_plan_any(din, dout, device)
        return plan, plan is not None
    return plan, False


class pointwise_op_3D(nn.Module):

    def __init__(self, in_codim, out_codim, dim1, dim2, dim3):
        super().__init__()
        self.conv = nn.Conv3d(int(in_codim), int(out_codim), 1)
        self.dim1, self.dim2, self.dim3 = int(dim1), int(dim2), int(dim3)

    def _corner_mask(self, spec, h1, h2, h3):
        key = (tuple(spec.shape[2:]), h1, h2, h3, str(spec.device))
        cache = self.__dict__.setdefault("_mask_cache", {})
        if key not in cache:
            m = torch.zeros((1, 1, *spec.shape[2:]), dtype=torch.float32)
            for rows in (slice(None, h1), slice(-h1, None)):
                for cols in (slice(None, h2), slice(-h2, None)):
                    m[:, :, rows, cols, :h3] = 1.0
            cache[key] = m.to(spec.device)
        return cache[key]

    def forward(self, x, dim1=None, dim2=None, dim3=None):
        if dim1 is None:
            dim1, dim2, dim3 = self.dim1, self.dim2, self.dim3
        on_device = x.is_cuda and x.dtype == torch.float32 and x.dim() == 5
        out = channel_mix(x.contiguous(), self.conv.weight, self.conv.bias) if on_device else self.conv(x)
        if on_device:
            plan, any_grid = _resample3d_kernels(self, out.shape[-3:], (dim1, dim2, dim3), out.device)
            if plan is not None:
                return (_FftResample3dAnyFn if any_grid else _FftResample3dFn).apply(out, (dim1, dim2, dim3), plan)
        if on_device and not STOCK_FFT_RESAMPLE3D:
            raise RuntimeError(
                f"pointwise_op_3D: the FFT crop / resample {tuple(out.shape[-3:])} -> {(dim1, dim2, dim3)} is outside the range of the "
                "pruned-DFT kernels (they take an even number of kept rows per complex axis - at most 80 / 48 - and (W, T) planes of at most "
                "1792 elements with T <= 64); set uno_amd.integral_operators.STOCK_FFT_RESAMPLE3D = True to run this layer's resampling "
                "through torch.fft (rocFFT) instead, or - for axis lengths of 2 ... 128 - uno_amd.integral_operators.NATIVE_RESAMPLE3D_ANY = True "
                "(enable_native_resample3d_any(model) for one model) to run it on the any-grid HIP kernels")
        spec = torch.fft.rfftn(out, dim=[-3, -2, -1])
        h1, h2, h3 = dim1 // 2, dim2 // 2, dim3 // 2
        if on_device:
            return torch.fft.irfftn(spec * self._corner_mask(spec, h1, h2, h3), s=(dim1, dim2, dim3))
        kept = torch.zeros_like(spec)
        for rows in (slice(None, h1), slice(-h1, None)):
            for cols in (slice(None, h2), slice(-h2, None)):
                kept[:, :, rows, cols, :h3] = spec[:, :, rows, cols, :h3]
        out = torch.fft.irfftn(kept, s=(dim1, dim2, dim3))
        return F.interpolate(out, size=(dim1, dim2, dim3), mode="trilinear", align_corners=True)


ONE_BUFFER_3D = True
ONE_BUFFER_3D_ANY = False


def enable_one_buffer_any_grid(module: nn.Module, enabled: bool = True) -> nn.Module:
    for m in module.modules():
        if isinstance(m, OperatorBlock_3D):
            m.one_buffer_any_grid = bool(enabled)
            if enabled:
                m.w.native_any_grid = True
    return module


class OperatorBlock_3D(nn.Module):

    def __init__(self, in_codim, out_codim, dim1, dim2, dim3, modes1, modes2, modes3, Normalize=False, Non_Lin=True):
        super().__init__()
        self.conv = SpectralConv3d_Uno(in_codim, out_codim, dim1, dim2, dim3, modes1, modes2, modes3)
        self.w = pointwise_op_3D(in_codim, out_codim, dim1, dim2, dim3)
        self.normalize = Normalize
        self.non_lin = Non_Lin
        if Normalize:
            self.normalize_layer = nn.InstanceNorm3d(int(out_codim), affine=True)

    def forward(self, x, dim1=None, dim2=None, dim3=None):
        fused = self._fused(x, dim1, dim2, dim3)
        if fused is not None:
            out, activated = fused
            if self.normalize:
                return instance_norm_gelu(out, self.normalize_layer, self.non_lin)
            return out if (activated or not self.non_lin) else F.gelu(out)
        out = self.conv(x, dim1, dim2, dim3) + self.w(x, dim1, dim2, dim3)
        if self.normalize:
            return instance_norm_gelu(out, self.normalize_layer, self.non_lin)
        if self.non_lin:
            out = F.gelu(out)
        return out

    def _fused(self, x, dim1, dim2, dim3):
        conv, w = self.conv, self.w
        if not (ONE_BUFFER_3D and x.is_cuda and x.dtype == torch.float32 and x.dim() == 5 and x.shape[1] == conv.in_channels
                and w.conv.weight.dtype == torch.float32):
            return None
        if dim1 is not None:
            dims = (int(dim1), int(dim2), int(dim3))
        else:
            dims = (int(w.dim1), int(w.dim2), int(w.dim3))
            if (conv.dim1, conv.dim2, conv.dim3) != dims:
                return None
        din = tuple(x.shape[-3:])
        plan, any_grid = _resample3d_kernels(w, din, dims, x.device)
        if plan is None or (any_grid and not (getattr(self, "one_buffer_any_grid", False) or ONE_BUFFER_3D_ANY)):
            return None
        if dim1 is not None:
# ... 63 lines not shown
```

Before: 1540 samples/s.

## Share conv1 input spectrum with conv5 skip branch via larger-mode DFT and crop

conv1 now computes the forward DFT of c0 at conv5's larger mode count, writes it into a buffer shaped for conv5's concatenated input, and crops it down to its own modes with a new spectrum_crop kernel. conv5's cat block then reuses that spectrum for the c0 channels instead of running a second DFT on the same tensor, guarded by pointer, stride and version checks. A second change adds a two-column-per-lane variant of the fused forward DFT kernel for narrower widths with two blocks per CU. The cost is a larger DFT in conv1, an extra crop kernel, a buffer held across blocks, and possibly a copy when the saved-tensor stack is active.

```diff
diff --git a/include/uno_spectral.h b/include/uno_spectral.h
--- a/include/uno_spectral.h
+++ b/include/uno_spectral.h
@@ -82,6 +82,9 @@
 int uno_dft2d_forward_resample(const float* images, float* spec, int n_img, int H, int W, int m1, int m2, float scale, int hermitian_cols,
                                int mask_overlap, int group, int stride, int offset, float* resampled, int Ho, int Wo, const int* col_start,
                                const float* col_wt, int KW, const int* row_tiles, const float* row_op, void* stream);
+
+int uno_spectrum_crop(const float* src, float* dst, int n_img, int M1, int M2, int m1, int m2, int src_group, int src_stride, int src_offset,
+                      int dst_group, int dst_stride, int dst_offset, void* stream);
 
 int uno_dft2d_forward_bf16(const void* images, float* spec, int n_img, int H, int W, int m1, int m2,
                            float scale, int hermitian_cols, int mask_overlap, void* stream);
diff --git a/uno_amd/_native.py b/uno_amd/_native.py
--- a/uno_amd/_native.py
+++ b/uno_amd/_native.py
@@ -44,6 +44,7 @@
     "uno_dft2d_inverse_add": (C.c_int, [_fp, _fp] + [_i] * 5 + [C.c_float, _i, _i, _fp, _i, _i, _fp, _fp, _fp, _fp, _fp]),
     "uno_dft2d_forward_grouped": (C.c_int, [_fp, _fp] + [_i] * 5 + [C.c_float] + [_i] * 5 + [_fp]),
     "uno_dft2d_inverse_grouped": (C.c_int, [_fp, _fp] + [_i] * 5 + [C.c_float] + [_i] * 5 + [_fp]),
+    "uno_spectrum_crop": (C.c_int, [_fp, _fp] + [_i] * 11 + [_fp]),
     "uno_mode_mix": (C.c_int, [_fp, C.POINTER(_fp), _fp] + [_i] * 6 + [_fp]),
     "uno_mode_wgrad": (C.c_int, [_fp, _fp, C.POINTER(_fp)] + [_i] * 5 + [_fp]),
     "uno_mode_backward": (C.c_int, [_fp, _fp, C.POINTER(_fp), _fp, C.POINTER(_fp)] + [_i] * 6 + [_fp]),
@@ -367,6 +368,35 @@
     return out
 
 
+def spectrum_crop(src, m1, m2, out=None, channels=None, channel_offset=0, out_channel_offset=0):
+    _require(src, torch.complex64, "src")
+    *lead, R2, M2 = src.shape
+    M1 = R2 // 2
+    if R2 != 2 * M1 or not (1 <= m1 <= M1 and 1 <= m2 <= M2):
+        raise RuntimeError(f"uno_amd: spectrum_crop of {tuple(src.shape)} to modes ({m1}, {m2}): need an even row count and 1 <= modes <= the source's")
+    sg = ss = so = dg = ds = do = 0
+    if channels is not None or out is not None:
+        if src.dim() != 4:
+            raise RuntimeError("uno_amd: spectrum_crop of a channel range needs src (B, Ctot, 2*M1, M2)")
+        C1 = src.shape[1] - channel_offset if channels is None else int(channels)
+        if channel_offset < 0 or C1 < 1 or channel_offset + C1 > src.shape[1]:
+            raise RuntimeError("uno_amd: src must hold the requested channel range")
+        lead = [src.shape[0], C1]
+        sg, ss, so = C1, src.shape[1], int(channel_offset)
+    if out is None:
+        out = torch.empty((*lead, 2 * m1, m2), dtype=torch.complex64, device=src.device)
+    else:
+        _require(out, torch.complex64, "out")
+        if out.dim() != 4 or out.shape[0] != lead[0] or tuple(out.shape[2:]) != (2 * m1, m2) or out_channel_offset < 0 \
+                or out_channel_offset + lead[1] > out.shape[1] or out.device != src.device:
+            raise RuntimeError("uno_amd: out must be (B, Cout, 2*m1, m2) with room for the channels at out_channel_offset")
+        dg, ds, do = lead[1], out.shape[1], int(out_channel_offset)
+    with torch.cuda.device(src.device):
+        rc = lib().uno_spectrum_crop(_ptr(src), _ptr(out), _count(lead), M1, M2, int(m1), int(m2), sg, ss, so, dg, ds, do, _stream(src))
+    _check(rc, "uno_spectrum_crop")
+    return out
+
+
 def reserve_cus(n: int) -> int:
     return int(lib().uno_reserve_cus(int(n)))
 
diff --git a/uno_amd/block2d.py b/uno_amd/block2d.py
--- a/uno_amd/block2d.py
+++ b/uno_amd/block2d.py
@@ -121,6 +121,58 @@
     if tabs is None or not _native.dft2d_forward_resample_applies(n, H, W, m1, m2, Ho, Wo, tabs[1].shape[1]):
         return None
     return tabs
+
+
+SHARE_FORWARD_SPECTRUM = True
+
+
+class SpectrumShare:
+
+    def __init__(self, modes, channels, channel_offset):
+        self.modes = (int(modes[0]), int(modes[1]))
+        self.channels, self.offset = int(channels), int(channel_offset)
+        self.spec = self.src = None
+
+    @classmethod
+    def for_block(cls, block, channel_offset):
+        return cls((block.conv.modes1, block.conv.modes2), block.conv.in_channels, channel_offset)
+
+    def reset(self):
+        self.spec = self.src = None
+
+    def dest(self, x, m1, m2):
+        self.reset()
+        M1, M2 = self.modes
+        H, W = x.shape[-2], x.shape[-1]
+        if not SHARE_FORWARD_SPECTRUM or x.dtype != torch.float32 or x.dim() != 4 or not x.is_cuda or m1 > M1 or m2 > M2 \
+                or M1 > H or M2 > W // 2 + 1 or self.offset < 0 or self.offset + x.shape[1] != self.channels:
+            return None
+        self.spec = torch.empty((x.shape[0], self.channels, 2 * M1, M2), dtype=torch.complex64, device=x.device)
+        self.src = (x, x._version)
+        return self.spec, M1, M2, self.offset
+
+    def take(self, x2, C1, Ci, m1, m2):
+        spec, src = self.spec, self.src
+        self.reset()
+        if spec is None or (m1, m2) != self.modes or Ci != self.channels or C1 != self.offset:
+            return None
+        x, version = src
+        if x2.data_ptr() != x.data_ptr() or x2.shape != x.shape or x2.stride() != x.stride() or x2.dtype != x.dtype or x2._version != version:
+            return None
+        return spec
+
+
+def _source_spectrum(x, xt, m1, m2, dest, rs=None, Ho=0, Wo=0):
+    H, W = x.shape[-2], x.shape[-1]
+    tgt, k1, k2, off = (xt, m1, m2, 0) if dest is None else dest
+    res = None
+    if rs is None:
+        _native.dft2d_forward(x, k1, k2, 1.0 / (H * W), out=tgt, channel_offset=off)
+    else:
+        _, res = _native.dft2d_forward_resample(x, k1, k2, Ho, Wo, rs, 1.0 / (H * W), out=tgt, channel_offset=off)
+    if dest is not None:
+        _native.spectrum_crop(tgt, m1, m2, out=xt, channels=x.shape[1], channel_offset=off)
+    return res
 
 
 def _stage_wgrad(stack, gslot, xt, gO, w1, w2, leaves, both_gw, need_gx):
@@ -171,7 +223,7 @@
 class _OperatorBlock2dFn(torch.autograd.Function):
 
     @staticmethod
-    def forward(ctx, x, w1, w2, cw, cb, Ho, Wo, half_weights=False, fuse_gelu=False, join=None, out_join=None):
+    def forward(ctx, x, w1, w2, cw, cb, Ho, Wo, half_weights=False, fuse_gelu=False, join=None, out_join=None, share=None):
         ctx.leaves = (w1, w2, cw, cb)
         ctx.join = None
         if join is not None:
@@ -183,27 +235,34 @@
         B, Ci, H, W = x.shape
         Co = cw.shape[0]
         w1, w2, cwm, cb, same, mix_last = _block_prologue(ctx, 1, x, Ci, w1, w2, cw, cb, Ho, Wo, half_weights)
+        m1, m2 = w1.shape[2], w1.shape[3]
+        dest = share.dest(x, m1, m2) if (share is not None and not half_weights and w1.dtype == torch.complex64) else None
+        k1m = (m1, m2) if dest is None else dest[1:3]
         t = fused = None
         if not mix_last and not half_weights and x.dtype == torch.float32:
             t = _native.channel_mix(x.view(B, Ci, -1), cwm, cb).view(B, Co, H, W)
-            fused = _fused_addend(t, Ho, Wo, w1.shape[2], w1.shape[3], False)
+            fused = _fused_addend(t, Ho, Wo, m1, m2, False)
         if fused is not None:
-            m1, m2 = w1.shape[2], w1.shape[3]
             xt = _xt_dest(ctx.stack, B, Ci, m1, m2, x.device)
-            _native.dft2d_forward(x, m1, m2, 1.0 / (H * W), out=xt, channel_offset=0)
+            _source_spectrum(x, xt, m1, m2, dest)
             O = _native.mode_mix(xt.view(B, Ci, 2, m1 * m2), [w1, w2], 0)
             s = _native.dft2d_inverse(O.view(B, Co, 2 * m1, m2), Ho, Wo, 1.0, True, True, addend=fused)
-        elif mix_last and not same and not half_weights and (rs := _fused_resample(x, w1.shape[2], w1.shape[3], Ho, Wo, False)) is not None:
-            m1, m2 = w1.shape[2], w1.shape[3]
+        elif mix_last and not same and not half_weights and (rs := _fused_resample(x, *k1m, Ho, Wo, False)) is not None:
             xt = _xt_dest(ctx.stack, B, Ci, m1, m2, x.device)
-            _, pre_act = _native.dft2d_forward_resample(x, m1, m2, Ho, Wo, rs, 1.0 / (H * W), out=xt, channel_offset=0)
+            pre_act = _source_spectrum(x, xt, m1, m2, dest, rs, Ho, Wo)
             O = _native.mode_mix(xt.view(B, Ci, 2, m1 * m2), [w1, w2], 0)
             s = _native.dft2d_inverse(O.view(B, Co, 2 * m1, m2), Ho, Wo, 1.0, True, True)
         else:
             pre_act = None
             if mix_last and not same:
                 pre_act = resample_forward(x, Ho, Wo)
-            s, xt = _native.spectral_conv2d_forward(x, w1, w2, Ho, Wo, xt_out=_xt_slot(ctx.stack))
+            if dest is None:
+                s, xt = _native.spectral_conv2d_forward(x, w1, w2, Ho, Wo, xt_out=_xt_slot(ctx.stack))
+            else:
+                xt = _xt_dest(ctx.stack, B, Ci, m1, m2, x.device)
+                _source_spectrum(x, xt, m1, m2, dest)
+                O = _native.mode_mix(xt.view(B, Ci, 2, m1 * m2), [w1, w2], 0)
+                s = _native.dft2d_inverse(O.view(B, Co, 2 * m1, m2), Ho, Wo, 1.0, True, True)
         out = s
         if fused is not None:
             act = x
@@ -293,13 +352,13 @@
                         gx = torch.ops.aten.gelu_backward(gx, xpre)
                     join.dgelu_applied = True
             join.reset()
-        return gx, gw1, gw2, gcw, gcb, None, None, None, None, None, None
+        return gx, gw1, gw2, gcw, gcb, None, None, None, None, None, None, None
 
 
 class _OperatorBlock2dCatFn(torch.autograd.Function):
 
     @staticmethod
-    def forward(ctx, x1, x2, w1, w2, cw, cb, Ho, Wo, half_weights=False, defer=None):
+    def forward(ctx, x1, x2, w1, w2, cw, cb, Ho, Wo, half_weights=False, defer=None, share=None):
         ctx.leaves = (w1, w2, cw, cb)
         ctx.defer = defer if (defer is not None and defer.owner and ctx.needs_input_grad[1]) else None
         x1, x2 = _plain(x1), _plain(x2)
@@ -307,9 +366,14 @@
         C2 = x2.shape[1]
         Ci, Co, m1, m2 = w1.shape
         w1, w2, cwm, cb, same, mix_last = _block_prologue(ctx, 2, x1, Ci, w1, w2, cw, cb, Ho, Wo, half_weights)
-        xt = _xt_dest(ctx.stack, B, Ci, m1, m2, x1.device)
+        shared = share.take(x2, C1, Ci, m1, m2) if (share is not None and not half_weights and x2.dtype == torch.float32
+                                                    and w1.dtype == torch.complex64) else None
+        xt = shared if (shared is not None and ctx.stack is None) else _xt_dest(ctx.stack, B, Ci, m1, m2, x1.device)
         _native.dft2d_forward(x1, m1, m2, 1.0 / (H * W), out=xt, channel_offset=0)
-        _native.dft2d_forward(x2, m1, m2, 1.0 / (H * W), out=xt, channel_offset=C1)
+        if shared is None:
+            _native.dft2d_forward(x2, m1, m2, 1.0 / (H * W), out=xt, channel_offset=C1)
+        elif shared is not xt:
+            xt[:, C1:].copy_(shared[:, C1:])
         O = _native.mode_mix(xt.view(B, Ci, 2, m1 * m2), [w1, w2], 0)
         t = fused = None
         if not mix_last and not half_weights and x1.dtype == torch.float32:
@@ -382,7 +446,7 @@
             gcw = None if gcw is None else gcw.view(cw_shape)
         if ctx.defer is not None and gx2 is not None:
             gx2 = ctx.defer.late(gx2)
-        return gx1, gx2, gw1, gw2, gcw, gcb, None, None, None, None
+        return gx1, gx2, gw1, gw2, gcw, gcb, None, None, None, None, None
 
 
 def spectral_conv2d(x, weights1, weights2, dim1, dim2):
diff --git a/uno_amd/build.py b/uno_amd/build.py
--- a/uno_amd/build.py
+++ b/uno_amd/build.py
@@ -13,7 +13,7 @@
 LIBDIR = os.path.join(HERE, "lib")
 LIB = os.path.join(LIBDIR, "libuno_spectral.so")
 STAMP = os.path.join(LIBDIR, "libuno_spectral.stamp")
-SOURCES = ["capi.hip", "capi_spectral.hip", "capi_pointwise.hip", "dft2d_fwd.hip", "dft2d_fwd_r4.hip", "dft2d_fwd_fd.hip", "dft2d_inv.hip", "dft2d_inv_b.hip", "dft2d_inv_c.hip", "dft2d_inv_add.hip", "dft2d_plane.hip", "dft2d_b16.hip", "mode_gemm.hip", "cdft_axis.hip", "dft3d_volume.hip", "dft_generic.hip", "resample3d_any.hip", "resample2d.hip", "channel_mix.hip", "channel_wgrad.hip", "adam.hip", "pointwise_fused.hip", "instnorm.hip", "lift_bwd.hip", "rel_l2_steps.hip", "rollout.hip", "rollout_train.hip"]
+SOURCES = ["capi.hip", "capi_spectral.hip", "capi_pointwise.hip", "dft2d_fwd.hip", "dft2d_fwd_r4.hip", "dft2d_fwd_fd.hip", "spectrum_crop.hip", "dft2d_inv.hip", "dft2d_inv_b.hip", "dft2d_inv_c.hip", "dft2d_inv_add.hip", "dft2d_plane.hip", "dft2d_b16.hip", "mode_gemm.hip", "cdft_axis.hip", "dft3d_volume.hip", "dft_generic.hip", "resample3d_any.hip", "resample2d.hip", "channel_mix.hip", "channel_wgrad.hip", "adam.hip", "pointwise_fused.hip", "instnorm.hip", "lift_bwd.hip", "rel_l2_steps.hip", "rollout.hip", "rollout_train.hip"]
 HEADERS = ["uno_common.h", "channel_mix_common.h", "dft2d_fwd_common.h", "dft2d_fwd_kernel.h", "dft2d_fwd_ft_kernel.h", "dft2d_fwd_ht_kernel.h", "dft2d_fwd_fd_kernel.h", "dft2d_inv_kernel.h", "dft2d_inv_add_kernel.h", os.path.join("..", "..", "include", "uno_spectral.h")]
 ARCH = "gfx950"
 FLAGS = ["-O3", "-std=c++17", "-fPIC", f"--offload-arch={ARCH}", "-fno-gpu-rdc", "-Wall", "-Wno-unused-function"]
diff --git a/uno_amd/csrc/capi_spectral.hip b/uno_amd/csrc/capi_spectral.hip
--- a/uno_amd/csrc/capi_spectral.hip
+++ b/uno_amd/csrc/capi_spectral.hip
@@ -244,6 +244,31 @@
     if (!p.twH || !p.twW) return -6;
     p.fd_out = resampled; p.fd_startW = col_start; p.fd_wtW = col_wt; p.fd_tiles = row_tiles; p.fd_rowop = row_op;
     return launch_dft2d_fwd_fd(p, (hipStream_t)stream);
+}
+
+int uno_spectrum_crop(const float* src, float* dst, int n_img, int M1, int M2, int m1, int m2, int src_group, int src_stride, int src_offset,
+                      int dst_group, int dst_stride, int dst_offset, void* stream) {
+    const char* who = "uno_spectrum_crop";
+    if (n_img < 0) { set_error("%s: negative image count", who); return -1; }
+    if (m1 < 1 || m2 < 1 || m1 > M1 || m2 > M2 || (long long)M1 * M2 > 0x7fffffffLL / 4) {
+        set_error("%s: bad mode counts (%d, %d) -> (%d, %d) (need 1 <= m1 <= M1, 1 <= m2 <= M2)", who, M1, M2, m1, m2);
+        return -1;
+    }
+    if (n_img == 0) return 0;
+    if (!src || !dst) { set_error("%s: null pointer", who); return -1; }
+    if (src == dst) { set_error("%s: dst must not alias src", who); return -1; }
+    if (src_group <= 0) { src_group = n_img; src_stride = 0; src_offset = 0; }
+    else if (src_offset < 0 || src_stride < src_offset + src_group || n_img % src_group) {
+        set_error("%s: bad source grouping (group %d, stride %d, offset %d, images %d)", who, src_group, src_stride, src_offset, n_img);
+        return -1;
+    }
+    if (dst_group <= 0) { dst_group = n_img; dst_stride = 0; dst_offset = 0; }
+    else if (dst_offset < 0 || dst_stride < dst_offset + dst_group || n_img % dst_group) {
+        set_error("%s: bad destination grouping (group %d, stride %d, offset %d, images %d)", who, dst_group, dst_stride, dst_offset, n_img);
+        return -1;
+    }
+    return launch_spectrum_crop(src, dst, n_img, M1, M2, m1, m2, src_group, src_stride, src_offset, dst_group, dst_stride, dst_offset,
+                                (hipStream_t)stream);
 }
 
 int uno_dft2d_forward_bf16(const void* images, float* spec, int n_img, int H, int W, int m1, int m2, float scale,
diff --git a/uno_amd/csrc/dft2d_fwd_fd.hip b/uno_amd/csrc/dft2d_fwd_fd.hip
--- a/uno_amd/csrc/dft2d_fwd_fd.hip
+++ b/uno_amd/csrc/dft2d_fwd_fd.hip
@@ -21,6 +21,10 @@
     int NT, MT, R4;
     FwdFtGeometry g;
     if (!fd_class(p, &NT, &MT, &R4) || !fwd_fd_geometry(p, NT, MT, R4, &g)) { set_error("dft2d_fwd_fd: the form does not apply"); return -3; }
+    if (fwd_fd_columns_per_lane(p.W) == FD_CE2) {
+        if (NT == 2) return launch_fwd_fd<2, 3, 1, FD_CE2>(p, g, s);
+        return R4 == 1 ? launch_fwd_fd<1, 1, 1, FD_CE2>(p, g, s) : launch_fwd_fd<1, 1, 2, FD_CE2>(p, g, s);
+    }
     if (NT == 2) return launch_fwd_fd<2, 3, 1>(p, g, s);
     return R4 == 1 ? launch_fwd_fd<1, 1, 1>(p, g, s) : launch_fwd_fd<1, 1, 2>(p, g, s);
 }
diff --git a/uno_amd/csrc/dft2d_fwd_fd_kernel.h b/uno_amd/csrc/dft2d_fwd_fd_kernel.h
--- a/uno_amd/csrc/dft2d_fwd_fd_kernel.h
+++ b/uno_amd/csrc/dft2d_fwd_fd_kernel.h
@@ -7,14 +7,17 @@
 constexpr int FD_NC = 13;
 constexpr int FD_KT = 10;
 constexpr int FD_CE = 4;
+constexpr int FD_CE2 = 2;
 constexpr int FD_WR = (FD_NC * 16 + 63) / 64;
 #ifndef UNO_FD_KO
 #define UNO_FD_KO 0
 #endif
 constexpr int FD_MINW = 416, FD_MAXW = 447;
-
-template <int NT, int MT, int R4>
-__global__ __launch_bounds__(256) void dft2d_fwd_fd_kernel(Dft2dParams p) {
+constexpr int FD_MINW2 = 192, FD_MAXW2 = 223;
+constexpr size_t FD_LDS_HALF = (160 * 1024) / 2 - 1024;
+
+template <int NT, int MT, int R4, int CE = FD_CE>
+__global__ __launch_bounds__(256, CE == FD_CE2 ? 2 : 1) void dft2d_fwd_fd_kernel(Dft2dParams p) {
     constexpr int NTF = R4 > 0 ? NT - 1 : NT;
     constexpr int NQ = R4 > 0 ? R4 : 1;
     constexpr int NTFA = NTF > 0 ? NTF : 1;
@@ -63,12 +66,12 @@
     for (int e = tid; e < FWD_TAILMAX * 64; e += nthreads) { UNO_FWD_PUT_TAIL_COLUMNS(e); }
     UNO_FWD_BUILD_OPERAND_TABLES();
 
-    int sc[FD_CE];
-    float wc[FD_CE][FD_KT];
+    int sc[CE];
+    float wc[CE][FD_KT];
     {
         const int KW = p.fd_KW;
 #pragma unroll
-        for (int e = 0; e < FD_CE; ++e) {
+        for (int e = 0; e < CE; ++e) {
             const int j = min(64 * e + lane, Wo - 1);
             const int s = p.fd_startW[j];
             sc[e] = max(min(s - (lane >> 5), W - FD_KT), 0);
@@ -89,11 +92,11 @@
     const float2* tabF = sTabF + lane;
     const float2* tab4 = sTab4 + 4 * kk + (lane & 3);
 
-    float C[FD_NC][FD_CE];
+    float C[FD_NC][CE];
 #pragma unroll
     for (int c = 0; c < FD_NC; ++c)
 #pragma unroll
-        for (int e = 0; e < FD_CE; ++e) C[c][e] = 0.f;
+        for (int e = 0; e < CE; ++e) C[c][e] = 0.f;
 
     if (active) {
         float* const oimg = p.fd_out + (size_t)image * Ho * Wo;
@@ -104,7 +107,7 @@
                 if (c < pend_ncomp && (unsigned)(pend_ibase + c) < (unsigned)Ho && !(UNO_FD_KO & 4)) {
                     float* orow = oimg + (size_t)(pend_ibase + c) * Wo;
 #pragma unroll
-                    for (int e = 0; e < FD_CE; ++e)
+                    for (int e = 0; e < CE; ++e)
                         if (64 * e + lane < Wo) orow[64 * e + lane] = C[c][e];
                 }
             }
@@ -114,7 +117,7 @@
 #pragma unroll
                     for (int c = 0; c < FD_NC; ++c)
 #pragma unroll
-                        for (int e = 0; e < FD_CE; ++e) C[c][e] = (c + n < FD_NC) ? C[(c + n < FD_NC) ? c + n : 0][e] : 0.f;
+                        for (int e = 0; e < CE; ++e) C[c][e] = (c + n < FD_NC) ? C[(c + n < FD_NC) ? c + n : 0][e] : 0.f;
                 }
             }
         };
@@ -215,13 +218,13 @@
             }
 #undef UNO_FD_MFMA
 
-            float Y[16][FD_CE];
+            float Y[16][CE];
             {
                 const float* trow = buf + phase;
-                float xv[2][FD_CE][FD_KT];
-                auto read_row = [&](float (&x)[FD_CE][FD_KT], int r) {
-#pragma unroll
-                    for (int e = 0; e < FD_CE; ++e) {
+                float xv[2][CE][FD_KT];
+                auto read_row = [&](float (&x)[CE][FD_KT], int r) {
+#pragma unroll
+                    for (int e = 0; e < CE; ++e) {
                         const float* q = trow + r * W + sc[e];
 #pragma unroll
                         for (int t = 0; t < FD_KT; ++t) x[e][t] = q[t];
@@ -230,11 +233,11 @@
                 if (!(UNO_FD_KO & 1)) read_row(xv[0], 0);
 #pragma unroll
                 for (int r = 0; r < 16; ++r) {
-                    if (UNO_FD_KO & 1) { for (int e = 0; e < FD_CE; ++e) Y[r][e] = 0.f; continue; }
+                    if (UNO_FD_KO & 1) { for (int e = 0; e < CE; ++e) Y[r][e] = 0.f; continue; }
                     if (r + 1 < 16) read_row(xv[(r + 1) & 1], r + 1);
                     __builtin_amdgcn_sched_barrier(0);
 #pragma unroll
-                    for (int e = 0; e < FD_CE; ++e) {
+                    for (int e = 0; e < CE; ++e) {
                         float acc = 0.f;
 #pragma unroll
                         for (int t = 0; t < FD_KT; ++t) acc = fmaf(wc[e][t], xv[r & 1][e][t], acc);
@@ -265,7 +268,7 @@
                         for (int r = 4 * q4; r < 4 * q4 + 4; ++r) {
                             const float w = __int_as_float(__builtin_amdgcn_readlane(__float_as_int(wv[(c * 16 + r) >> 6]), (c * 16 + r) & 63));
 #pragma unroll
-                            for (int e = 0; e < FD_CE; ++e) C[c][e] = fmaf(w, Y[r][e], C[c][e]);
+                            for (int e = 0; e < CE; ++e) C[c][e] = fmaf(w, Y[r][e], C[c][e]);
                         }
                     }
                 }
@@ -282,29 +285,36 @@
     if (active) UNO_FWD_STORE_SPECTRUM(false, MT, image);
 }
 
+static int fwd_fd_columns_per_lane(int W) {
+    return (W >= FD_MINW && W <= FD_MAXW) ? FD_CE : ((W >= FD_MINW2 && W <= FD_MAXW2) ? FD_CE2 : 0);
+}
+
 static bool fwd_fd_geometry(const Dft2dParams& p, int NT, int MT, int R4, FwdFtGeometry* out) {
     (void)MT;
     const int NTF = R4 > 0 ? NT - 1 : NT;
-    if (p.bf16 || p.rowfreq || p.W < FD_MINW || p.W > FD_MAXW) return false;
-    if (p.fd_Ho < 1 || p.fd_Wo < 1 || p.fd_Wo > 64 * FD_CE || p.fd_KW < 1 || p.fd_KW > FD_KT - 1) return false;
+    const int ce = fwd_fd_columns_per_lane(p.W);
+    if (p.bf16 || p.rowfreq || ce == 0) return false;
+    if (p.fd_Ho < 1 || p.fd_Wo < 1 || p.fd_Wo > 64 * ce || p.fd_KW < 1 || p.fd_KW > FD_KT - 1) return false;
     if ((long long)p.fd_Ho * p.fd_Wo > 0x7fffffffLL / 4) return false;
     const int cus = ft_device_cu_count();
+    const size_t budget = ce == FD_CE2 ? FD_LDS_HALF : FT_LDS_BUDGET;
     int g = 4;
     while (g > 1 && (long long)(p.n_img + g - 1) / g < cus) --g;
-    while (g > 1 && fwd_ft_lds_bytes(p, NTF, R4, g) > FT_LDS_BUDGET) --g;
+    while (g > 1 && fwd_ft_lds_bytes(p, NTF, R4, g) > budget) --g;
     const size_t lds = fwd_ft_lds_bytes(p, NTF, R4, g);
-    if (lds > FT_LDS_BUDGET) return false;
+    if (lds > budget) return false;
     *out = FwdFtGeometry{1, g, lds};
     return true;
 }
 
-template <int NT, int MT, int R4>
+template <int NT, int MT, int R4, int CE = FD_CE>
 static int launch_fwd_fd(Dft2dParams p, const FwdFtGeometry& g, hipStream_t s) {
-    auto K = dft2d_fwd_fd_kernel<NT, MT, R4>;
+    auto K = dft2d_fwd_fd_kernel<NT, MT, R4, CE>;
     static int lds_slot[64];
     if (!ensure_dynamic_lds(reinterpret_cast<const void*>(K), g.lds, lds_slot)) { set_error("dft2d_fwd_fd: cannot raise dynamic LDS to %zu", g.lds); return -4; }
     char name[64];
-    snprintf(name, sizeof(name), "uno::dft2d_fwd_fd_kernel<%d, %d, %d>", NT, MT, R4);
+    if constexpr (CE == FD_CE) snprintf(name, sizeof(name), "uno::dft2d_fwd_fd_kernel<%d, %d, %d>", NT, MT, R4);
+    else snprintf(name, sizeof(name), "uno::dft2d_fwd_fd_kernel<%d, %d, %d, %d>", NT, MT, R4, CE);
     p.nw = 1;
     p.rev = fwd_ft_sweep();
     {
diff --git a/uno_amd/csrc/spectrum_crop.hip b/uno_amd/csrc/spectrum_crop.hip
--- /dev/null
+++ b/uno_amd/csrc/spectrum_crop.hip
@@ -0,0 +1,45 @@
+#include "uno_common.h"
+
+namespace uno {
+
+struct SpectrumCropParams {
+    const float2* src; float2* dst;
+    long long total;
+    int M1, M2, m1, m2;
+    int s_group, s_stride, s_offset;
+    int d_group, d_stride, d_offset;
+};
+
+__global__ __launch_bounds__(256) void spectrum_crop_kernel(SpectrumCropParams p) {
+    const long long idx = (long long)blockIdx.x * 256 + threadIdx.x;
+    if (idx >= p.total) return;
+    const int per = 2 * p.m1 * p.m2;
+    const int img = (int)(idx / per);
+    const int e = (int)(idx - (long long)img * per);
+    const int r = e / p.m2, c = e - r * p.m2;
+    const int sr = r < p.m1 ? r : r + 2 * (p.M1 - p.m1);
+    const size_t si = (size_t)(img / p.s_group) * p.s_stride + p.s_offset + img % p.s_group;
+    const size_t di = (size_t)(img / p.d_group) * p.d_stride + p.d_offset + img % p.d_group;
+    p.dst[di * per + e] = p.src[(si * (2 * p.M1) + sr) * p.M2 + c];
+}
+
+int launch_spectrum_crop(const float* src, float* dst, int n_img, int M1, int M2, int m1, int m2, int s_group, int s_stride, int s_offset,
+                         int d_group, int d_stride, int d_offset, hipStream_t s) {
+    SpectrumCropParams p;
+    p.src = reinterpret_cast<const float2*>(src); p.dst = reinterpret_cast<float2*>(dst);
+    p.total = (long long)n_img * 2 * m1 * m2;
+    p.M1 = M1; p.M2 = M2; p.m1 = m1; p.m2 = m2;
+    p.s_group = s_group; p.s_stride = s_stride; p.s_offset = s_offset;
+    p.d_group = d_group; p.d_stride = d_stride; p.d_offset = d_offset;
+    const long long blocks = (p.total + 255) / 256;
+    if (blocks > 0x7fffffffLL) { set_error("spectrum_crop: %lld elements are more than one launch takes", p.total); return -1; }
+    {
+        ProfScope prof("uno::spectrum_crop_kernel", 2.0 * (double)p.total * 8.0, s);
+        hipLaunchKernelGGL(spectrum_crop_kernel, dim3((unsigned)blocks), dim3(256), 0, s, p);
+    }
+    const hipError_t e = hipGetLastError();
+    if (e != hipSuccess) { set_error("spectrum_crop launch: %s", hipGetErrorString(e)); return -5; }
+    return 0;
+}
+
+}
diff --git a/uno_amd/csrc/uno_common.h b/uno_amd/csrc/uno_common.h
--- a/uno_amd/csrc/uno_common.h
+++ b/uno_amd/csrc/uno_common.h
@@ -242,6 +242,8 @@
 int launch_dft2d_inv_add(const Dft2dParams& p, hipStream_t s);
 bool dft2d_fwd_fd_applies(const Dft2dParams& p);
 int launch_dft2d_fwd_fd(const Dft2dParams& p, hipStream_t s);
+int launch_spectrum_crop(const float* src, float* dst, int n_img, int M1, int M2, int m1, int m2, int s_group, int s_stride, int s_offset,
+                         int d_group, int d_stride, int d_offset, hipStream_t s);
 bool dft2d_fwd_plane_applies(const Dft2dParams& p);
 bool dft2d_inv_plane_applies(const Dft2dParams& p);
 bool dft2d_b16_applies(const Dft2dParams& p);
diff --git a/uno_amd/harness/models.py b/uno_amd/harness/models.py
--- a/uno_amd/harness/models.py
+++ b/uno_amd/harness/models.py
@@ -6,7 +6,7 @@
 import torch.nn as nn
 import torch.nn.functional as F
 
-from ..integral_operators import (GradJoin, OperatorBlock_2D, OperatorBlock_3D, channel_mix, channel_mix_cat, channel_mix_cat_project,
+from ..integral_operators import (GradJoin, SpectrumShare, OperatorBlock_2D, OperatorBlock_3D, channel_mix, channel_mix_cat, channel_mix_cat_project,
                                   enable_native_resample3d_any, enable_one_buffer_any_grid, gelu_channel_mix, gelu_channel_mix_pad, gelu_pad2d, gelu_project, gelu_project2,
                                   lift_gelu_pad)
 
@@ -67,10 +67,11 @@
         if fused:
             jc, j2 = GradJoin(), GradJoin()
             c0 = self.conv0(lifted, d1 // 2, d2 // 2, join=jl, out_join=jc)
-            c1 = self.conv1(c0, d1 // 4, d2 // 4, join=jc)
+            sc = SpectrumShare.for_block(self.conv5, self.conv4.conv.out_channels)
+            c1 = self.conv1(c0, d1 // 4, d2 // 4, join=jc, share=sc)
             c2 = self.conv2(c1, d1 // 4, d2 // 4, out_join=j2)
             skip5 = [self.conv4(c2, d1 // 2, d2 // 2, join=j2), c0]
-            out = channel_mix_cat_project([self.conv5.forward_cat(skip5, d1, d2, defer_gelu=True, defer_grad=jc), lifted], self.fc1.weight,
+            out = channel_mix_cat_project([self.conv5.forward_cat(skip5, d1, d2, defer_gelu=True, defer_grad=jc, share=sc), lifted], self.fc1.weight,
                                           self.fc1.bias, self.fc2.weight, self.fc2.bias, gelu_first=True, defer_grad=jl, crop=(S1, S2))
             return out[:, :, :S1, :S2].permute(0, 2, 3, 1).contiguous()
         else:
diff --git a/uno_amd/integral_operators.py b/uno_amd/integral_operators.py
--- a/uno_amd/integral_operators.py
+++ b/uno_amd/integral_operators.py
@@ -5,14 +5,14 @@
 import torch.nn.functional as F
 
 from ._param_grads import release_pass_state
-from .block2d import _OperatorBlock2dCatFn, _OperatorBlock2dFn, _SpectralConv2dFn, spectral_conv2d, spectral_conv2d_mixed
+from .block2d import SpectrumShare, _OperatorBlock2dCatFn, _OperatorBlock2dFn, _SpectralConv2dFn, spectral_conv2d, spectral_conv2d_mixed
 from .pointwise import (GradJoin, _dev_act, channel_mix, channel_mix_cat, channel_mix_cat_project, gelu_channel_mix, gelu_channel_mix_pad,
                         gelu_pad2d, gelu_project, gelu_project2, instance_norm_gelu, lift_gelu_pad)
 from .resample import resample2d_bicubic_aa
 from .spectral3d import (_FftResample3dAnyFn, _FftResample3dFn, _OperatorBlock3dFn, _resample3d_plan, _resample3d_plan_any, spectral_conv3d)
 
 __all__ = [
-    "enable_mixed_precision", "enable_native_resample3d_any", "enable_one_buffer_any_grid", "GradJoin", "channel_mix_cat_project", "release_pass_state",
+    "enable_mixed_precision", "enable_native_resample3d_any", "enable_one_buffer_any_grid", "GradJoin", "SpectrumShare", "channel_mix_cat_project", "release_pass_state",
     "SpectralConv1d_Uno", "pointwise_op_1D", "OperatorBlock_1D",
     "SpectralConv2d_Uno", "pointwise_op_2D", "OperatorBlock_2D",
     "SpectralConv3d_Uno", "pointwise_op_3D", "OperatorBlock_3D",
@@ -98,17 +98,17 @@
         if Normalize:
             self.normalize_layer = nn.InstanceNorm2d(int(out_codim), affine=True)
 
-    def forward(self, x, dim1=None, dim2=None, *, join=None, out_join=None):
+    def forward(self, x, dim1=None, dim2=None, *, join=None, out_join=None, share=None):
         if self.non_lin and not self.normalize:
-            return self._branches(x, dim1, dim2, gelu=True, join=join, out_join=out_join)
+            return self._branches(x, dim1, dim2, gelu=True, join=join, out_join=out_join, share=share)
         if out_join is not None:
             out_join.void()
-        out = self._branches(x, dim1, dim2, join=join)
+        out = self._branches(x, dim1, dim2, join=join, share=share)
         if self.normalize:
             return instance_norm_gelu(out, self.normalize_layer, self.non_lin)
         return out
 
-    def forward_cat(self, xs, dim1=None, dim2=None, defer_gelu=False, defer_grad=None):
+    def forward_cat(self, xs, dim1=None, dim2=None, defer_gelu=False, defer_grad=None, share=None):
         if defer_gelu and (self.normalize or not self.non_lin):
             raise ValueError("defer_gelu needs a block with Non_Lin=True and Normalize=False")
         xs = list(xs)
@@ -128,14 +128,14 @@
         if dim1 is not None:
             conv.dim1, conv.dim2 = dim1, dim2
         out = _OperatorBlock2dCatFn.apply(xs[0], xs[1], conv.weights1, conv.weights2, w.conv.weight, w.conv.bias, int(d1), int(d2),
-                                          xs[0].dtype == torch.bfloat16, defer_grad)
+                                          xs[0].dtype == torch.bfloat16, defer_grad, share)
         if defer_gelu:
             return out
         if self.normalize:
             return instance_norm_gelu(out, self.normalize_layer, self.non_lin)
         return F.gelu(out) if self.non_lin else out
 
-    def _branches(self, x, dim1, dim2, gelu=False, join=None, out_join=None):
+    def _branches(self, x, dim1, dim2, gelu=False, join=None, out_join=None, share=None):
         conv, w = self.conv, self.w
         if dim1 is not None:
             conv.dim1, conv.dim2 = dim1, dim2
@@ -151,7 +151,7 @@
             out = conv(x) + w(x, d1, d2)
             return F.gelu(out) if gelu else out
         return _OperatorBlock2dFn.apply(x, conv.weights1, conv.weights2, w.conv.weight, w.conv.bias, int(d1), int(d2),
-                                        x.dtype == torch.bfloat16, bool(gelu), join, out_join)
+                                        x.dtype == torch.bfloat16, bool(gelu), join, out_join, share)
 
     def _takes(self, x):
         return (x.is_cuda and x.dim() == 4 and
```

Result: faster. 1581 samples/s, median of 6 (+2.6%).
